# clayne/CPU-Raytracer

Hardware: AMD Instinct MI355X
Metric: Mrays/s (primary+shadow+reflection+refraction) (higher is better)
Workload: dtype f32

## Files before the change

### cpu-raytracer_amd/csrc/plan_check.cpp

```cpp
#include <stdio.h>
#include <initializer_list>
#include <type_traits>
#include "rtx_plan.h"

static_assert(std::is_trivially_copyable<RenderPlan>::value, "the graph key compares a plan's bytes");

static int failures = 0;
static const char * current = "";
#define CASE(name) current = name
#define CHECK(x) do { if (!(x)) { printf("FAILED [%s] line %d: %s\n", current, __LINE__, #x); failures++; } } while (0)

enum { CW = RTX_RENDER_COUNT_WORK, SIMPLE = RTX_RENDER_SIMPLE_TRACE, CULL = RTX_RENDER_CULL_DEAD_SHADOW_RAYS, SERIAL = RTX_RENDER_SERIAL,
       LANE = RTX_RENDER_LANE_TRACE, PSTAT = RTX_RENDER_PACKET_STATS, PKC = RTX_RENDER_PACKET_CLOSEST, AOV = RTX_RENDER_AOV };
static const int NEVER = RTX_MAX_LEVELS + 1;

static PlanInputs frame() {
    PlanInputs in; memset(&in, 0, sizeof(in));
    in.tile_count = 64; in.batch_tiles = 64;
    Knobs & K = in.knobs;
    K.slot_budget = 48ll * 1000 * 1000; K.item_bytes_max = 1ll << 30; K.shade_grid = 4; K.lane_from_level = -1; K.lane_from_level_any = -1;
    K.split_items = 256; K.resolve_block = 256; K.pk4_order = 1; K.merge_any = true; K.lpt = -1;
    in.instance_count = 1; in.light_count = 2; in.bounces = 3; in.can_spawn = true; in.all_wide = true;
    in.stack = StackFigures{ false, 1, 10, 20 };
    in.n_cu = 256; in.pk_blocks_closest = 1024; in.pk_blocks_any = 1280;
// ... 317 lines not shown
    }
    CASE("graph");
    {
        PlanInputs in = frame(); in.knobs.graph = true;
        CHECK(plan_render(in).graph_eligible);
        in.timing = true;  CHECK(!plan_render(in).graph_eligible);
        in.timing = false; in.knobs.graph = false; CHECK(!plan_render(in).graph_eligible);
    }
    CASE("more tiles than a batch");
    {
        PlanInputs in = frame(); in.knobs.graph = true; in.knobs.lpt = 1; in.tile_count = 65;
        RenderPlan p = plan_render(in);
        CHECK(!p.graph_eligible && !p.lpt);
        in.knobs.graph = false;
        p = plan_render(in);
        CHECK(!p.graph_eligible && !p.lpt);
        in.tile_count = 64;
        CHECK(plan_render(in).lpt);
    }
    CASE("the key sees flags and views");
    {
        PlanInputs a = frame(), b = frame(); b.views = 1;
        CHECK(!same(plan_render(a), plan_render(b)));
        b = frame(CULL);
        CHECK(!same(plan_render(a), plan_render(b)));
    }
}

static void small_grids() {
    const struct { int n_cu, pk_closest, pk_any; } grids[] = { { 1, 8, 8 }, { 1, 16, 8 }, { 2, 16, 24 }, { 2, 32, 32 }, { 8, 32, 32 }, { 8, 8, 16 } };
    auto small = [](int n_cu, int pkc, int pka, uint32_t flags) {
        PlanInputs in = frame(flags); in.n_cu = n_cu; in.pk_blocks_closest = pkc; in.pk_blocks_any = pka; in.tile_count = in.batch_tiles = 60;
        return in;
    };
    CASE("small grids: a level's partial tallies fit its stride");
    for (const auto & g : grids)
        for (int fuse = 0; fuse <= 1; fuse++)
            for (uint32_t flags : { 0u, (uint32_t)SERIAL, (uint32_t)LANE, (uint32_t)CW, (uint32_t)SIMPLE, (uint32_t)AOV, (uint32_t)(CULL | SERIAL) }) {
                PlanInputs in = small(g.n_cu, g.pk_closest, g.pk_any, flags); in.knobs.fuse_shade = fuse != 0; in.bounces = RTX_MAX_LEVELS - 1;
                for (int shade_grid : { 1, 4, 64 }) {
                    in.knobs.shade_grid = shade_grid;
                    const RenderPlan p = plan_render(in);
                    CHECK(p.levels == RTX_MAX_LEVELS && p.shade_blocks == g.n_cu * shade_grid && p.pk_waves_closest == g.pk_closest);
                    CHECK(p.stats_stride >= 64 && p.stats_stride >= p.shade_blocks && p.stats_stride >= p.pk_waves_closest);
                    for (int slots : { 1024, 60 * 1024, 2025 * 1024 })
                        for (int l = 0; l < p.levels; l++) {
                            const int n = plan_stats_n(p, slots, l);
                            CHECK(n >= 1 && n <= p.stats_stride);
                            CHECK(n == (p.shade[l] == SHADE_NONE ? g.pk_closest : plan_level_blocks(slots, l, p.shade_blocks)));
                        }
                    if (fuse && flags == 0u) CHECK(all_shade(p, SHADE_NONE));
                    if (!fuse) for (int l = 0; l < p.levels; l++) CHECK(p.shade[l] != SHADE_NONE);
                }
            }
    {
        const RenderPlan p = plan_render(small(1, 8, 8, 0u));
        CHECK(p.shade_blocks == 4 && p.stats_stride == 64 && plan_stats_n(p, 60 * 1024, 0) == 64 && plan_stats_n(p, 60 * 1024, 3) == 64);
        CHECK(plan_render(small(8, 32, 32, 0u)).stats_stride == 64 && plan_render(small(32, 96, 96, 0u)).stats_stride == 128);
        CHECK(plan_render(frame()).stats_stride == 1024);
    }
    CASE("small grids: item capacity follows the chunk count");
    {
        CHECK(plan_render(small(1, 8, 8, 0u)).item_cap == 24192);
        CHECK(plan_render(small(2, 16, 16, 0u)).item_cap == 12096);
        CHECK(plan_render(small(8, 32, 32, 0u)).item_cap == 6080);
        PlanInputs in = small(1, 8, 8, 0u); in.tile_count = in.batch_tiles = 200;
        CHECK(plan_render(in).item_cap == 1 << 16 && plan_render(in).split);
        in.knobs.item_bytes_max = 8ll * 48 * 128;
        CHECK(plan_render(in).item_cap == 128 && plan_render(in).split);
        in.knobs.item_bytes_max = 8ll * 48 * 63;
        CHECK(plan_render(in).item_cap == 0 && !plan_render(in).split);
        in = small(1, 8, 8, 0u); in.knobs.split_items = 64; in.tile_count = in.batch_tiles = 1; in.light_count = 1;
        CHECK(plan_render(in).item_cap == 256);
    }
    CASE("small grids: the LPT default rule");
    for (const auto & g : grids) {
        PlanInputs in = small(g.n_cu, g.pk_closest, g.pk_any, 0u);
        RenderPlan p = plan_render(in);
        CHECK(p.lpt && p.lpt_n == 960);
        in.flags = SERIAL;
        CHECK(!plan_render(in).lpt);
        in.knobs.lpt = 1;
        CHECK(plan_render(in).lpt);
        in.flags = 0; in.knobs.lpt = 0;
        CHECK(!plan_render(in).lpt);
        in.knobs.lpt = -1; in.tile_count = in.batch_tiles = g.pk_closest / 8;
        CHECK(plan_render(in).lpt);
        if (g.pk_closest > 8) { in.tile_count = in.batch_tiles = g.pk_closest / 8 - 1; CHECK(!plan_render(in).lpt); }
    }
}

static void twelve_levels() {
    CASE("twelve levels");
    const int L = RTX_MAX_LEVELS;
    static_assert(sizeof(((RenderPlan *)0)->any) / sizeof(AnyLaunch) == RTX_MAX_LEVELS && sizeof(((RenderPlan *)0)->closest) / sizeof(int32_t) == RTX_MAX_LEVELS &&
                  sizeof(((RenderPlan *)0)->shade) / sizeof(int32_t) == RTX_MAX_LEVELS, "the plan's per-level arrays");
    long plans = 0;
    for (uint32_t bits = 0; bits < 256; bits++) {
        const uint32_t flags = (bits & 1 ? SERIAL : 0) | (bits & 2 ? LANE : 0) | (bits & 4 ? PKC : 0) | (bits & 8 ? CULL : 0) | (bits & 16 ? CW : 0) |
                               (bits & 32 ? SIMPLE : 0) | (bits & 64 ? PSTAT : 0) | (bits & 128 ? AOV : 0);
        for (int lights : { 1, 33 }) for (int instances : { 1, 2, 65 }) for (int fuse = 0; fuse <= 1; fuse++) for (int split : { 0, 64 })
        for (int merge = 0; merge <= 1; merge++) for (int lane_from : { -1, 0, 5, 11 }) for (int lane_from_any : { -1, 5 }) {
            PlanInputs in = frame(flags);
            in.bounces = L - 1; in.can_spawn = true; in.light_count = lights; in.instance_count = instances;
            in.knobs.fuse_shade = fuse != 0; in.knobs.split_items = split; in.knobs.merge_any = merge != 0;
            in.knobs.lane_from_level = lane_from; in.knobs.lane_from_level_any = lane_from_any;
            const RenderPlan p = plan_render(in);
            plans++;
            CHECK(p.levels == L);
            CHECK(p.n_any >= 1 && p.n_any <= L);
            const bool plain = (flags & (CW | SIMPLE)) != 0;
            for (int l = 0; l < L; l++) {
                const int c = p.closest[l], s = p.shade[l];
                CHECK(c >= CLOSEST_PLAIN && c <= CLOSEST_PACKET_FUSED_CULL && s >= SHADE_NONE && s <= SHADE_AOV_CULL);
                CHECK((c == CLOSEST_PLAIN || c == CLOSEST_PLAIN_COUNT) == plain);
                CHECK((s == SHADE_NONE) == (c == CLOSEST_PACKET_FUSED || c == CLOSEST_PACKET_FUSED_CULL));
                CHECK((s == SHADE_AOV || s == SHADE_AOV_COUNT || s == SHADE_AOV_CULL) == ((flags & AOV) != 0 && l == 0));
                const int n = plan_stats_n(p, in.batch_tiles * 1024, l);
                CHECK(n >= 1 && n <= p.stats_stride);
            }
            int covered[RTX_MAX_LEVELS] = { 0 };
            int last_after = -1;
            for (int i = 0; i < p.n_any && i < L; i++) {
                const AnyLaunch & a = p.any[i];
                CHECK(a.lo >= 0 && a.lo <= a.hi && a.hi <= L - 1);
                CHECK(a.after_level >= a.hi && a.after_level <= p.levels - 1);
                CHECK(a.after_level >= last_after); last_after = a.after_level;
                CHECK(a.stream == (p.overlap ? 1 : 0));
                CHECK(a.kernel >= ANY_PLAIN && a.kernel <= ANY_PACKET_SPLIT && (a.items == 0 || a.kernel == ANY_PACKET_SPLIT));
                if (a.kernel == ANY_PLAIN || a.kernel == ANY_PLAIN_COUNT) CHECK(a.lo == a.hi);
                for (int l = a.lo; l <= a.hi && l < L; l++) if (l >= 0) covered[l]++;
            }
            for (int l = 0; l < L; l++) CHECK(covered[l] == 1);
            if (p.split) CHECK(p.item_cap >= 64 && p.item_cap <= (1 << 16));
        }
    }
    CHECK(plans == 256l * 2 * 3 * 2 * 2 * 2 * 4 * 2);
    {
        PlanInputs in = frame(SERIAL); in.bounces = L - 1; in.light_count = 33;
        CHECK(schedule(plan_render(in), { { 11, 0, ANY_PACKET_SPLIT, 0, 11, 1 } }));
        in.flags = 0;
        CHECK(schedule(plan_render(in), { { 0, 1, ANY_PACKET_SPLIT, 0, 0, 1 }, { 11, 1, ANY_PACKET_SPLIT, 1, 11, 1 } }));
        in.instance_count = 2; in.knobs.split_items = 0;
        CHECK(schedule(plan_render(in), { { 0, 1, ANY_PACKET, 0, 0, 0 }, { 11, 1, ANY_PACKET, 1, 1, 0 }, { 11, 1, ANY_LANE, 2, 11, 0 } }));
        in.knobs.lane_from_level = 11;
        const RenderPlan p = plan_render(in);
        CHECK(p.closest[10] == CLOSEST_PACKET && p.closest[11] == CLOSEST_LANE);
        CHECK(schedule(p, { { 0, 1, ANY_PACKET, 0, 0, 0 }, { 11, 1, ANY_PACKET, 1, 10, 0 }, { 11, 1, ANY_LANE, 11, 11, 0 } }));
        in.flags = SERIAL; in.knobs.merge_any = false;
        CHECK(plan_render(in).n_any == L);
    }
}

int main() {
    small_grids();
    twelve_levels();
    modes_and_schedule();
    instrumented_modes();
    stack_limits();
    two_deep_trees();
    lpt_items_graph();
    if (failures) { printf("plan_check: %d FAILED\n", failures); return 1; }
    printf("plan_check: ok\n");
    return 0;
}
```

### cpu-raytracer_amd/csrc/rtx_api.hip

```cpp
#include <hip/hip_runtime.h>
#include <stdio.h>
#include <stdlib.h>
#include <string.h>
#include <math.h>
#include <string>
#include <vector>
#include <algorithm>
#include <type_traits>

#include "../../include/rtx.h"
#include "rtx_device.h"
#include "rtx_math.h"
#include "rtx_libm.h"
#include "rtx_texture.h"
#include "rtx_trace.h"
#include "rtx_shade.h"
#include "rtx_packet.h"
#include "rtx_present.h"
#include "rtx_update.h"
#include "rtx_refit.h"
#include "rtx_build.h"
#include "rtx_normals.h"
#include "rtx_query.h"
#include "rtx_nearest.h"
#include "rtx_hits.h"
#include "rtx_sweep.h"
#include "rtx_overlap.h"
#include "rtx_boxsweep.h"
#include "rtx_texmip.h"
#include <rocprim/device/device_radix_sort.hpp>
#include "rtx_hostmem.h"
#include "rtx_layout_host.h"
#include "rtx_plan.h"

#define SLOT_BUDGET (48ll * 1000 * 1000)

static long long knob_int(const char * name, long long dflt, long long lo, long long hi) {
    const char * e = getenv(name);
    if (!e || !*e) return dflt;
    char * end = nullptr; const long long v = strtoll(e, &end, 10);
    if (end == e || *end != 0 || v < lo || v > hi) { fprintf(stderr, "librtx_hip: %s=%s ignored (expected an integer in [%lld, %lld])\n", name, e, lo, hi); return dflt; }
    return v;
}
static double knob_real(const char * name, double dflt, double lo, double hi) {
    const char * e = getenv(name);
    if (!e || !*e) return dflt;
    char * end = nullptr; const double v = strtod(e, &end);
    if (end == e || *end != 0 || !(v >= lo && v <= hi)) { fprintf(stderr, "librtx_hip: %s=%s ignored (expected a number in [%g, %g])\n", name, e, lo, hi); return dflt; }
    return v;
}
struct KernelTime { const char * name; hipEvent_t a, b; };

struct rtx_ctx {
    rtx_config cfg;
    hipStream_t stream = nullptr;
    hipStream_t own_stream = nullptr;
    hipStream_t any_stream = nullptr;
    hipEvent_t ev_shade0 = nullptr, ev_shade_last = nullptr, ev_any_done = nullptr;
    void * ext_rgb = nullptr, * ext_packed = nullptr;
    std::string err;
    int n_cu = 0;

    struct BlasRefit { std::vector<int32_t> map4, map4c; bool bound = false; int32_t vertex_count = 0; DevBuf block; DevRefit dev; float * planes[3] = { nullptr, nullptr, nullptr }; void * sort_tmp = nullptr; size_t sort_bytes = 0; };
    struct BlasBuild { bool allocated = false; DevBuf block; DevBuild dev; void * sort_tmp = nullptr; size_t sort_bytes = 0; int levels = 0; };
    struct BlasNormals { bool allocated = false, set = false; DevBuf block; DevNormals dev; void * sort_tmp = nullptr; size_t sort_bytes = 0; unsigned int key_bits = 0; };
    struct BlasSide { bool allocated = false; DevBuf block; DevSide dev; };
    struct BlasHost { std::vector<DevBuf> arrays; int max_local_material = -1, inner_depth = -1; bool packet_ok = true; BlasRefit refit; BlasBuild build; BlasNormals normals; BlasSide side; };
    std::vector<DevBlas> h_blas;
    std::vector<BlasHost> blas;
    DevBuf d_blas, d_materials, d_textures, d_sky, d_ewa;
    std::vector<DevTexture> h_tex;
    std::vector<DevBuf> tex_texels;
    struct TexUpdate { bool allocated = false; rtxt::Plan plan; };
    std::vector<TexUpdate> tex_update;
    DevBuf d_srgb_lut;
    bool sky_uploaded = false;
    int material_count = 0, sky_size = 0;
    std::vector<rtx_material> h_materials; int tlas_inner_depth = -1; std::vector<int> frame_primitive_materials; bool refs_dirty = true; Knobs knobs; int item_blocks = 0, item_cap_alloc = 0; DevBuf d_pk_items, d_pk_item_count;

    DevBuf d_frame;
    StageRing frame_ring;
    DevScene scene;
    bool frame_set = false;
    bool frame_rigid = true;
    DevBuf d_upd, d_upd_sort; int upd_cap = 0;
    DevBuf d_views, d_vfb_rgb, d_vfb_packed;
    StageRing view_ring;
    int32_t view_count = 0, vfb_cap = 0, ext_vcap = 0;
    void * ext_vrgb = nullptr, * ext_vpacked = nullptr;
    DevBuf d_rays;
    StageRing ray_ring;
    int32_t ray_count = 0, ext_ray_count = 0;
    const void * ext_rays = nullptr;
    uint32_t aov_channels = 0; bool aov_ext = false; int64_t aov_ext_cap = 0; DevAov aov_ext_ptrs = {};
    DevBuf d_aov[8]; int64_t aov_own_cap[8] = {};

    DevQueues q;
    DevBuf qb[20];
    DevBuf d_query[4], d_query_counters, d_query_heads; int32_t query_cap = 0;
    DevBuf d_query_sort; int32_t query_sort_cap = 0; size_t query_sort_tmp = 0;
    DevBuf d_nearest_head; bool nearest_fetch = true;
    int query_grid = 0;
    DevBuf d_object_masks; StageRing mask_ring; bool masks_set = false; int32_t mask_counts[3] = { 0, 0, 0 };
    std::vector<DevSideBlas> h_side; DevBuf d_side; StageRing side_ring; bool side_dirty = true;
    size_t slots_alloc = 0, shadow_alloc = 0;
    DevBuf d_stats_partial, d_pk_fifo, d_counters, d_spill, d_fb_rgb, d_fb_packed, d_display, d_gamma, d_pk_heads;
    int trace_blocks_closest = 0, trace_blocks_any = 0, trace_blocks_count = 0;
    int pk_blocks_closest = 0, pk_blocks_any = 0;

    rtx_stats stats_acc; rtx_work_counters work_acc; uint32_t err_flags_acc = 0;
    bool stats_pending = false;

    bool timing = false;
    bool serial = false;
    hipGraphExec_t graph_exec = nullptr; std::vector<unsigned char> graph_key, graph_warm;
    DevBuf d_pk_cost, d_pk_order; hipStream_t order_stream = nullptr; hipEvent_t ev_cost = nullptr, ev_order = nullptr; int32_t lpt_key[5] = { -1, -1, -1, -1, -1 }; bool lpt_valid = false;
    std::vector<KernelTime> times;
    std::vector<hipEvent_t> event_pool;
    size_t event_next = 0;
};

extern "C" int rtx_abi_version(void) { return RTX_ABI_VERSION; }

extern "C" const char * rtx_last_error(const rtx_ctx * ctx) { return ctx ? ctx->err.c_str() : "null context"; }

extern "C" int rtx_create(const rtx_config * config, rtx_ctx ** out_ctx) {
    if (!config || !out_ctx) return RTX_ERR_INVALID_ARG;
    *out_ctx = nullptr;
    if (config->width <= 0 || config->height <= 0 || config->bounces < 0) return RTX_ERR_INVALID_ARG;
    if (config->bounces + 1 > RTX_MAX_LEVELS) return RTX_ERR_LIMIT;
    if (config->stack_size < 1 || config->stack_size > RTX_MAX_STACK) return RTX_ERR_LIMIT;
    if (config->traversal_strategy < 0 || config->traversal_strategy > 1 || config->texture_mode < 0 || config->texture_mode > 2 ||
        config->mip_filter < 0 || config->mip_filter > 2) return RTX_ERR_INVALID_ARG;
    int n_dev = 0;
    if (hipGetDeviceCount(&n_dev) != hipSuccess || n_dev <= 0) return RTX_ERR_NO_DEVICE;
    if (config->device < 0 || config->device >= n_dev) return RTX_ERR_NO_DEVICE;
    if (hipSetDevice(config->device) != hipSuccess) return RTX_ERR_NO_DEVICE;

    rtx_ctx * c = new rtx_ctx();
    c->cfg = *config;
    memset(&c->scene, 0, sizeof(c->scene));
    memset(&c->q, 0, sizeof(c->q));
    memset(&c->stats_acc, 0, sizeof(c->stats_acc));
    memset(&c->work_acc, 0, sizeof(c->work_acc));
    hipDeviceProp_t prop;
    if (hipGetDeviceProperties(&prop, config->device) != hipSuccess) { delete c; return RTX_ERR_HIP; }
    c->n_cu = prop.multiProcessorCount;
    {
        const long long cus = knob_int("RTX_GRID_CUS", c->n_cu, 1, 1 << 20);
        if (cus < c->n_cu) c->n_cu = (int)cus;
    }
    if (hipStreamCreateWithFlags(&c->own_stream, hipStreamNonBlocking) != hipSuccess) { delete c; return RTX_ERR_HIP; }
    c->stream = c->own_stream;
    hipEventCreateWithFlags(&c->ev_shade0, hipEventDisableTiming); hipEventCreateWithFlags(&c->ev_shade_last, hipEventDisableTiming);
    hipEventCreateWithFlags(&c->ev_any_done, hipEventDisableTiming);

    float ewa[RTX_EWA_LUT_SIZE];
    {
        const float alpha = 2.0f;
        const float denom = 1.0f / (float)(RTX_EWA_LUT_SIZE - 1);
        const float exp_neg_alpha = expf(-alpha);
        for (int i = 0; i < RTX_EWA_LUT_SIZE; i++) { float r2 = (float)i * denom; ewa[i] = expf(-alpha * r2) - exp_neg_alpha; }
    }
    int rc = upload(c, c->d_ewa, ewa, sizeof(ewa));
    rtx_material m0; memset(&m0, 0, sizeof(m0)); m0.texture_id = -1; m0.index_of_refraction = 1.0f;
    if (!rc) rc = upload(c, c->d_materials, &m0, sizeof(m0));
    c->material_count = 1;
    const size_t px = (size_t)config->width * config->height;
    if (!rc) rc = ensure(c, c->d_fb_rgb, px * 12);
    if (!rc) rc = ensure(c, c->d_fb_packed, px * 4);
    if (!rc) rc = ensure(c, c->d_counters, sizeof(DevCounters));
    if (!rc) rc = ensure(c, c->d_pk_heads, (size_t)2 * (RTX_MAX_LEVELS + 1) * RTX_PK_CLASSES * 32 * sizeof(uint32_t));
    float zero_sky[6] = { 0, 0, 0, 0, 0, 0 };
    if (!rc) rc = upload(c, c->d_sky, zero_sky, sizeof(zero_sky));
    c->sky_size = 1;
    if (rc) { rtx_destroy(c); return rc; }
    hipMemset(c->d_fb_rgb.p, 0, px * 12);
    hipMemset(c->d_fb_packed.p, 0, px * 4);

    Knobs & K = c->knobs;
    K.slot_budget = knob_int("RTX_SLOT_BUDGET", SLOT_BUDGET, 1024, 1ll << 31);
    K.item_bytes_max = knob_int("RTX_PK_ITEM_BYTES", 1ll << 30, 0, 1ll << 36);
    K.shade_grid = (int)knob_int("RTX_SHADE_GRID", 4, 1, 64);
    K.lane_from_level = (int)knob_int("RTX_LANE_FROM_LEVEL", -1, 0, 1 << 20);
    K.lane_from_level_any = (int)knob_int("RTX_LANE_FROM_LEVEL_ANY", -1, 0, 1 << 20);
    K.split_items = (int)knob_int("RTX_PK_SPLIT", 256, 0, 1 << 16);
    if (K.split_items > 0) K.split_items = (K.split_items + 63) & ~63;
    K.resolve_block = (int)knob_int("RTX_RESOLVE_BLOCK", 256, 64, 256);
    if (K.resolve_block != 64 && K.resolve_block != 128 && K.resolve_block != 256) K.resolve_block = 256;
    K.pk4_order = (int)knob_int("RTX_PK4_ORDER", 1, 0, 1);
    K.merge_any = knob_int("RTX_SERIAL_MERGE_ANY", 1, 0, 1) != 0;
    K.no_wide = knob_int("RTX_PK_WIDE", 1, 0, 1) == 0;
    K.lpt = (int)knob_int("RTX_PK_LPT", -1, -1, 1);
    K.graph = knob_int("RTX_GRAPH", 0, 0, 1) != 0;
    K.no_wide_closest = knob_int("RTX_PK_WIDE_CLOSEST", 1, 0, 1) == 0;
    K.fuse_shade = knob_int("RTX_FUSE_SHADE", 0, 0, 1) != 0;
    K.update_small_max = (int)knob_int("RTX_UPDATE_SMALL_MAX", RTX_UPDATE_SMALL_MAX, 0, RTX_UPDATE_SMALL_MAX);
    K.tex_pass_levels = (int)knob_int("RTX_TEX_PASS_LEVELS", rtxt::DEFAULT_PASS_LEVELS, 1, rtxt::MAX_PASS_LEVELS);
    c->nearest_fetch = knob_int("RTX_NEAREST_FETCH", 1, 0, 1) != 0;
    c->query_grid = (int)knob_int("RTX_QUERY_GRID", 0, 0, 1 << 20);
    K.fail_item_alloc = knob_int("RTX_DEBUG_FAIL_ITEM_ALLOC", 0, 0, 1) != 0;
    int bpc = 0;
    hipOccupancyMaxActiveBlocksPerMultiprocessor(&bpc, k_trace_fast<false>, RTX_TRACE_BLOCK, 0);
    c->trace_blocks_closest = c->n_cu * (bpc > 0 ? bpc : 2);
    hipOccupancyMaxActiveBlocksPerMultiprocessor(&bpc, k_trace_fast<true>, RTX_TRACE_BLOCK, 0);
    c->trace_blocks_any = c->n_cu * (bpc > 0 ? bpc : 2);
    hipOccupancyMaxActiveBlocksPerMultiprocessor(&bpc, k_trace<false, true>, RTX_TRACE_BLOCK, 0);
    c->trace_blocks_count = c->n_cu * (bpc > 0 ? bpc : 2);
    if (K.fuse_shade) hipOccupancyMaxActiveBlocksPerMultiprocessor(&bpc, k_packet<false, false, false, true, false>, RTX_PK_BLOCK, 0);
    else              hipOccupancyMaxActiveBlocksPerMultiprocessor(&bpc, k_packet<false, false>, RTX_PK_BLOCK, 0);
    c->pk_blocks_closest = (c->n_cu * (bpc > 0 ? bpc : 4) + 1) & ~1;
    hipOccupancyMaxActiveBlocksPerMultiprocessor(&bpc, k_packet<true, false>, RTX_PK_BLOCK, 0);
    c->pk_blocks_any = (c->n_cu * (bpc > 0 ? bpc : 4) + 1) & ~1;
    {
        const double f = knob_real("RTX_PK_GRID_SCALE", 1.0, 0.05, 16.0);
        if (f != 1.0) { c->pk_blocks_closest = ((int)(c->pk_blocks_closest * f) + 1) & ~1; c->pk_blocks_any = ((int)(c->pk_blocks_any * f) + 1) & ~1; }
        const double fa = knob_real("RTX_PK_GRID_ANY", 0.0, 0.05, 64.0), fc = knob_real("RTX_PK_GRID_CLOSEST", 0.0, 0.05, 64.0);
        if (fa > 0.0) c->pk_blocks_any = ((int)(c->n_cu * fa) + 1) & ~1;
        if (fc > 0.0) c->pk_blocks_closest = ((int)(c->n_cu * fc) + 1) & ~1;
    }
    {
        const int g = RTX_PK_CLASSES * RTX_WAVE / RTX_PK_BLOCK > 1 ? RTX_PK_CLASSES * RTX_WAVE / RTX_PK_BLOCK : 1;
        c->pk_blocks_any = (c->pk_blocks_any + g - 1) / g * g; c->pk_blocks_closest = (c->pk_blocks_closest + g - 1) / g * g;
        if (c->pk_blocks_any < g) c->pk_blocks_any = g;
        if (c->pk_blocks_closest < g) c->pk_blocks_closest = g;
    }
    long long max_threads = (long long)(c->trace_blocks_closest > c->trace_blocks_any ? c->trace_blocks_closest : c->trace_blocks_any) * RTX_TRACE_BLOCK;
    if ((long long)c->trace_blocks_count * RTX_TRACE_BLOCK > max_threads) max_threads = (long long)c->trace_blocks_count * RTX_TRACE_BLOCK;
    if ((long long)c->pk_blocks_any * RTX_PK_BLOCK > max_threads) max_threads = (long long)c->pk_blocks_any * RTX_PK_BLOCK;
    if ((long long)c->pk_blocks_closest * RTX_PK_BLOCK > max_threads) max_threads = (long long)c->pk_blocks_closest * RTX_PK_BLOCK;
    c->q.pk_defer_t0 = (int)knob_int("RTX_PK_DEFER", 8, 0, 64);
    c->q.pk_defer_leaf = (int)knob_int("RTX_PK_DEFER_LEAF", c->q.pk_defer_t0 / 2, 0, 64);
    c->q.pk_defer_t0_closest = (int)knob_int("RTX_PK_DEFER_CLOSEST", 64, 0, 64);
    c->q.pk_closest_asm = (int)knob_int("RTX_PK_CLOSEST_ASM", 1, 0, 1);
    c->q.pk_defer_t0_primary = (int)knob_int("RTX_PK_DEFER_PRIMARY", c->q.pk_closest_asm ? 4 : 64, 0, 64);
    c->q.pk_order = (int)knob_int("RTX_PK_ORDER", 1, 0, 1);
    c->q.prof_level = (int)knob_int("RTX_LANE_PROF_LEVEL", 2, 0, 100 + RTX_MAX_LEVELS);
    c->q.pk_defer_grow = (int)knob_int("RTX_PK_GROW", 3, 0, 31);
    c->q.spill_threads = (int)max_threads;
    rc = ensure(c, c->d_spill, (size_t)c->q.spill_threads * (RTX_MAX_STACK - RTX_LDS_STACK) * 4 * 3);
    if (!rc) rc = ensure(c, c->d_pk_fifo, (size_t)c->q.spill_threads * RTX_PK_FIFO * 8);
    { int ib = 0; hipOccupancyMaxActiveBlocksPerMultiprocessor(&ib, k_items, RTX_ITEM_BLOCK, 0); c->item_blocks = c->n_cu * (ib > 0 ? ib : 4);
      const double f = knob_real("RTX_ITEM_GRID", 0.0, 0.05, 64.0); if (f > 0.0) c->item_blocks = (int)(c->n_cu * f) > 0 ? (int)(c->n_cu * f) : 1; }
    c->q.pk_items = nullptr; c->q.pk_item_count = nullptr; c->q.pk_item_cap = 0;
    if (rc) { rtx_destroy(c); return rc; }
    bind_tables(c);
    *out_ctx = c;
    return RTX_OK;
}

extern "C" int rtx_destroy(rtx_ctx * c) {
    if (!c) return RTX_ERR_INVALID_ARG;
    hipSetDevice(c->cfg.device);
    if (c->stream) hipStreamSynchronize(c->stream);
    for (hipEvent_t e : c->event_pool) hipEventDestroy(e);
    if (c->graph_exec) { hipGraphExecDestroy(c->graph_exec); c->graph_exec = nullptr; }
    if (c->order_stream) { hipStreamSynchronize(c->order_stream); hipStreamDestroy(c->order_stream); hipEventDestroy(c->ev_cost); hipEventDestroy(c->ev_order); }
    if (c->any_stream) { hipStreamSynchronize(c->any_stream); hipStreamDestroy(c->any_stream); }
    if (c->ev_shade0) hipEventDestroy(c->ev_shade0);
    if (c->ev_shade_last) hipEventDestroy(c->ev_shade_last);
    if (c->ev_any_done) hipEventDestroy(c->ev_any_done);
    if (c->own_stream) hipStreamDestroy(c->own_stream);
    delete c;
    return RTX_OK;
}

static bool validate_tree(const rtx_bvh_node * nodes, int node_count, int64_t primitive_count, int * max_inner_depth = nullptr, int * max_leaf_count = nullptr) {
    if (node_count < 1) return false;
    std::vector<unsigned char> seen((size_t)node_count, 0);
    std::vector<std::pair<int, int>> stack(1, std::make_pair(0, 0));
    int deepest = -1, biggest = 0;
    while (!stack.empty()) {
        const int i = stack.back().first, d = stack.back().second; stack.pop_back();
        if (seen[i]) return false;
        seen[i] = 1;
        const int cnt = nodes[i].count & 0x3fffffff, f = nodes[i].left_or_first;
        if (cnt > 0) { if (f < 0 || (int64_t)f + cnt > primitive_count) return false; if (cnt > biggest) biggest = cnt; }
        else { if (f < 0 || f + 1 >= node_count) return false; if (d > deepest) deepest = d; stack.push_back(std::make_pair(f, d + 1)); stack.push_back(std::make_pair(f + 1, d + 1)); }
    }
    if (max_inner_depth) *max_inner_depth = deepest;
    if (max_leaf_count) *max_leaf_count = biggest;
    return true;
}


struct BlasStaged { DevBlas B; rtx_ctx::BlasHost H; };

template <typename T> static int stage_array(rtx_ctx * c, std::vector<DevBuf> & arrays, const void * src, size_t copy, size_t bytes, const T ** out) {
    DevBuf b;
    if (int rc = ensure(c, b, bytes)) return rc;
    if (copy) HIP_OK(c, hipMemcpy(b.p, src, copy, hipMemcpyHostToDevice));
    *out = (const T *)b.p;
    arrays.push_back(std::move(b));
    return RTX_OK;
}

template <typename Accept> static int upload_blas_table(rtx_ctx * c, std::vector<DevBlas> & table, Accept && accept) {
    return replace_table(c, c->d_blas, table.data(), table.size() * sizeof(DevBlas), [&] { c->h_blas.swap(table); accept(); });
}

static void drop_side_entry(rtx_ctx * c, int32_t blas_id) {
    if ((size_t)blas_id < c->h_side.size() && c->h_side[blas_id].vert_pn) { memset(&c->h_side[blas_id], 0, sizeof(DevSideBlas)); c->side_dirty = true; }
}

static int commit_blas(rtx_ctx * c, int32_t blas_id, BlasStaged & S) {
    std::vector<DevBlas> table = c->h_blas;
    if ((size_t)blas_id >= table.size()) { DevBlas none; memset(&none, 0, sizeof(none)); table.resize(blas_id + 1, none); }
    table[blas_id] = S.B;
    return upload_blas_table(c, table, [&] {
        if (c->blas.size() < c->h_blas.size()) c->blas.resize(c->h_blas.size());
        c->blas[blas_id] = std::move(S.H);
        c->refs_dirty = true;
        drop_side_entry(c, blas_id);
    });
}

static int stage_blas(rtx_ctx * c, int32_t blas_id, const rtx_bvh_node * nodes, int32_t node_count,
                      const rtx_triangle_hot * tri_hot, const rtx_triangle_cold * tri_cold,
                      int32_t triangle_count, int32_t material_offset, int pk4_order, BlasStaged & S) {
    if (!c || blas_id < 0 || blas_id >= (1 << 20) || !nodes || node_count <= 0 || triangle_count < 0 || (triangle_count > 0 && (!tri_hot || !tri_cold)))
        return RTX_ERR_INVALID_ARG;
    int inner_depth = -1, leaf_max = 0;
    if (!validate_tree(nodes, node_count, triangle_count, &inner_depth, &leaf_max)) return RTX_ERR_INVALID_ARG;
    int max_local = -1;
    for (int i = 0; i < triangle_count; i++) { if (tri_cold[i].material_id < 0) return RTX_ERR_INVALID_ARG; if (tri_cold[i].material_id > max_local) max_local = tri_cold[i].material_id; }
    hipSetDevice(c->cfg.device);

    std::vector<float4> nd; convert_nodes(nodes, node_count, nd);
    std::vector<float4> th((size_t)RTX_TRI_STRIDE * (triangle_count > 0 ? triangle_count : 1), make_float4(0.0f, 0.0f, 0.0f, 0.0f));
    for (int i = 0; i < triangle_count; i++) {
        th[RTX_TRI_STRIDE * (size_t)i]     = make_float4(tri_hot[i].position_0[0], tri_hot[i].position_0[1], tri_hot[i].position_0[2], 0.0f);
        th[RTX_TRI_STRIDE * (size_t)i + 1] = make_float4(tri_hot[i].position_edge_1[0], tri_hot[i].position_edge_1[1], tri_hot[i].position_edge_1[2], 0.0f);
        th[RTX_TRI_STRIDE * (size_t)i + 2] = make_float4(tri_hot[i].position_edge_2[0], tri_hot[i].position_edge_2[1], tri_hot[i].position_edge_2[2], 0.0f);
    }
    std::vector<float4> ndp; convert_nodes_pk(nodes, node_count, ndp);
    rtx_ctx::BlasHost & H = S.H;
    std::vector<float4> nd4; int need4 = 0;
    const bool wide = !c->knobs.no_wide && build_nodes_pk4(nodes, node_count, triangle_count, nd4, &need4, pk4_order, RTX_PK4_MAX_NEED, &H.refit.map4) && need4 <= RTX_PK4_MAX_NEED;
    std::vector<float4> nd4c; int need4c = 0;
    const bool wide_closest = !c->knobs.no_wide_closest && build_nodes_pk4c(nodes, node_count, triangle_count, nd4c, &need4c, &H.refit.map4c) && need4c <= RTX_MAX_STACK - 2;
    if (!wide) H.refit.map4.clear();
    if (!wide_closest) H.refit.map4c.clear();
    std::vector<float> planes[3];
    for (int a = 0; a < 3; a++) {
        planes[a].reserve((size_t)node_count * 2);
        for (int i = 0; i < node_count; i++) { planes[a].push_back(nodes[i].aabb_min[a]); planes[a].push_back(nodes[i].aabb_max[a]); }
        planes[a].erase(std::remove_if(planes[a].begin(), planes[a].end(), [](float v) { return v != v; }), planes[a].end());
        std::sort(planes[a].begin(), planes[a].end());
        planes[a].erase(std::unique(planes[a].begin(), planes[a].end()), planes[a].end());
        if (planes[a].empty()) planes[a].push_back(INFINITY);
    }
    DevBlas & B = S.B;
    memset(&B, 0, sizeof(B));
    int rc = RTX_OK;
    for (int a = 0; a < 3 && !rc; a++) { rc = stage_array(c, H.arrays, planes[a].data(), planes[a].size() * 4, planes[a].size() * 4, &B.planes[a]); B.plane_count[a] = (int32_t)planes[a].size(); }
    if (!rc && wide_closest) rc = stage_array(c, H.arrays, nd4c.data(), nd4c.size() * 16, nd4c.size() * 16, &B.pk4c_nodes);
    if (!rc && wide) rc = stage_array(c, H.arrays, nd4.data(), nd4.size() * 16, nd4.size() * 16, &B.pk4_nodes);
    if (!rc) rc = stage_array(c, H.arrays, nd.data(), nd.size() * 16, nd.size() * 16, &B.nodes);
    if (!rc) rc = stage_array(c, H.arrays, ndp.data(), ndp.size() * 16, ndp.size() * 16, &B.pk_nodes);
    if (!rc) rc = stage_array(c, H.arrays, th.data(), th.size() * 16, th.size() * 16, &B.tri_hot);
    if (!rc) rc = stage_array(c, H.arrays, tri_cold, (size_t)triangle_count * sizeof(rtx_triangle_cold), (size_t)(triangle_count > 0 ? triangle_count : 1) * sizeof(rtx_triangle_cold), &B.tri_cold);
    if (rc) return rc;
    B.node_count = node_count; B.tri_count = triangle_count; B.material_offset = material_offset; B.pk4_need = wide ? need4 : -1; B.pk4c_need = wide_closest ? need4c : -1;
    H.max_local_material = max_local;
    H.inner_depth = inner_depth;
    H.packet_ok = leaf_max < 65536 && node_count < (1 << 26) && triangle_count < (1 << 25);
    return RTX_OK;
}

extern "C" int rtx_upload_blas(rtx_ctx * c, int32_t blas_id, const rtx_bvh_node * nodes, int32_t node_count,
                               const rtx_triangle_hot * tri_hot, const rtx_triangle_cold * tri_cold,
                               int32_t triangle_count, int32_t material_offset) {
    BlasStaged S;
    if (int rc = stage_blas(c, blas_id, nodes, node_count, tri_hot, tri_cold, triangle_count, material_offset, c ? c->knobs.pk4_order : 0, S)) return rc;
    return commit_blas(c, blas_id, S);
}

extern "C" int rtx_upload_materials(rtx_ctx * c, const rtx_material * materials, int32_t count) {
    if (!c || !materials || count <= 0) return RTX_ERR_INVALID_ARG;
    if (count > RTX_MAX_MATERIALS) return RTX_ERR_LIMIT;
    hipSetDevice(c->cfg.device);
    return replace_table(c, c->d_materials, materials, (size_t)count * sizeof(rtx_material), [&] {
        c->material_count = count;
        c->h_materials.assign(materials, materials + count); c->refs_dirty = true;
    });
}

static int commit_texture(rtx_ctx * c, int32_t texture_id, const rtx_texture_desc & desc, DevBuf & d, const rtx_ctx::TexUpdate & update) {
    std::vector<DevTexture> table = c->h_tex;
    if ((size_t)texture_id >= table.size()) { DevTexture none; memset(&none, 0, sizeof(none)); table.resize(texture_id + 1, none); }
    table[texture_id].desc = desc;
    table[texture_id].texels = (const float4 *)d.p;
    return replace_table(c, c->d_textures, table.data(), table.size() * sizeof(DevTexture), [&] {
        c->h_tex.swap(table);
        if (c->tex_texels.size() < c->h_tex.size()) { c->tex_texels.resize(c->h_tex.size()); c->tex_update.resize(c->h_tex.size()); }
        c->tex_texels[texture_id] = std::move(d);
        c->tex_update[texture_id] = update;
        c->refs_dirty = true;
    });
}

extern "C" int rtx_upload_texture(rtx_ctx * c, int32_t texture_id, const rtx_texture_desc * desc, const float * texels_rgb, int64_t texel_count) {
    if (!c || texture_id < 0 || texture_id >= 4096 || !desc || !texels_rgb) return RTX_ERR_INVALID_ARG;
    if (desc->width <= 0 || desc->height <= 0 || desc->mip_levels < 1 || desc->mip_levels > RTX_MAX_MIP_LEVELS) return RTX_ERR_INVALID_ARG;
    for (int l = 0; l < desc->mip_levels; l++) {
        const int64_t lw = desc->width >> l, lh = desc->height >> l;
        if (lw < 1 || lh < 1 || desc->mip_offsets[l] < 0 || desc->mip_offsets[l] + lw * lh > texel_count) return RTX_ERR_INVALID_ARG;
    }
    hipSetDevice(c->cfg.device);
    DevBuf d;
    {
        std::vector<float4> padded((size_t)texel_count);
        for (int64_t i = 0; i < texel_count; i++) padded[(size_t)i] = make_float4(texels_rgb[3 * i], texels_rgb[3 * i + 1], texels_rgb[3 * i + 2], 0.0f);
        if (int rc = upload(c, d, padded.data(), (size_t)texel_count * 16)) return rc;
    }
    return commit_texture(c, texture_id, *desc, d, rtx_ctx::TexUpdate());
}

extern "C" int rtx_upload_sky(rtx_ctx * c, const float * texels_rgb, int32_t size) {
    if (!c || !texels_rgb || size <= 0 || size > 16384) return RTX_ERR_INVALID_ARG;
    hipSetDevice(c->cfg.device);
    std::vector<float> padded((size_t)size * size * 3 + 3, 0.0f);
    memcpy(padded.data(), texels_rgb, (size_t)size * size * 12);
    return replace_table(c, c->d_sky, padded.data(), padded.size() * 4, [&] { c->sky_size = size; c->sky_uploaded = true; });
}

extern "C" int rtx_set_frame(rtx_ctx * c, const rtx_frame * f) {
    if (!c || !f) return RTX_ERR_INVALID_ARG;
    if (f->tlas_node_count < 0 || f->instance_count < 0 || f->sphere_count < 0 || f->plane_count < 0 || f->tlas_index_count < 0 ||
        f->point_light_count < 0 || f->spot_light_count < 0 || f->directional_light_count < 0) return RTX_ERR_INVALID_ARG;
    if ((f->tlas_node_count && !f->tlas_nodes) || (f->instance_count && !f->instances) || (f->tlas_index_count && !f->tlas_indices) ||
        (f->sphere_count && !f->spheres) || (f->plane_count && !f->planes) || (f->point_light_count && !f->point_lights) ||
        (f->spot_light_count && !f->spot_lights) || (f->directional_light_count && !f->directional_lights)) return RTX_ERR_INVALID_ARG;
    if (f->instance_count >= (1 << 28) || f->sphere_count >= (1 << 28) || f->plane_count >= (1 << 28)) return RTX_ERR_LIMIT;
    hipSetDevice(c->cfg.device);
    int tlas_depth = -1;
    if (f->tlas_node_count > 0 && !validate_tree(f->tlas_nodes, f->tlas_node_count, f->tlas_index_count, &tlas_depth)) return RTX_ERR_INVALID_ARG;
    for (int i = 0; i < f->tlas_index_count; i++) if (f->tlas_indices[i] < 0 || f->tlas_indices[i] >= f->instance_count) return RTX_ERR_INVALID_ARG;
    for (int i = 0; i < f->instance_count; i++) {
        const int b = f->instances[i].blas_id;
        if (b < 0 || (size_t)b >= c->h_blas.size() || !c->h_blas[b].nodes) return RTX_ERR_STATE;
    }
    bool rigid = true;
    for (int i = 0; i < f->instance_count; i++) {
        if (!rtxu::matrix_finite(f->instances[i].world) || !rtxu::matrix_finite(f->instances[i].world_inv)) {
            c->err = "rtx_set_frame: instance " + std::to_string(i) + " has a NaN or infinite world / world_inv cell"; return RTX_ERR_INVALID_ARG;
        }
        rigid = rigid && rtxu::instance_rigid(f->instances[i].world, f->instances[i].world_inv);
    }
    std::vector<float4> nd, ndp; convert_nodes(f->tlas_nodes, f->tlas_node_count, nd); convert_nodes_pk(f->tlas_nodes, f->tlas_node_count, ndp);
    const void * src[9] = { nd.data(), ndp.data(), f->tlas_indices, f->instances, f->spheres, f->planes, f->point_lights, f->spot_lights, f->directional_lights };
    const size_t len[9] = { nd.size() * 16, ndp.size() * 16, (size_t)f->tlas_index_count * 4, (size_t)f->instance_count * sizeof(rtx_instance),
                            (size_t)f->sphere_count * sizeof(rtx_sphere), (size_t)f->plane_count * sizeof(rtx_plane), (size_t)f->point_light_count * sizeof(rtx_point_light),
                            (size_t)f->spot_light_count * sizeof(rtx_spot_light), (size_t)f->directional_light_count * sizeof(rtx_directional_light) };
    size_t off[9], total = 0;
    for (int k = 0; k < 9; k++) { off[k] = total; total += (len[k] + 255) & ~(size_t)255; if (len[k] == 0) total += 256; }
    int rc = RTX_OK;
    if (total > c->d_frame.cap) {
        HIP_OK(c, hipStreamSynchronize(c->stream));
        rc = ensure(c, c->d_frame, total + total / 2);
        if (rc) return rc;
    }
    rc = stage_copy(c, c->frame_ring, c->d_frame.p, total, total + total / 2, [&](void * host) { for (int k = 0; k < 9; k++) if (len[k]) memcpy((char *)host + off[k], src[k], len[k]); });
    if (rc) return rc;
    char * const fb = (char *)c->d_frame.p;

    DevScene & s = c->scene;
    s.width = c->cfg.width; s.height = c->cfg.height; s.bounces = c->cfg.bounces; s.stack_size = c->cfg.stack_size;
    s.traversal_strategy = c->cfg.traversal_strategy; s.texture_mode = c->cfg.texture_mode; s.mip_filter = c->cfg.mip_filter;
    s.heatmap = c->cfg.heatmap ? 1 : 0;
    s.diff_enabled = c->cfg.texture_mode == RTX_TEXTURE_MIPMAP;
    s.max_anisotropy = c->cfg.max_anisotropy;
    s.tile_count_x = (c->cfg.width + RTX_TILE_SIZE - 1) / RTX_TILE_SIZE;
    memcpy(s.cam_pos, f->camera.position, 12); memcpy(s.cam_tl, f->camera.rotated_top_left_corner, 12);
    memcpy(s.cam_x, f->camera.rotated_x_axis, 12); memcpy(s.cam_y, f->camera.rotated_y_axis, 12);
    memcpy(s.ambient, f->ambient, 12);
    bind_tables(c);
    s.ewa_table = (const float *)c->d_ewa.p;
    s.tlas_nodes = (const float4 *)(fb + off[0]); s.tlas_node_count = f->tlas_node_count; s.pk_tlas_nodes = (const float4 *)(fb + off[1]);
    s.tlas_indices = (const int32_t *)(fb + off[2]); s.tlas_index_count = f->tlas_index_count;
    s.instances = (const rtx_instance *)(fb + off[3]); s.instance_count = f->instance_count;
    s.spheres = (const rtx_sphere *)(fb + off[4]); s.sphere_count = f->sphere_count;
    s.planes = (const rtx_plane *)(fb + off[5]); s.plane_count = f->plane_count;
    s.point_lights = (const rtx_point_light *)(fb + off[6]); s.point_light_count = f->point_light_count;
    s.spot_lights = (const rtx_spot_light *)(fb + off[7]); s.spot_light_count = f->spot_light_count;
    s.dir_lights = (const rtx_directional_light *)(fb + off[8]); s.dir_light_count = f->directional_light_count;
    s.light_count = f->point_light_count + f->spot_light_count + f->directional_light_count;
    c->frame_primitive_materials.clear();
    for (int i = 0; i < f->sphere_count; i++) c->frame_primitive_materials.push_back(f->spheres[i].material_id);
    for (int i = 0; i < f->plane_count; i++) c->frame_primitive_materials.push_back(f->planes[i].material_id);
    c->tlas_inner_depth = tlas_depth;
    c->frame_set = true; c->refs_dirty = true; c->frame_rigid = rigid;
    return RTX_OK;
}

static int validate_references(rtx_ctx * c) {
    if (!c->refs_dirty) return RTX_OK;
    const int nm = c->material_count;
    for (int id : c->frame_primitive_materials) if (id < 0 || id >= nm) { c->err = "sphere / plane material id outside the uploaded material table"; return RTX_ERR_STATE; }
    for (size_t b = 0; b < c->h_blas.size(); b++) {
        if (!c->h_blas[b].nodes) continue;
        const int hi = c->blas[b].max_local_material;
        if (c->h_blas[b].material_offset < 0 || (hi >= 0 && (long long)c->h_blas[b].material_offset + hi >= nm)) { c->err = "BLAS material_offset + triangle material id outside the uploaded material table"; return RTX_ERR_STATE; }
    }
    for (size_t b = 0; b < c->h_blas.size(); b++)
        if (c->h_blas[b].nodes && c->blas[b].inner_depth + 2 > c->cfg.stack_size) {
            c->err = "BVH deeper than rtx_config.stack_size allows (BVH_TRAVERSAL_STACK_SIZE, Config.h:25): an inner node at depth " + std::to_string(c->blas[b].inner_depth) + " needs " + std::to_string(c->blas[b].inner_depth + 2) + " stack entries";
            return RTX_ERR_LIMIT;
        }
    if (c->tlas_inner_depth + 2 > c->cfg.stack_size) { c->err = "TLAS deeper than rtx_config.stack_size allows (BVH_TRAVERSAL_STACK_SIZE, Config.h:25)"; return RTX_ERR_LIMIT; }
    for (size_t i = 0; i < c->h_materials.size(); i++) {
        const int t = c->h_materials[i].texture_id;
        if (t >= 0 && ((size_t)t >= c->h_tex.size() || !c->h_tex[t].texels)) { c->err = "material refers to a texture id that was never uploaded"; return RTX_ERR_STATE; }
    }
    c->refs_dirty = false;
    return RTX_OK;
}

static int plan_batch(rtx_ctx * c, int tiles, int & out_tiles) {
    const int levels = c->cfg.bounces + 1;
    const long long per_tile = 1024ll * ((1ll << levels) - 1);
    const long long budget = c->knobs.slot_budget;
    long long t = budget / per_tile;
    if (t < 1) t = 1;
    out_tiles = (int)(t < tiles ? t : tiles);
    return RTX_OK;
}

static int alloc_queues(rtx_ctx * c, int batch_tiles) {
    const int levels = c->cfg.bounces + 1;
    const long long P = 1024ll * batch_tiles;
    long long total = 0;
    const long long chunk_slack = c->knobs.fuse_shade ? (long long)c->pk_blocks_closest * (RTX_PK_BLOCK / RTX_WAVE) * RTX_PK_CHUNK : 0;
    for (int d = 0; d <= RTX_MAX_LEVELS; d++) {
        long long cap = d < levels ? (P << d) + (d > 0 ? chunk_slack : 0) : 0;
        c->q.level_base[d] = (int32_t)total; c->q.level_cap[d] = (int32_t)cap;
        total += cap;
    }
    if (total >= (1ll << 31)) { c->err = "batch too large"; return RTX_ERR_LIMIT; }
    const int nL = c->scene.light_count;
    long long stotal = 0;
    for (int d = 0; d <= RTX_MAX_LEVELS; d++) { c->q.shadow_base[d] = (int32_t)stotal; stotal += (long long)c->q.level_cap[d] * nL; }
    if (stotal >= (1ll << 31)) { c->err = "shadow queue too large"; return RTX_ERR_LIMIT; }
    const size_t slots = (size_t)total, sslots = (size_t)(stotal > 0 ? stotal : 1);
    int rc = 0, k = 0;
    void ** f4[] = { (void **)&c->q.r0, (void **)&c->q.r1, (void **)&c->q.r2, (void **)&c->q.r3, (void **)&c->q.r4, (void **)&c->q.h0,
                     (void **)&c->q.n0, (void **)&c->q.n1, (void **)&c->q.n2, (void **)&c->q.c0, (void **)&c->q.c1,
                     (void **)&c->q.sp, (void **)&c->q.sn };
    for (void ** p : f4) { if (!rc) rc = ensure(c, c->qb[k], slots * 16); *p = c->qb[k].p; k++; }
    if (!rc) rc = ensure(c, c->qb[k], slots * 4); c->q.h1 = (int32_t *)c->qb[k].p; k++;
    c->q.views = nullptr; c->q.s0 = c->q.s1 = nullptr; c->q.shadow_explicit = 0; c->q.cull = 0;
    if (!rc) rc = ensure(c, c->qb[k], sslots * 4); c->q.socc = (uint32_t *)c->qb[k].p; k++;
    c->q.spill = (int32_t *)c->d_spill.p;
    c->q.counters = (DevCounters *)c->d_counters.p;
    c->q.pk_heads = (uint32_t *)c->d_pk_heads.p;
    c->q.pk_fifo = (int32_t *)c->d_pk_fifo.p;
    c->q.fb_rgb = (float *)(c->ext_rgb ? c->ext_rgb : c->d_fb_rgb.p);
    c->q.fb_packed = (uint32_t *)(c->ext_packed ? c->ext_packed : c->d_fb_packed.p);
    return rc;
}

__global__ void k_begin_batch(DevCounters * ctr, uint32_t * pk_heads, uint32_t primary_slots, uint32_t closest_threads, uint32_t any_threads,
                              uint32_t pk_waves_closest, uint32_t pk_waves_any, int first_batch) {
    const int i = threadIdx.x;
    if (first_batch) {
        uint32_t * w = reinterpret_cast<uint32_t *>(ctr);
        for (int k = i; k < (int)(sizeof(DevCounters) / 4); k += blockDim.x) w[k] = 0u;
        __syncthreads();
    }
    if (i <= RTX_MAX_LEVELS) { ctr->ray_count[i] = (i == 0) ? primary_slots : 0u; ctr->item_max[i] = 0u; ctr->fetch_closest[i] = closest_threads; ctr->fetch_any[i] = any_threads; }
    for (int k = i; k < 2 * (RTX_MAX_LEVELS + 1) * RTX_PK_CLASSES; k += blockDim.x)
        pk_heads[k * 32] = (k < (RTX_MAX_LEVELS + 1) * RTX_PK_CLASSES ? pk_waves_closest : pk_waves_any) / RTX_PK_CLASSES;
}

static hipEvent_t next_event(rtx_ctx * c) {
    if (c->event_next == c->event_pool.size()) { hipEvent_t e; hipEventCreate(&e); c->event_pool.push_back(e); }
    return c->event_pool[c->event_next++];
}

__global__ __launch_bounds__(1024) void k_packet_order(const uint32_t * __restrict__ cost, uint32_t * __restrict__ order, const uint32_t n) {
    __shared__ uint32_t hist[256], base[256];
    for (uint32_t i = threadIdx.x; i < 256; i += blockDim.x) hist[i] = 0;
    __syncthreads();
    auto cls = [](uint32_t c) { const uint32_t k = c >> 7; return 255u - (k < 255u ? k : 255u); };
    for (uint32_t i = threadIdx.x; i < n; i += blockDim.x) atomicAdd(&hist[cls(cost[i])], 1u);
    __syncthreads();
    if (threadIdx.x == 0) { uint32_t acc = 0; for (int k = 0; k < 256; k++) { base[k] = acc; acc += hist[k]; } }
    __syncthreads();
    for (uint32_t i = threadIdx.x; i < n; i += blockDim.x) order[atomicAdd(&base[cls(cost[i])], 1u)] = i;
}

template <typename F>
static void launch_timed(rtx_ctx * c, const char * name, hipStream_t stream, F && launch) {
    if (c->timing) {
        KernelTime kt; kt.name = name; kt.a = next_event(c); kt.b = next_event(c);
        hipEventRecord(kt.a, stream);
        launch();
        hipEventRecord(kt.b, stream);
        c->times.push_back(kt);
    } else launch();
}

static void begin_batch(rtx_ctx * c, DevCounters * counters, uint32_t * pk_heads, uint32_t primary_slots, bool plain, bool first_batch) {
    hipLaunchKernelGGL(k_begin_batch, dim3(1), dim3(64), 0, c->stream, counters, pk_heads, primary_slots,
                       (uint32_t)((plain ? c->trace_blocks_count : c->trace_blocks_closest) * RTX_TRACE_BLOCK),
                       (uint32_t)((plain ? c->trace_blocks_count : c->trace_blocks_any) * RTX_TRACE_BLOCK),
                       (uint32_t)(c->pk_blocks_closest * (RTX_PK_BLOCK / RTX_WAVE)), (uint32_t)(c->pk_blocks_any * (RTX_PK_BLOCK / RTX_WAVE)), first_batch ? 1 : 0);
}

static void launch_closest_level1(rtx_ctx * c, const DevScene & sc, const DevQueues & q, bool lane) {
    if (lane) hipLaunchKernelGGL((k_trace_fast<false>), dim3(c->trace_blocks_closest), dim3(RTX_TRACE_BLOCK), 0, c->stream, sc, q, 1, 1);
    else      hipLaunchKernelGGL((k_packet<false, false>), dim3(c->pk_blocks_closest), dim3(RTX_PK_BLOCK), 0, c->stream, sc, q, 1, 1);
}
static void launch_any_level0(rtx_ctx * c, const DevScene & sc, const DevQueues & q, bool lane) {
    if (lane) hipLaunchKernelGGL((k_trace_fast<true>), dim3(c->trace_blocks_any), dim3(RTX_TRACE_BLOCK), 0, c->stream, sc, q, 0, 0);
    else      hipLaunchKernelGGL((k_packet<true, false>), dim3(c->pk_blocks_any), dim3(RTX_PK_BLOCK), 0, c->stream, sc, q, 0, 0);
}

static int32_t frame_tiles(const rtx_ctx * c) { return ((c->cfg.width + RTX_TILE_SIZE - 1) / RTX_TILE_SIZE) * ((c->cfg.height + RTX_TILE_SIZE - 1) / RTX_TILE_SIZE); }
static bool all_meshes_wide(const rtx_ctx * c) {
    for (const DevBlas & b : c->h_blas) if (b.nodes && !b.pk4_nodes) return false;
    return true;
}

static size_t aligned_parts(const size_t * len, size_t * off, int n) {
    size_t total = 0;
    for (int k = 0; k < n; k++) { off[k] = total; total += (len[k] + 255) & ~(size_t)255; }
    return total;
}

template <typename Key> static int sort_storage_bytes(rtx_ctx * c, size_t count, unsigned int bits, size_t & bytes) {
    bytes = 0;
    if (rocprim::radix_sort_keys(nullptr, bytes, (const Key *)nullptr, (Key *)nullptr, (unsigned int)count, 0u, bits, c->stream) == hipSuccess) return RTX_OK;
    hipGetLastError(); c->err = "rocprim::radix_sort_keys size query failed"; return RTX_ERR_HIP;
}

static int sort_failed(rtx_ctx * c, hipError_t se) {
    hipGetLastError(); c->err = std::string("rocprim::radix_sort_keys: ") + hipGetErrorString(se); return RTX_ERR_HIP;
}

static int read_lane_nodes(rtx_ctx * c, const float4 * dev, int n, rtx_bvh_node * out) {
    std::vector<float4> nd((size_t)2 * n);
    HIP_OK(c, hipMemcpy(nd.data(), dev, nd.size() * 16, hipMemcpyDeviceToHost));
    for (int i = 0; i < n; i++) rtxl::node_from_lane(nd.data(), i, out[i]);
    return RTX_OK;
}

extern "C" int rtx_update_instances(rtx_ctx * c, const void * positions_dev, const void * rotations_dev, int32_t instance_count) {
    if (!c) return RTX_ERR_INVALID_ARG;
    if (!positions_dev || !rotations_dev || ((uintptr_t)positions_dev & 3) || ((uintptr_t)rotations_dev & 3) || instance_count < 1) {
        c->err = "rtx_update_instances: null or misaligned pose pointer, or no instances"; return RTX_ERR_INVALID_ARG; }
    if (instance_count > RTX_UPDATE_MAX_INSTANCES) { c->err = "rtx_update_instances supports up to 65 536 instances"; return RTX_ERR_LIMIT; }
    if (!c->frame_set) { c->err = "rtx_update_instances before rtx_set_frame"; return RTX_ERR_STATE; }
    if (instance_count != c->scene.instance_count) { c->err = "rtx_update_instances: instance_count differs from the frame's"; return RTX_ERR_INVALID_ARG; }
    if (rtxu::tree_inner_depth(instance_count) + 2 > c->cfg.stack_size) {
        c->err = "rtx_update_instances: the balanced TLAS of " + std::to_string(instance_count) + " instances needs " + std::to_string(rtxu::tree_inner_depth(instance_count) + 2) +
                 " stack entries, rtx_config.stack_size allows fewer (BVH_TRAVERSAL_STACK_SIZE, Config.h:25)";
        return RTX_ERR_LIMIT;
    }
    hipSetDevice(c->cfg.device);
    const int n = instance_count, levels = rtxu::tree_levels(n), slots = rtxu::tree_node_count(n);
    const bool small = n <= c->knobs.update_small_max;
    const size_t len[7] = { (size_t)slots * 32, (size_t)slots * 32, (size_t)n * 4, (size_t)n * sizeof(rtx_instance), (size_t)n * 24, (size_t)n * 8, 24 };
    size_t off[7];
    const size_t total = aligned_parts(len, off, 7);
    if (n > c->upd_cap || total > c->d_upd.cap) {
        HIP_OK(c, hipStreamSynchronize(c->stream));
        if (int rc = ensure(c, c->d_upd, total)) return rc;
        c->upd_cap = n;
    }
    size_t sort_bytes = 0;
    if (!small) {
        if (int rc = sort_storage_bytes<uint64_t>(c, (size_t)n, RTXU_KEY_BITS, sort_bytes)) return rc;
        const size_t keys_in = ((size_t)n * 8 + 255) & ~(size_t)255;
        if (keys_in + sort_bytes > c->d_upd_sort.cap) {
            HIP_OK(c, hipStreamSynchronize(c->stream));
            if (int rc = ensure(c, c->d_upd_sort, keys_in + sort_bytes)) return rc;
        }
    }
    char * const ub = (char *)c->d_upd.p;
    DevUpdate u;
    u.positions = (const float *)positions_dev; u.rotations = (const float *)rotations_dev;
    u.src_instances = c->scene.instances; u.blas = c->scene.blas;
    u.nodes = (float4 *)(ub + off[0]); u.pk_nodes = (float4 *)(ub + off[1]); u.indices = (int32_t *)(ub + off[2]);
    u.instances = (rtx_instance *)(ub + off[3]); u.aabbs = (float *)(ub + off[4]); u.keys = (uint64_t *)(ub + off[5]); u.bounds = (uint32_t *)(ub + off[6]);
    u.n = n; u.levels = levels;
    if (small) {
        launch_timed(c, "k_update_small", c->stream, [&] { hipLaunchKernelGGL(k_update_small, dim3(1), dim3(RTX_UPDATE_BLOCK), 0, c->stream, u); });
    } else {
        uint64_t * const keys_in = (uint64_t *)c->d_upd_sort.p;
        void * const sort_tmp = (char *)c->d_upd_sort.p + (((size_t)n * 8 + 255) & ~(size_t)255);
        const int blocks = (n + 255) / 256;
        HIP_OK(c, hipMemsetAsync(u.bounds, 0xff, 24, c->stream));
        launch_timed(c, "k_update_instances", c->stream, [&] { hipLaunchKernelGGL(k_update_instances, dim3(blocks), dim3(256), 0, c->stream, u); });
        launch_timed(c, "k_update_keys", c->stream, [&] { hipLaunchKernelGGL(k_update_keys, dim3(blocks), dim3(256), 0, c->stream, u, keys_in); });
        hipError_t se = hipSuccess;
        launch_timed(c, "update_radix_sort", c->stream, [&] { se = rocprim::radix_sort_keys(sort_tmp, sort_bytes, (const uint64_t *)keys_in, u.keys, (unsigned int)n, 0u, (unsigned int)RTXU_KEY_BITS, c->stream); });
        if (se != hipSuccess) return sort_failed(c, se);
        for (int d = levels; d > RTX_UPDATE_TOP_LEVELS; d--)
            launch_timed(c, "k_update_level", c->stream, [&] { hipLaunchKernelGGL(k_update_level, dim3(((1 << d) + 255) / 256), dim3(256), 0, c->stream, u, d); });
        launch_timed(c, "k_update_top", c->stream, [&] { hipLaunchKernelGGL(k_update_top, dim3(1), dim3(RTX_UPDATE_BLOCK), 0, c->stream, u); });
    }
    HIP_OK(c, hipGetLastError());
    DevScene & s = c->scene;
    s.tlas_nodes = u.nodes; s.pk_tlas_nodes = u.pk_nodes; s.tlas_node_count = slots;
    s.tlas_indices = u.indices; s.tlas_index_count = n; s.instances = u.instances;
    c->tlas_inner_depth = rtxu::tree_inner_depth(n);
    c->refs_dirty = true;
    c->frame_rigid = true;
    return RTX_OK;
}

extern "C" int rtx_read_frame_state(rtx_ctx * c, rtx_instance * instances, rtx_bvh_node * tlas_nodes, int32_t * tlas_node_count, int32_t * tlas_indices) {
    if (!c) return RTX_ERR_INVALID_ARG;
    if (!c->frame_set) { c->err = "rtx_read_frame_state before rtx_set_frame"; return RTX_ERR_STATE; }
    hipSetDevice(c->cfg.device);
    HIP_OK(c, hipStreamSynchronize(c->stream));
    const DevScene & s = c->scene;
    if (tlas_node_count) *tlas_node_count = s.tlas_node_count;
    if (instances && s.instance_count) HIP_OK(c, hipMemcpy(instances, s.instances, (size_t)s.instance_count * sizeof(rtx_instance), hipMemcpyDeviceToHost));
    if (tlas_indices && s.tlas_index_count) HIP_OK(c, hipMemcpy(tlas_indices, s.tlas_indices, (size_t)s.tlas_index_count * 4, hipMemcpyDeviceToHost));
    if (tlas_nodes && s.tlas_node_count) return read_lane_nodes(c, s.tlas_nodes, s.tlas_node_count, tlas_nodes);
    return RTX_OK;
}

static int refit_launch_finish(rtx_ctx * c, rtx_ctx::BlasRefit & R, bool build = false) {
    const DevRefit & r = R.dev;
    const int n = r.node_count;
    const dim3 grid((2 * n + 4 + RTX_REFIT_BLOCK - 1) / RTX_REFIT_BLOCK);
    if (build) launch_timed(c, "k_build_finish", c->stream, [&] { hipLaunchKernelGGL(k_build_finish, grid, dim3(RTX_REFIT_BLOCK), 0, c->stream, r); });
    else launch_timed(c, "k_refit_finish", c->stream, [&] { hipLaunchKernelGGL(k_refit_finish, grid, dim3(RTX_REFIT_BLOCK), 0, c->stream, r); });
    hipError_t se = hipSuccess;
    launch_timed(c, "refit_plane_sort", c->stream, [&] {
        for (int a = 0; a < 3 && se == hipSuccess; a++) {
            size_t bytes = R.sort_bytes;
            se = rocprim::radix_sort_keys(R.sort_tmp, bytes, (const float *)r.plane_keys[a], R.planes[a], (unsigned int)(2 * n), 0u, 32u, c->stream);
        }
    });
    if (se != hipSuccess) return sort_failed(c, se);
    HIP_OK(c, hipGetLastError());
    return RTX_OK;
}

static int plan_refit(rtx_ctx * c, DevBlas & B, rtx_ctx::BlasRefit & R, const int32_t * slot_vertices, int32_t vertex_count) {
    const int n = B.node_count, T = B.tri_count;
    std::vector<float4> nd((size_t)2 * n);
    HIP_OK(c, hipMemcpy(nd.data(), B.nodes, nd.size() * 16, hipMemcpyDeviceToHost));
    std::vector<int32_t> parent;
    parent_table(nd.data(), n, parent);
    size_t sort_bytes = 0;
    if (int rc = sort_storage_bytes<float>(c, (size_t)2 * n, 32u, sort_bytes)) return rc;
    const size_t slots = (size_t)2 * n + 4, pl = (size_t)2 * n * 4;
    const size_t len[12] = { (size_t)(T > 0 ? T : 1) * 12, (size_t)n * 4, (size_t)n * 4, R.map4.empty() ? 0 : slots * 4, R.map4c.empty() ? 0 : slots * 4, pl, pl, pl, pl, pl, pl, sort_bytes };
    size_t off[12];
    if (int rc = ensure(c, R.block, aligned_parts(len, off, 12))) return rc;
    char * const bb = (char *)R.block.p;
    if (T) HIP_OK(c, hipMemcpy(bb + off[0], slot_vertices, (size_t)T * 12, hipMemcpyHostToDevice));
    HIP_OK(c, hipMemcpy(bb + off[1], parent.data(), (size_t)n * 4, hipMemcpyHostToDevice));
    HIP_OK(c, hipMemset(bb + off[2], 0, (size_t)n * 4));
    if (!R.map4.empty()) HIP_OK(c, hipMemcpy(bb + off[3], R.map4.data(), slots * 4, hipMemcpyHostToDevice));
    if (!R.map4c.empty()) HIP_OK(c, hipMemcpy(bb + off[4], R.map4c.data(), slots * 4, hipMemcpyHostToDevice));
    DevRefit & r = R.dev;
    memset(&r, 0, sizeof(r));
    r.slot_vertices = (const int32_t *)(bb + off[0]); r.parent = (const int32_t *)(bb + off[1]); r.arrivals = (uint32_t *)(bb + off[2]);
    r.map4 = R.map4.empty() ? nullptr : (const int32_t *)(bb + off[3]); r.map4c = R.map4c.empty() ? nullptr : (const int32_t *)(bb + off[4]);
    for (int a = 0; a < 3; a++) r.plane_keys[a] = (float *)(bb + off[5 + a]);
    r.nodes = (float4 *)B.nodes; r.pk_nodes = (float4 *)B.pk_nodes; r.pk4_nodes = (float4 *)B.pk4_nodes; r.pk4c_nodes = (float4 *)B.pk4c_nodes;
    r.tri_hot = (float4 *)B.tri_hot; r.tri_cold = (float4 *)B.tri_cold;
    r.node_count = n; r.tri_count = T;
    R.sort_tmp = bb + off[11]; R.sort_bytes = sort_bytes;
    for (int a = 0; a < 3; a++) { R.planes[a] = (float *)(bb + off[8 + a]); B.planes[a] = R.planes[a]; B.plane_count[a] = 2 * n; }
    const int rc = refit_launch_finish(c, R);
    const hipError_t waited = hipStreamSynchronize(c->stream);
    if (rc) return rc;
    if (waited != hipSuccess) { c->err = std::string("hipStreamSynchronize: ") + hipGetErrorString(waited); return RTX_ERR_HIP; }
    R.bound = true; R.vertex_count = vertex_count;
    return RTX_OK;
}

extern "C" int rtx_bind_blas_vertices(rtx_ctx * c, int32_t blas_id, const int32_t * slot_vertices, int32_t vertex_count) {
    if (!c) return RTX_ERR_INVALID_ARG;
    if (!slot_vertices || blas_id < 0 || blas_id >= (1 << 20) || vertex_count < 1) { c->err = "rtx_bind_blas_vertices: null index table, bad id or no vertices"; return RTX_ERR_INVALID_ARG; }
    if ((size_t)blas_id >= c->h_blas.size() || !c->h_blas[blas_id].nodes) { c->err = "rtx_bind_blas_vertices: no BLAS uploaded under that id"; return RTX_ERR_STATE; }
    const int64_t T3 = 3 * (int64_t)c->h_blas[blas_id].tri_count;
    for (int64_t k = 0; k < T3; k++) if (slot_vertices[k] < 0 || slot_vertices[k] >= vertex_count) {
        c->err = "rtx_bind_blas_vertices: vertex index outside [0, vertex_count)"; return RTX_ERR_INVALID_ARG; }
    hipSetDevice(c->cfg.device);
    HIP_OK(c, hipStreamSynchronize(c->stream));
    rtx_ctx::BlasRefit & R = c->blas[blas_id].refit;
    if (R.bound) {
        if (T3) HIP_OK(c, hipMemcpy((void *)R.dev.slot_vertices, slot_vertices, (size_t)T3 * 4, hipMemcpyHostToDevice));
        R.vertex_count = vertex_count;
        return RTX_OK;
    }
    DevBlas B = c->h_blas[blas_id];
    rtx_ctx::BlasRefit N; N.map4 = R.map4; N.map4c = R.map4c;
    if (int rc = plan_refit(c, B, N, slot_vertices, vertex_count)) return rc;
    std::vector<DevBlas> table = c->h_blas;
    table[blas_id] = B;
    return upload_blas_table(c, table, [&] { c->blas[blas_id].refit = std::move(N); });
}

extern "C" int rtx_refit_blas(rtx_ctx * c, int32_t blas_id, const void * positions_dev, const void * normals_dev, int32_t vertex_count) {
    if (!c) return RTX_ERR_INVALID_ARG;
    if (!positions_dev || ((uintptr_t)positions_dev & 3) || ((uintptr_t)normals_dev & 3)) { c->err = "rtx_refit_blas: null or misaligned vertex pointer"; return RTX_ERR_INVALID_ARG; }
    if (blas_id < 0 || (size_t)blas_id >= c->h_blas.size() || !c->h_blas[blas_id].nodes || !c->blas[blas_id].refit.bound) {
        c->err = "rtx_refit_blas: no BLAS uploaded under that id, or no vertices bound to it (rtx_bind_blas_vertices)"; return RTX_ERR_STATE; }
    rtx_ctx::BlasRefit & R = c->blas[blas_id].refit;
    if (vertex_count != R.vertex_count) { c->err = "rtx_refit_blas: vertex_count differs from the bound one"; return RTX_ERR_INVALID_ARG; }
    hipSetDevice(c->cfg.device);
    DevRefit & r = R.dev;
    r.positions = (const float *)positions_dev; r.normals = (const float *)normals_dev;
    const int n = r.node_count, T = r.tri_count;
    if (T) launch_timed(c, "k_refit_triangles", c->stream, [&] { hipLaunchKernelGGL(k_refit_triangles, dim3((T + RTX_REFIT_BLOCK - 1) / RTX_REFIT_BLOCK), dim3(RTX_REFIT_BLOCK), 0, c->stream, r); });
    launch_timed(c, "k_refit_climb", c->stream, [&] { hipLaunchKernelGGL(k_refit_climb, dim3((n + RTX_REFIT_BLOCK - 1) / RTX_REFIT_BLOCK), dim3(RTX_REFIT_BLOCK), 0, c->stream, r); });
    return refit_launch_finish(c, R);
}

extern "C" int rtx_alloc_blas(rtx_ctx * c, int32_t blas_id, int32_t triangle_count, int32_t vertex_count, const int32_t * material_ids, int32_t material_offset) {
    if (!c) return RTX_ERR_INVALID_ARG;
    if (blas_id < 0 || blas_id >= (1 << 20) || triangle_count < 1 || vertex_count < 1) { c->err = "rtx_alloc_blas: bad id, no triangles or no vertices"; return RTX_ERR_INVALID_ARG; }
    int max_local = 0;
    if (material_ids) for (int i = 0; i < triangle_count; i++) {
        if (material_ids[i] < 0) { c->err = "rtx_alloc_blas: negative material id"; return RTX_ERR_INVALID_ARG; }
        if (material_ids[i] > max_local) max_local = material_ids[i];
    }
    if (triangle_count >= RTX_BUILD_MAX_TRIANGLES) { c->err = "rtx_alloc_blas supports fewer than 2^24 triangles (the 4-wide walks' limit)"; return RTX_ERR_LIMIT; }
    if (rtxb::tree_inner_depth(triangle_count) + 2 > c->cfg.stack_size) {
        c->err = "rtx_alloc_blas: the balanced BLAS of " + std::to_string(triangle_count) + " triangles needs " + std::to_string(rtxb::tree_inner_depth(triangle_count) + 2) +
                 " stack entries, rtx_config.stack_size allows fewer (BVH_TRAVERSAL_STACK_SIZE, Config.h:25)";
        return RTX_ERR_LIMIT;
    }
    hipSetDevice(c->cfg.device);
    const int T = triangle_count;
    std::vector<rtx_bvh_node> nodes;
    balanced_topology(T, nodes);
    BlasStaged S;
    {
        std::vector<rtx_triangle_hot> hot((size_t)T); std::vector<rtx_triangle_cold> cold((size_t)T);
        memset(hot.data(), 0, hot.size() * sizeof(rtx_triangle_hot)); memset(cold.data(), 0, cold.size() * sizeof(rtx_triangle_cold));
        if (int rc = stage_blas(c, blas_id, nodes.data(), (int32_t)nodes.size(), hot.data(), cold.data(), T, material_offset, 0, S)) return rc;
    }
    S.H.max_local_material = max_local;
    HIP_OK(c, hipStreamSynchronize(c->stream));
    {
        std::vector<int32_t> sv((size_t)3 * T, -1);
        if (int rc = plan_refit(c, S.B, S.H.refit, sv.data(), vertex_count)) return rc;
    }
    size_t sort_bytes = 0;
    if (int rc = sort_storage_bytes<uint64_t>(c, (size_t)T, RTXB_KEY_BITS, sort_bytes)) return rc;
    const size_t len[5] = { (size_t)T * 4, 24, (size_t)T * 8, (size_t)T * 8, sort_bytes };
    size_t off[5];
    rtx_ctx::BlasBuild & U = S.H.build;
    if (int rc = ensure(c, U.block, aligned_parts(len, off, 5))) return rc;
    char * const bb = (char *)U.block.p;
    if (material_ids) HIP_OK(c, hipMemcpy(bb + off[0], material_ids, (size_t)T * 4, hipMemcpyHostToDevice));
    else HIP_OK(c, hipMemset(bb + off[0], 0, (size_t)T * 4));
    memset(&U.dev, 0, sizeof(U.dev));
    U.dev.material_ids = (const int32_t *)(bb + off[0]); U.dev.bounds = (uint32_t *)(bb + off[1]);
    U.dev.keys_in = (uint64_t *)(bb + off[2]); U.dev.keys = (uint64_t *)(bb + off[3]);
    U.dev.slot_vertices = (int32_t *)S.H.refit.dev.slot_vertices;
    U.dev.tri_count = T; U.dev.vertex_count = vertex_count;
// ... 153 lines not shown
    if (nodes) if (int rc = read_lane_nodes(c, B.nodes, B.node_count, nodes)) return rc;
    if (hot && B.tri_count) {
        std::vector<float4> th((size_t)RTX_TRI_STRIDE * B.tri_count);
        HIP_OK(c, hipMemcpy(th.data(), B.tri_hot, th.size() * 16, hipMemcpyDeviceToHost));
        for (int i = 0; i < B.tri_count; i++) {
            const float4 * t = &th[(size_t)RTX_TRI_STRIDE * i];
            hot[i].position_0[0] = t[0].x; hot[i].position_0[1] = t[0].y; hot[i].position_0[2] = t[0].z;
            hot[i].position_edge_1[0] = t[1].x; hot[i].position_edge_1[1] = t[1].y; hot[i].position_edge_1[2] = t[1].z;
            hot[i].position_edge_2[0] = t[2].x; hot[i].position_edge_2[1] = t[2].y; hot[i].position_edge_2[2] = t[2].z;
        }
    }
    if (cold && B.tri_count) HIP_OK(c, hipMemcpy(cold, B.tri_cold, (size_t)B.tri_count * sizeof(rtx_triangle_cold), hipMemcpyDeviceToHost));
    return RTX_OK;
}

extern "C" int rtx_alloc_texture(rtx_ctx * c, int32_t texture_id, int32_t width, int32_t height, int32_t mipmapped) {
    if (!c) return RTX_ERR_INVALID_ARG;
    if (texture_id < 0 || texture_id >= 4096 || width < 1 || height < 1) { c->err = "rtx_alloc_texture: id outside [0, 4096) or an empty side"; return RTX_ERR_INVALID_ARG; }
    rtx_texture_desc desc; int64_t texel_count = 0;
    if (rtxt::chain_shape(width, height, mipmapped, &desc, &texel_count)) { c->err = "rtx_alloc_texture: more than RTX_MAX_MIP_LEVELS levels, or more texels than the int32_t offsets hold"; return RTX_ERR_LIMIT; }
    hipSetDevice(c->cfg.device);
    if (!c->d_srgb_lut.p) {
        float lut[256];
        for (int b = 0; b < 256; b++) {
            const float x = float(b) * 0.00392156862f;
            lut[b] = x <= 0.0f ? 0.0f : x >= 1.0f ? 1.0f : x < 0.04045f ? x / 12.92f : powf((x + 0.055f) / 1.055f, 2.4f);
        }
        DevBuf t;
        if (int rc = upload(c, t, lut, sizeof(lut))) return rc;
        c->d_srgb_lut = std::move(t);
    }
    DevBuf d;
    if (int rc = ensure(c, d, (size_t)texel_count * 16)) return rc;
    HIP_OK(c, hipMemsetAsync(d.p, 0, (size_t)texel_count * 16, c->stream));
    rtx_ctx::TexUpdate U;
    U.allocated = true;
    U.plan = rtxt::plan_passes(width, height, desc.mip_levels, c->knobs.tex_pass_levels);
    return commit_texture(c, texture_id, desc, d, U);
}

extern "C" int rtx_update_texture(rtx_ctx * c, int32_t texture_id, const void * texels_dev, int32_t format) {
    if (!c) return RTX_ERR_INVALID_ARG;
    if (!texels_dev || (format != RTX_TEXELS_RGB_F32 && format != RTX_TEXELS_RGBA8_SRGB) || (format == RTX_TEXELS_RGB_F32 && ((uintptr_t)texels_dev & 3))) {
        c->err = "rtx_update_texture: null or misaligned texel pointer, or an unknown format"; return RTX_ERR_INVALID_ARG; }
    if (texture_id < 0 || (size_t)texture_id >= c->h_tex.size() || !c->h_tex[texture_id].texels || !c->tex_update[texture_id].allocated) {
        c->err = "rtx_update_texture: the id was not created by rtx_alloc_texture (or was uploaded again since)"; return RTX_ERR_STATE; }
    hipSetDevice(c->cfg.device);
    const rtxt::Plan & plan = c->tex_update[texture_id].plan;
    float4 * const chain = (float4 *)c->tex_texels[texture_id].p;
    const float * const lut = (const float *)c->d_srgb_lut.p;
    for (int k = 0; k < plan.count; k++) {
        const rtxt::Pass & p = plan.pass[k];
        const dim3 grid((unsigned)(p.tiles_x * p.tiles_y)), block(rtxt::BLOCK);
        if (k > 0) launch_timed(c, "k_texmip_chain", c->stream, [&] { hipLaunchKernelGGL(k_texmip<TEXMIP_CHAIN>, grid, block, 0, c->stream, p, (const void *)nullptr, chain, lut); });
        else if (format == RTX_TEXELS_RGB_F32) launch_timed(c, "k_texmip_rgb_f32", c->stream, [&] { hipLaunchKernelGGL(k_texmip<TEXMIP_RGB_F32>, grid, block, 0, c->stream, p, texels_dev, chain, lut); });
        else launch_timed(c, "k_texmip_rgba8", c->stream, [&] { hipLaunchKernelGGL(k_texmip<TEXMIP_RGBA8_SRGB>, grid, block, 0, c->stream, p, texels_dev, chain, lut); });
    }
    HIP_OK(c, hipGetLastError());
    return RTX_OK;
}

extern "C" int rtx_read_texture(rtx_ctx * c, int32_t texture_id, rtx_texture_desc * desc, float * texels_rgb, int64_t capacity_texels) {
    if (!c) return RTX_ERR_INVALID_ARG;
    if (texture_id < 0 || texture_id >= 4096) { c->err = "rtx_read_texture: bad id"; return RTX_ERR_INVALID_ARG; }
    if ((size_t)texture_id >= c->h_tex.size() || !c->h_tex[texture_id].texels) { c->err = "rtx_read_texture: no texture under that id"; return RTX_ERR_STATE; }
    const DevTexture & T = c->h_tex[texture_id];
    int64_t count = 0;
    for (int l = 0; l < T.desc.mip_levels; l++) {
        const int64_t end = (int64_t)T.desc.mip_offsets[l] + (int64_t)(T.desc.width >> l) * (T.desc.height >> l);
        if (end > count) count = end;
    }
    if (texels_rgb && capacity_texels < count) { c->err = "rtx_read_texture: capacity_texels is smaller than the chain"; return RTX_ERR_INVALID_ARG; }
    if (desc) *desc = T.desc;
    if (!texels_rgb) return RTX_OK;
    hipSetDevice(c->cfg.device);
    HIP_OK(c, hipStreamSynchronize(c->stream));
    std::vector<float4> padded((size_t)count);
    HIP_OK(c, hipMemcpy(padded.data(), T.texels, (size_t)count * 16, hipMemcpyDeviceToHost));
    for (int64_t i = 0; i < count; i++) { texels_rgb[3 * i] = padded[(size_t)i].x; texels_rgb[3 * i + 1] = padded[(size_t)i].y; texels_rgb[3 * i + 2] = padded[(size_t)i].z; }
    return RTX_OK;
}

extern "C" int rtx_update_sky(rtx_ctx * c, const void * texels_dev, int32_t size) {
    if (!c) return RTX_ERR_INVALID_ARG;
    if (!texels_dev || ((uintptr_t)texels_dev & 3)) { c->err = "rtx_update_sky: null or misaligned texel pointer"; return RTX_ERR_INVALID_ARG; }
    if (!c->sky_uploaded) { c->err = "rtx_update_sky: no probe to copy over (rtx_upload_sky)"; return RTX_ERR_STATE; }
    if (size != c->sky_size) { c->err = "rtx_update_sky: size differs from the uploaded one"; return RTX_ERR_INVALID_ARG; }
    hipSetDevice(c->cfg.device);
    HIP_OK(c, hipMemcpyAsync(c->d_sky.p, texels_dev, (size_t)size * size * 12, hipMemcpyDeviceToDevice, c->stream));
    return RTX_OK;
}

extern "C" int rtx_debug_read_layouts(rtx_ctx * c, int32_t blas_id, int32_t * info8, float * pk_nodes, float * pk4_nodes, float * pk4c_nodes,
                                      float * planes_x, float * planes_y, float * planes_z) {
    if (!c) return RTX_ERR_INVALID_ARG;
    if (blas_id < -1 || blas_id >= (1 << 20)) { c->err = "rtx_debug_read_layouts: bad id"; return RTX_ERR_INVALID_ARG; }
    int32_t info[8] = { 0, 0, 0, 0, 0, 0, 0, 0 };
    if (blas_id == -1) {
        if (!c->frame_set) { c->err = "rtx_debug_read_layouts before rtx_set_frame"; return RTX_ERR_STATE; }
        hipSetDevice(c->cfg.device);
        HIP_OK(c, hipStreamSynchronize(c->stream));
        const DevScene & s = c->scene;
        info[0] = s.tlas_node_count;
        if (info8) memcpy(info8, info, sizeof(info));
        if (pk_nodes && s.tlas_node_count) HIP_OK(c, hipMemcpy(pk_nodes, s.pk_tlas_nodes, (size_t)s.tlas_node_count * 32, hipMemcpyDeviceToHost));
        return RTX_OK;
    }
    if ((size_t)blas_id >= c->h_blas.size() || !c->h_blas[blas_id].nodes) { c->err = "rtx_debug_read_layouts: no BLAS uploaded under that id"; return RTX_ERR_STATE; }
    hipSetDevice(c->cfg.device);
    HIP_OK(c, hipStreamSynchronize(c->stream));
    const DevBlas & B = c->h_blas[blas_id];
    info[0] = B.node_count; info[1] = B.pk4_nodes ? 1 : 0; info[2] = B.pk4c_nodes ? 1 : 0;
    for (int a = 0; a < 3; a++) info[3 + a] = B.plane_count[a];
    if (info8) memcpy(info8, info, sizeof(info));
    const size_t wide_bytes = ((size_t)4 * B.node_count + 8) * 16;
    if (pk_nodes) HIP_OK(c, hipMemcpy(pk_nodes, B.pk_nodes, (size_t)B.node_count * 32, hipMemcpyDeviceToHost));
    if (pk4_nodes && B.pk4_nodes) HIP_OK(c, hipMemcpy(pk4_nodes, B.pk4_nodes, wide_bytes, hipMemcpyDeviceToHost));
    if (pk4c_nodes && B.pk4c_nodes) HIP_OK(c, hipMemcpy(pk4c_nodes, B.pk4c_nodes, wide_bytes, hipMemcpyDeviceToHost));
    float * const planes[3] = { planes_x, planes_y, planes_z };
    for (int a = 0; a < 3; a++)
        if (planes[a] && B.plane_count[a]) HIP_OK(c, hipMemcpy(planes[a], B.planes[a], (size_t)B.plane_count[a] * 4, hipMemcpyDeviceToHost));
    return RTX_OK;
}

static StackFigures stack_figures(const rtx_ctx * c) {
    StackFigures s = { false, c->tlas_inner_depth < 0 ? 0 : c->tlas_inner_depth + 1, 0, 0 };
    for (size_t b = 0; b < c->h_blas.size(); b++) {
        if (!c->h_blas[b].nodes) continue;
        if (!c->blas[b].packet_ok) s.unfit_mesh = true;
        const int depth = c->blas[b].inner_depth + 2;
        const int any = c->h_blas[b].pk4_nodes ? c->h_blas[b].pk4_need : depth;
        if (any > s.blas_any) s.blas_any = any;
        if (2 * depth > s.blas_shared) s.blas_shared = 2 * depth;
    }
    return s;
}

static int render_tiles_impl(rtx_ctx * c, int32_t first_tile, int32_t tile_stride, int32_t tile_count, uint32_t flags, uint32_t * tile_major, int views = RTX_CAM_TILES);
static int aov_targets_of_call(rtx_ctx * c, int64_t pixels, DevAov & out);

extern "C" int rtx_render_tiles(rtx_ctx * c, int32_t first_tile, int32_t tile_stride, int32_t tile_count, uint32_t flags) {
    return render_tiles_impl(c, first_tile, tile_stride, tile_count, flags, nullptr);
}

static PlanInputs gather_plan_inputs(const rtx_ctx * c, uint32_t flags, int views, int tile_count, int batch_tiles, bool tile_major) {
    PlanInputs in; memset(&in, 0, sizeof(in));
    in.flags = flags; in.views = views; in.tile_count = tile_count; in.batch_tiles = batch_tiles; in.tile_major = tile_major; in.timing = c->timing;
    in.knobs = c->knobs;
    in.instance_count = c->scene.instance_count; in.light_count = c->scene.light_count; in.bounces = c->cfg.bounces; in.heatmap = c->scene.heatmap != 0;
    in.can_spawn = plan_can_spawn(c->h_materials.data(), c->h_materials.size());
    in.all_wide = all_meshes_wide(c);
    in.stack = stack_figures(c);
    in.n_cu = c->n_cu; in.pk_blocks_closest = c->pk_blocks_closest; in.pk_blocks_any = c->pk_blocks_any;
    return in;
}

static int alloc_for_plan(rtx_ctx * c, RenderPlan & plan) {
    if (int rc = ensure(c, c->d_stats_partial, (size_t)(RTX_MAX_LEVELS + 1) * plan.stats_stride * 4 * sizeof(uint32_t))) return rc;
    c->q.pk_items = nullptr; c->q.pk_item_count = nullptr; c->q.pk_item_cap = 0;
    if (plan.split) {
        const size_t chunks = (size_t)c->pk_blocks_any * (RTX_PK_BLOCK / RTX_WAVE);
        int cap = plan.item_cap;
        if (cap <= c->item_cap_alloc && c->d_pk_items.p && !c->knobs.fail_item_alloc) cap = c->item_cap_alloc;
        else {
            c->item_cap_alloc = 0;
            const size_t bytes = c->knobs.fail_item_alloc ? ((size_t)1 << 46) : chunks * (size_t)cap * 48;
            if (ensure(c, c->d_pk_items, bytes) == 0 && ensure(c, c->d_pk_item_count, chunks * 4) == 0) c->item_cap_alloc = cap;
            else { (void)hipGetLastError(); c->err.clear(); cap = 0; }
        }
        if (cap >= 64) { c->q.pk_items = (uint4 *)c->d_pk_items.p; c->q.pk_item_count = (uint32_t *)c->d_pk_item_count.p; c->q.pk_item_cap = cap; }
        else plan_drop_split(plan);
    }
    c->q.pk_cost = nullptr; c->q.pk_lpt_order = nullptr;
    if (plan.lpt) {
        if (int rc = ensure(c, c->d_pk_cost, (size_t)plan.lpt_n * 4)) return rc;
        if (int rc = ensure(c, c->d_pk_order, (size_t)plan.lpt_n * 4)) return rc;
        if (!c->order_stream) HIP_OK(c, hipStreamCreateWithFlags(&c->order_stream, hipStreamNonBlocking));
        if (!c->ev_cost) HIP_OK(c, hipEventCreateWithFlags(&c->ev_cost, hipEventDisableTiming));
        if (!c->ev_order) HIP_OK(c, hipEventCreateWithFlags(&c->ev_order, hipEventDisableTiming));
    }
    if (plan.overlap && !c->any_stream) HIP_OK(c, hipStreamCreateWithFlags(&c->any_stream, hipStreamNonBlocking));
    return RTX_OK;
}

static int lpt_begin(rtx_ctx * c, const RenderPlan & plan, int32_t first_tile, int32_t tile_stride, int32_t tile_count) {
    if (!plan.lpt) { c->lpt_valid = false; return RTX_OK; }
    const int32_t key[5] = { first_tile, tile_stride, tile_count, plan.levels, plan.views };
    const bool use_order = c->lpt_valid && memcmp(key, c->lpt_key, sizeof(key)) == 0;
    memcpy(c->lpt_key, key, sizeof(key));
    c->q.pk_cost = (uint32_t *)c->d_pk_cost.p;
    if (use_order) c->q.pk_lpt_order = (const uint32_t *)c->d_pk_order.p;
    if (c->lpt_valid) HIP_OK(c, hipStreamWaitEvent(c->stream, c->ev_order, 0));
    return RTX_OK;
}

template <typename F>
static void with_views(int views, F && launch) {
    if (views == RTX_CAM_RAYS) launch(std::integral_constant<int, RTX_CAM_RAYS>()); else if (views) launch(std::integral_constant<int, RTX_CAM_VIEWS>()); else launch(std::integral_constant<int, RTX_CAM_TILES>());
}

static void launch_closest(rtx_ctx * c, const RenderPlan & plan, const DevScene & sc, const DevQueues & q, int level) {
    const int kernel = plan.closest[level];
    const bool fused = kernel == CLOSEST_PACKET_FUSED || kernel == CLOSEST_PACKET_FUSED_CULL;
    launch_timed(c, fused ? "k_trace_closest_shade" : "k_trace_closest", c->stream, [&] { with_views(plan.views, [&](auto V) { constexpr int VW = decltype(V)::value;
        const dim3 plain(c->trace_blocks_count), lane(c->trace_blocks_closest), tb(RTX_TRACE_BLOCK), pk(c->pk_blocks_closest), pb(RTX_PK_BLOCK);
        switch (kernel) {
        case CLOSEST_PLAIN_COUNT:       hipLaunchKernelGGL((k_trace<false, true, VW>),  plain, tb, 0, c->stream, sc, q, level); break;
        case CLOSEST_PLAIN:             hipLaunchKernelGGL((k_trace<false, false, VW>), plain, tb, 0, c->stream, sc, q, level); break;
        case CLOSEST_LANE:              hipLaunchKernelGGL((k_trace_fast<false, VW>),   lane, tb, 0, c->stream, sc, q, level, level); break;
        case CLOSEST_PACKET_STATS:      hipLaunchKernelGGL((k_packet<false, true, false, false, false, VW>),  pk, pb, 0, c->stream, sc, q, level, level); break;
        case CLOSEST_PACKET_FUSED_CULL: hipLaunchKernelGGL((k_packet<false, false, false, true, true, VW>),   pk, pb, 0, c->stream, sc, q, level, level); break;
        case CLOSEST_PACKET_FUSED:      hipLaunchKernelGGL((k_packet<false, false, false, true, false, VW>),  pk, pb, 0, c->stream, sc, q, level, level); break;
        default:                        hipLaunchKernelGGL((k_packet<false, false, false, false, false, VW>), pk, pb, 0, c->stream, sc, q, level, level); break;
        }
    }); });
}

static void launch_shade(rtx_ctx * c, const RenderPlan & plan, const DevScene & sc, const DevQueues & q, const DevAov & aov_t, int level) {
    if (plan.shade[level] == SHADE_NONE) return;
    launch_timed(c, "k_shade", c->stream, [&] { with_views(plan.views, [&](auto V) { constexpr int VW = decltype(V)::value;
        const dim3 g(plan_level_blocks(q.primary_slots, level, plan.shade_blocks)), b(RTX_SHADE_BLOCK);
        switch (plan.shade[level]) {
        case SHADE_AOV_COUNT: hipLaunchKernelGGL((k_shade<true, false, VW, true, DevAov>),  g, b, 0, c->stream, sc, q, level, aov_t); break;
        case SHADE_AOV_CULL:  hipLaunchKernelGGL((k_shade<false, true, VW, true, DevAov>),  g, b, 0, c->stream, sc, q, level, aov_t); break;
        case SHADE_AOV:       hipLaunchKernelGGL((k_shade<false, false, VW, true, DevAov>), g, b, 0, c->stream, sc, q, level, aov_t); break;
        case SHADE_COUNT:     hipLaunchKernelGGL((k_shade<true, false, VW>),  g, b, 0, c->stream, sc, q, level); break;
        case SHADE_CULL:      hipLaunchKernelGGL((k_shade<false, true, VW>),  g, b, 0, c->stream, sc, q, level); break;
        default:              hipLaunchKernelGGL((k_shade<false, false, VW>), g, b, 0, c->stream, sc, q, level); break;
        }
    }); });
}

static void launch_any(rtx_ctx * c, const AnyLaunch & a, const DevScene & sc, const DevQueues & q) {
    const hipStream_t st = a.stream ? c->any_stream : c->stream;
    const dim3 plain(c->trace_blocks_count), lane(c->trace_blocks_any), tb(RTX_TRACE_BLOCK), pk(c->pk_blocks_any), pb(RTX_PK_BLOCK);
    launch_timed(c, "k_trace_any", st, [&] {
        switch (a.kernel) {
        case ANY_PLAIN_COUNT:   hipLaunchKernelGGL((k_trace<true, true>),   plain, tb, 0, st, sc, q, a.lo); break;
        case ANY_PLAIN:         hipLaunchKernelGGL((k_trace<true, false>),  plain, tb, 0, st, sc, q, a.lo); break;
        case ANY_LANE:          hipLaunchKernelGGL((k_trace_fast<true>),    lane, tb, 0, st, sc, q, a.lo, a.hi); break;
        case ANY_PACKET_STATS:  hipLaunchKernelGGL((k_packet<true, true>),  pk, pb, 0, st, sc, q, a.lo, a.hi); break;
        case ANY_PACKET_SPLIT:  hipLaunchKernelGGL((k_packet<true, false, true>), pk, pb, 0, st, sc, q, a.lo, a.hi); break;
        default:                hipLaunchKernelGGL((k_packet<true, false>), pk, pb, 0, st, sc, q, a.lo, a.hi); break;
        }
    });
    if (a.items) launch_timed(c, "k_trace_items", st, [&] { hipLaunchKernelGGL(k_items, dim3(c->item_blocks), dim3(RTX_ITEM_BLOCK), 0, st, sc, q, c->pk_blocks_any * (RTX_PK_BLOCK / RTX_WAVE), a.lo); });
}

static int run_batch(rtx_ctx * c, const RenderPlan & plan, const DevScene & sc, const DevQueues & q, const DevAov & aov_t, bool first_batch) {
    begin_batch(c, q.counters, q.pk_heads, (uint32_t)q.primary_slots, plan.plain != 0, first_batch);
    if (plan.heatmap) {
        launch_closest(c, plan, sc, q, 0);
        launch_timed(c, "k_heatmap", c->stream, [&] { with_views(plan.views, [&](auto V) { if constexpr (decltype(V)::value != RTX_CAM_RAYS) hipLaunchKernelGGL((k_heatmap<decltype(V)::value>), dim3(plan.stream_blocks), dim3(256), 0, c->stream, sc, q); }); });
        return RTX_OK;
    }
    int next_any = 0;
    for (int level = 0; level < plan.levels; level++) {
        launch_closest(c, plan, sc, q, level);
        if (plan.lpt && level == 0) {
            HIP_OK(c, hipEventRecord(c->ev_cost, c->stream)); HIP_OK(c, hipStreamWaitEvent(c->order_stream, c->ev_cost, 0));
            hipLaunchKernelGGL(k_packet_order, dim3(1), dim3(1024), 0, c->order_stream, (const uint32_t *)c->d_pk_cost.p, (uint32_t *)c->d_pk_order.p, plan.lpt_n);
            HIP_OK(c, hipEventRecord(c->ev_order, c->order_stream));
            c->lpt_valid = true;
        }
        launch_shade(c, plan, sc, q, aov_t, level);
        bool joined = false;
        for (; next_any < plan.n_any && plan.any[next_any].after_level == level; next_any++) {
            if (plan.any[next_any].stream && !joined) {
                const hipEvent_t ev = level == 0 ? c->ev_shade0 : c->ev_shade_last;
                HIP_OK(c, hipEventRecord(ev, c->stream)); HIP_OK(c, hipStreamWaitEvent(c->any_stream, ev, 0));
                joined = true;
            }
            launch_any(c, plan.any[next_any], sc, q);
        }
    }
    if (plan.overlap) { HIP_OK(c, hipEventRecord(c->ev_any_done, c->any_stream)); HIP_OK(c, hipStreamWaitEvent(c->stream, c->ev_any_done, 0)); }
    for (int level = plan.levels - 1; level >= 0; level--)
        launch_timed(c, "k_resolve", c->stream, [&] { with_views(plan.views, [&](auto V) {
            hipLaunchKernelGGL((k_resolve<decltype(V)::value>), dim3(plan_level_blocks(q.primary_slots, level, plan.stream_blocks) * (256 / plan.resolve_block)), dim3(plan.resolve_block), 0, c->stream, sc, q, level); }); });
    return RTX_OK;
}

static std::vector<unsigned char> graph_key_of(const rtx_ctx * c, const RenderPlan & plan, int32_t first_tile, int32_t tile_stride, int32_t tile_count, const uint32_t * tile_major, const DevAov & aov_t) {
    const int32_t range[3] = { first_tile, tile_stride, tile_count };
    const struct { const void * p; size_t n; } parts[] = { { &c->scene, sizeof(DevScene) }, { &c->q, sizeof(DevQueues) }, { &plan, sizeof(plan) }, { range, sizeof(range) }, { &tile_major, sizeof(tile_major) }, { &aov_t, sizeof(aov_t) } };
    std::vector<unsigned char> key;
    for (const auto & part : parts) key.insert(key.end(), (const unsigned char *)part.p, (const unsigned char *)part.p + part.n);
    return key;
}

static int graph_finish(rtx_ctx * c, int rc) {
    hipGraph_t g = nullptr;
    const hipError_t ce = hipStreamEndCapture(c->stream, &g);
    hipError_t ie = hipSuccess;
    if (!rc && ce == hipSuccess && g) ie = hipGraphInstantiate(&c->graph_exec, g, nullptr, nullptr, 0);
    if (g) hipGraphDestroy(g);
    if (rc || ce != hipSuccess || !g || ie != hipSuccess) {
        hipGetLastError(); c->graph_exec = nullptr; c->graph_key.clear();
        if (!rc) c->err = (ce != hipSuccess || !g) ? "hipGraph capture failed" : "hipGraphInstantiate failed";
        return rc ? rc : RTX_ERR_HIP;
    }
    HIP_OK(c, hipGraphLaunch(c->graph_exec, c->stream));
    return RTX_OK;
}

static int render_tiles_impl(rtx_ctx * c, int32_t first_tile, int32_t tile_stride, int32_t tile_count, uint32_t flags, uint32_t * tile_major, int views) {
// ... 1229 lines not shown
```

### cpu-raytracer_amd/csrc/rtx_device.h

```cpp
#pragma once
#include <hip/hip_runtime.h>
#include <stdint.h>
#include "../../include/rtx.h"
#include "rtx_limits.h"

typedef float rtx_f4v __attribute__((ext_vector_type(4)));
typedef const __attribute__((address_space(1))) rtx_f4v * rtx_gptr;
#define RTX_GPTR(p) ((rtx_gptr)(const void *)(p))
static __device__ __forceinline__ float4 gld(rtx_gptr p, int i) { const rtx_f4v v = p[i]; return make_float4(v.x, v.y, v.z, v.w); }
typedef float rtx_f3v __attribute__((ext_vector_type(3)));
static __device__ __forceinline__ float3 gld3(rtx_gptr p, int i) {
    const rtx_f3v v = *(const __attribute__((address_space(1))) rtx_f3v *)(p + i);
    return make_float3(v.x, v.y, v.z);
}

#define RTX_TRI_STRIDE  4
#ifndef RTX_LDS_STACK
#define RTX_LDS_STACK    16
#endif
#define RTX_TRACE_BLOCK  256

#define PRIM_NONE     0
#define PRIM_TRI      (1 << 28)
#define PRIM_SPHERE   (2 << 28)
#define PRIM_PLANE    (3 << 28)
#define PRIM_KIND(p)  ((p) & (3 << 28))
#define PRIM_INDEX(p) ((p) & ((1 << 28) - 1))

#define NF_HIT      1
#define NF_LIT      2
#define NF_REFL     4
#define NF_REFR     8
#define NF_TIR      16
#define NF_ENTER    32
#define RAY_DEAD_PIXEL (-1)
#define NF_CLIP     64

struct DevBlas {
    const float4 *            nodes;
    const float4 *            pk_nodes;
    const float4 *            tri_hot;
    const rtx_triangle_cold * tri_cold;
    const float4 *            pk4_nodes;
    const float4 *            pk4c_nodes;
    const float *             planes[3];
    int32_t node_count, tri_count, material_offset, pk4_need, pk4c_need, plane_count[3];
};

struct DevTexture {
    rtx_texture_desc desc;
    const float4 *   texels;
};

struct DevCounters {
    uint32_t ray_count[RTX_MAX_LEVELS + 1];
    uint32_t item_max[RTX_MAX_LEVELS + 1];
    uint32_t fetch_closest[RTX_MAX_LEVELS + 1];
    uint32_t fetch_any[RTX_MAX_LEVELS + 1];
    uint32_t error_flags;
    uint32_t pad[3];
    unsigned long long stats[4];
    unsigned long long work[20];
};

#define ERR_STACK_OVERFLOW 1u
#define ERR_QUEUE_OVERFLOW 2u

enum { W_CLOSEST_RAYS, W_ANY_RAYS, W_TLAS_C, W_TLAS_A, W_BLAS_C, W_BLAS_A, W_INST_C, W_INST_A, W_TRI_C, W_TRI_A,
       W_TRI_HITS, W_SHADED, W_SKY, W_TEXELS, W_SPAWNED };

struct DevScene {
    int32_t width, height, bounces, stack_size;
    int32_t traversal_strategy, texture_mode, mip_filter, diff_enabled;
    int32_t heatmap;
    float   max_anisotropy;
    int32_t tile_count_x;
    float cam_pos[3], cam_tl[3], cam_x[3], cam_y[3];
    float ambient[3];

    const DevBlas *       blas;       int32_t blas_count;
    const rtx_material *  materials;  int32_t material_count;
    const DevTexture *    textures;   int32_t texture_count;
    const float *         sky;        int32_t sky_size;
    const float *         ewa_table;

    const float4 *        tlas_nodes;   int32_t tlas_node_count;
    const float4 *        pk_tlas_nodes;
    const int32_t *       tlas_indices; int32_t tlas_index_count;
    const rtx_instance *  instances;    int32_t instance_count;
    const rtx_sphere *    spheres;      int32_t sphere_count;
    const rtx_plane *     planes;       int32_t plane_count;
    const rtx_point_light *       point_lights; int32_t point_light_count;
    const rtx_spot_light *        spot_lights;  int32_t spot_light_count;
    const rtx_directional_light * dir_lights;   int32_t dir_light_count;
    int32_t light_count;
};

struct DevQueues {
    int32_t level_base[RTX_MAX_LEVELS + 1];
    int32_t level_cap[RTX_MAX_LEVELS + 1];
    int32_t shadow_base[RTX_MAX_LEVELS + 1];
    int32_t first_tile, tile_stride, tile_count, primary_slots;

    float4 * r0;
    float4 * r1;
    float4 * r2;
    float4 * r3;
    float4 * r4;
    float4 *  h0;
    int32_t * h1;
    float4 * n0;
    float4 * n1;
    float4 * n2;
    const rtx_camera * views;
    float4 * c0;
    float4 * c1;
    float4 *   sp;
    float4 *   sn;
    uint32_t * socc;
    float4 *   s0;
    float4 *   s1;
    int32_t    shadow_explicit;
    int32_t    cull;

    int32_t *     spill;
    int32_t       spill_threads;
    int32_t *     pk_fifo;
    int32_t       prof_level;
    int32_t       pk_order;
    int32_t       pk_defer_grow;
    int32_t       pk_closest_asm;
    int32_t       pk_defer_t0_primary;
    int32_t       pk_defer_t0_closest;
    int32_t       pk_defer_t0;
    int32_t       pk_defer_leaf;
    int32_t       pk_item_cap;
    uint4 *       pk_items;
    uint32_t *    pk_item_count;
    DevCounters * counters;
    uint32_t *    stats_partial;
    int32_t       stats_stride;
    int32_t       stats_n[RTX_MAX_LEVELS + 1];
    uint32_t *       pk_cost;
    const uint32_t * pk_lpt_order;
    uint32_t *    pk_heads;
    uint32_t *    tm_packed;
    int32_t       tm_base;
    float *       fb_rgb;
    uint32_t *    fb_packed;
};
```

### cpu-raytracer_amd/csrc/rtx_packet.h

```cpp
#pragma once
#include "rtx_math.h"
#include "rtx_device.h"
#include "rtx_trace.h"
#include "rtx_shade.h"

#define RTX_PK_CLASSES  8
#ifndef RTX_PK_WAVES_ANY
#define RTX_PK_WAVES_ANY 5
#endif
#ifndef RTX_PK_WAVES_SPLIT
#define RTX_PK_WAVES_SPLIT 5
#endif
#ifndef RTX_PK_WAVES_CLOSEST
#define RTX_PK_WAVES_CLOSEST 4
#endif
#ifndef RTX_PK_CHUNK
#define RTX_PK_CHUNK 64u
#endif
#ifndef RTX_PK_WAVES_FUSED
#define RTX_PK_WAVES_FUSED 3
#endif

typedef const __attribute__((address_space(4))) rtx_f4v * rtx_cptr;
typedef float rtx_f2v __attribute__((ext_vector_type(2)));
RTX_D int rfl(int v) { return __builtin_amdgcn_readfirstlane(v); }
RTX_D unsigned long long rfl64(unsigned long long v) { return ((unsigned long long)(uint32_t)rfl((int)(uint32_t)(v >> 32)) << 32) | (unsigned long long)(uint32_t)rfl((int)(uint32_t)v); }
RTX_D rtx_cptr pk_cptr(const void * p) {
    const unsigned long long a = (unsigned long long)p;
    const unsigned long long u = ((unsigned long long)(uint32_t)rfl((int)(uint32_t)(a >> 32)) << 32) | (unsigned long long)(uint32_t)rfl((int)(uint32_t)a);
    return (rtx_cptr)u;
}
RTX_D float4 sld(rtx_cptr p, int i) { const rtx_f4v v = p[i]; return make_float4(v.x, v.y, v.z, v.w); }

RTX_D float pk_min(float a, float b) { float r; asm("v_min_f32 %0, %1, %2" : "=v"(r) : "v"(a), "v"(b)); return r; }
RTX_D float pk_max(float a, float b) { float r; asm("v_max_f32 %0, %1, %2" : "=v"(r) : "v"(a), "v"(b)); return r; }
RTX_D float pk_min3(float a, float b, float c) { float r; asm("v_min3_f32 %0, %1, %2, %3" : "=v"(r) : "v"(a), "v"(b), "v"(c)); return r; }
RTX_D float pk_max3(float a, float b, float c) { float r; asm("v_max3_f32 %0, %1, %2, %3" : "=v"(r) : "v"(a), "v"(b), "v"(c)); return r; }
RTX_D float pk_max_s(float s, float b) { float r; asm("v_max_f32 %0, %1, %2" : "=v"(r) : "s"(s), "v"(b)); return r; }

#define PK_FLAG_ITER      0x40000000
#define PK_FLAG_PRETESTED 0x20000000

enum { PKS_PACKETS, PKS_PAIR_STEPS, PKS_TRI_STEPS, PKS_PAIR_LANES, PKS_TRI_LANES };

struct PkRay {
    rtx_f2v o_xy, o_zz, i_xy, i_zz;
    v3 d;
    float tcur;
};
RTX_D void pk_set_ray(PkRay & r, v3 o, v3 d, v3 inv) {
    r.o_xy = rtx_f2v{ o.x, o.y }; r.o_zz = rtx_f2v{ o.z, o.z };
    r.i_xy = rtx_f2v{ inv.x, inv.y }; r.i_zz = rtx_f2v{ inv.z, inv.z };
    r.d = d;
}

template <bool FAST>
RTX_D bool pk_slab(float4 q0, float4 q1, const PkRay & r) {
    const rtx_f2v t0xy = (rtx_f2v{ q0.x, q0.y } - r.o_xy) * r.i_xy;
    const rtx_f2v t1xy = (rtx_f2v{ q0.z, q0.w } - r.o_xy) * r.i_xy;
    const rtx_f2v tz   = (rtx_f2v{ q1.x, q1.y } - r.o_zz) * r.i_zz;
    if (FAST) {
        const float t_near = pk_max_s(RAY_EPSILON, pk_max3(pk_min(t0xy.x, t1xy.x), pk_min(t0xy.y, t1xy.y), pk_min(tz.x, tz.y)));
        const float t_far  = pk_min(r.tcur, pk_min3(pk_max(t0xy.x, t1xy.x), pk_max(t0xy.y, t1xy.y), pk_max(tz.x, tz.y)));
        return t_near < t_far;
    }
    const float tminx = fmin_ref(t0xy.x, t1xy.x), tminy = fmin_ref(t0xy.y, t1xy.y), tminz = fmin_ref(tz.x, tz.y);
    const float tmaxx = fmax_ref(t0xy.x, t1xy.x), tmaxy = fmax_ref(t0xy.y, t1xy.y), tmaxz = fmax_ref(tz.x, tz.y);
    const float t_near = fmax_ref(fmax_ref(RAY_EPSILON, tminx), fmax_ref(tminy, tminz));
    const float t_far  = fmin_ref(fmin_ref(r.tcur, tmaxx), fmin_ref(tmaxy, tmaxz));
    return t_near < t_far;
}

struct Pk4Step { int e1, e2, e3; bool q1, q2, q3; bool have_cur; int cur_first, cur_cnt; };
RTX_D Pk4Step pk4_step(rtx_gptr nodes4, const int first, const PkRay & ray) {
    const int base = 4 * first;
    const float4 a0 = gld(nodes4, base), a1 = gld(nodes4, base + 1), b0 = gld(nodes4, base + 2), b1 = gld(nodes4, base + 3);
    const float4 c0 = gld(nodes4, base + 4), c1 = gld(nodes4, base + 5), d0 = gld(nodes4, base + 6), d1 = gld(nodes4, base + 7);
    const bool p0 = pk_slab<true>(a0, a1, ray), p1 = pk_slab<true>(b0, b1, ray), p2 = pk_slab<true>(c0, c1, ray), p3 = pk_slab<true>(d0, d1, ray);
    Pk4Step r;
    r.e1 = rtxl::wide_pack((uint32_t)as_i(b1.z), (uint32_t)as_i(b1.w)); r.q1 = p1 & p0;
    r.e2 = rtxl::wide_pack((uint32_t)as_i(c1.z), (uint32_t)as_i(c1.w)); r.q2 = p2 & (p0 | p1);
    r.e3 = rtxl::wide_pack((uint32_t)as_i(d1.z), (uint32_t)as_i(d1.w)); r.q3 = p3 & (p0 | p1 | p2);
    r.have_cur = p0 | p1 | p2 | p3;
    r.cur_first = p0 ? as_i(a1.z) : (p1 ? as_i(b1.z) : (p2 ? as_i(c1.z) : as_i(d1.z)));
    r.cur_cnt   = p0 ? as_i(a1.w) : (p1 ? as_i(b1.w) : (p2 ? as_i(c1.w) : as_i(d1.w)));
    return r;
}

#ifdef RTX_PK_PROF
#define PK_T0() const unsigned long long pk_t0_ = __builtin_amdgcn_s_memtime()
#define PK_T1(slot) do { W.prof[slot] += __builtin_amdgcn_s_memtime() - pk_t0_; W.prof[slot + 5]++; } while (0)
#else
#define PK_T0() do {} while (0)
#define PK_T1(slot) do {} while (0)
#endif
struct PkWalk {
    rtx_cptr tlas, nodes, tris;
    rtx_gptr lane_nodes, lane_nodes4c, lane_tris;
    int sp, floor_sp, cur_inst, depth;
    int cur_idx, cur_first, cur_cnt;
    unsigned long long m, alive;
    int st_a, st_b, st_mlo, st_mhi, st_idx, st_df;
    PkRay ray;
    bool valid, occluded;
    int best_prim, best_tri; float best_u, best_v;
    unsigned long long pub;
    int fifo_n;
    int psp;
    int pk_steps;
    int item_n, cur_blas; uint32_t item_slot;
    uint32_t err;
    unsigned long long st_pairs, st_tris, st_pair_lanes, st_tri_lanes;
#ifdef RTX_PK_PROF
    unsigned long long prof[10];
#endif
#ifdef RTX_LANE_PROF
    uint32_t lp[16];
#endif
};

extern "C" __device__ int rtx_writelane(int value, int lane, int old) __asm("llvm.amdgcn.writelane.i32");

template <bool ANY>
RTX_D void pk_push(PkWalk & W, int a, int b, unsigned long long mask, int idx, int df) {
    if (W.sp >= RTX_PK_STACK) { W.err = 1; return; }
    W.st_a   = rtx_writelane(a, W.sp, W.st_a);
    W.st_b   = rtx_writelane(b, W.sp, W.st_b);
    W.st_mlo = rtx_writelane((int)(uint32_t)mask, W.sp, W.st_mlo);
    W.st_mhi = rtx_writelane((int)(uint32_t)(mask >> 32), W.sp, W.st_mhi);
    W.st_df  = rtx_writelane(df, W.sp, W.st_df);
    if (!ANY) W.st_idx = rtx_writelane(idx, W.sp, W.st_idx);
    W.sp++;
}

#define PK_ASM_SLAB(X0, X1, X2, X3, X4, X5, MASK)                                                                                   \
    "v_pk_add_f32 v[24:25], s[" #X0 ":" #X1 "], %[oxy] neg_lo:[0,1] neg_hi:[0,1]\n\t"                                              \
    "v_pk_add_f32 v[26:27], s[" #X2 ":" #X3 "], %[oxy] neg_lo:[0,1] neg_hi:[0,1]\n\t"                                              \
    "v_pk_add_f32 v[28:29], s[" #X4 ":" #X5 "], %[ozz] neg_lo:[0,1] neg_hi:[0,1]\n\t"                                              \
    "v_pk_mul_f32 v[24:25], %[ixy], v[24:25]\n\t"                                                                                   \
    "v_pk_mul_f32 v[26:27], %[ixy], v[26:27]\n\t"                                                                                   \
    "v_pk_mul_f32 v[28:29], %[izz], v[28:29]\n\t"                                                                                   \
    "v_min_f32 v30, v24, v26\n\t"                                                                                                   \
    "v_max_f32 v24, v24, v26\n\t"                                                                                                   \
    "v_min_f32 v31, v25, v27\n\t"                                                                                                   \
    "v_max_f32 v25, v25, v27\n\t"                                                                                                   \
    "v_min_f32 v26, v28, v29\n\t"                                                                                                   \
    "v_max_f32 v27, v28, v29\n\t"                                                                                                   \
    "v_max3_f32 v30, v30, v31, v26\n\t"                                                                                             \
    "v_min3_f32 v24, v24, v25, v27\n\t"                                                                                             \
    "v_max_f32 v30, %[eps], v30\n\t"                                                                                                \
    "v_min_f32 v24, %[tcur], v24\n\t"                                                                                               \
    "v_cmp_lt_f32 vcc, v30, v24\n\t"                                                                                                \
    "s_and_b64 " MASK ", vcc, %[m]\n\t"

#define PK_ASM_SLAB_S(X0, X1, X2, X3, X4, X5, MASK, NX, FX, NY, FY, NZ, FZ)                                                          \
    "v_pk_add_f32 v[24:25], s[" #X0 ":" #X1 "], %[oxy] neg_lo:[0,1] neg_hi:[0,1]\n\t"                                              \
    "v_pk_add_f32 v[26:27], s[" #X2 ":" #X3 "], %[oxy] neg_lo:[0,1] neg_hi:[0,1]\n\t"                                              \
    "v_pk_add_f32 v[28:29], s[" #X4 ":" #X5 "], %[ozz] neg_lo:[0,1] neg_hi:[0,1]\n\t"                                              \
    "v_pk_mul_f32 v[24:25], %[ixy], v[24:25]\n\t"                                                                                   \
    "v_pk_mul_f32 v[26:27], %[ixy], v[26:27]\n\t"                                                                                   \
    "v_pk_mul_f32 v[28:29], %[izz], v[28:29]\n\t"                                                                                   \
    "v_max3_f32 v30, " NX ", " NY ", " NZ "\n\t"                                                                                    \
    "v_min3_f32 v31, " FX ", " FY ", " FZ "\n\t"                                                                                    \
    "v_max_f32 v30, %[eps], v30\n\t"                                                                                                \
    "v_min_f32 v31, %[tcur], v31\n\t"                                                                                               \
    "v_cmp_lt_f32 vcc, v30, v31\n\t"                                                                                                \
    "s_and_b64 " MASK ", vcc, %[m]\n\t"
#define PK_ASM_QUAD_S(NX, FX, NY, FY, NZ, FZ)                                                                                       \
    PK_ASM_SLAB_S(48, 49, 50, 51, 52, 53, "s[80:81]", NX, FX, NY, FY, NZ, FZ)                                                       \
    PK_ASM_SLAB_S(56, 57, 58, 59, 60, 61, "s[82:83]", NX, FX, NY, FY, NZ, FZ)                                                       \
    PK_ASM_SLAB_S(64, 65, 66, 67, 68, 69, "s[84:85]", NX, FX, NY, FY, NZ, FZ)                                                       \
    PK_ASM_SLAB_S(72, 73, 74, 75, 76, 77, "s[86:87]", NX, FX, NY, FY, NZ, FZ)                                                       \
    "s_branch PKB_SEL_%=\n\t"

template <bool ANY>
RTX_D void pk_descend(PkWalk & W, int stack_size, int ordered, int thr) {
    W.cur_first = rfl(W.cur_first); W.cur_cnt = rfl(W.cur_cnt); W.cur_idx = rfl(W.cur_idx); W.m = rfl64(W.m); W.sp = rfl(W.sp);
    W.depth = rfl(W.depth); W.err = (uint32_t)rfl((int)W.err); stack_size = rfl(stack_size); ordered = rfl(ordered); thr = rfl(thr);
    int steps = rfl(W.pk_steps);
    const unsigned long long posx = __ballot(W.ray.d.x > 0.0f), posy = __ballot(W.ray.d.y > 0.0f), posz = __ballot(W.ray.d.z > 0.0f);
    const float eps = RAY_EPSILON;
    const unsigned long long nodes = rfl64((unsigned long long)W.nodes);
    if (ANY) {
        asm volatile(
            "s_mov_b64 s[94:95], %[nodes]\n\t"
            "PKA_TOP_%=:\n\t"
            "s_add_i32 s90, %[depth], 2\n\t"
            "s_cmp_gt_i32 s90, %[ssz]\n\t"
            "s_cselect_b32 %[err], 1, %[err]\n\t"
            "s_mov_b32 s92, %[first]\n\t"
            "s_mov_b32 s93, 0\n\t"
            "s_lshl_b64 s[92:93], s[92:93], 5\n\t"
            "s_add_u32 s92, s92, s94\n\t"
            "s_addc_u32 s93, s93, s95\n\t"
            "s_load_dwordx16 s[64:79], s[92:93], 0x0\n\t"
            "s_lshr_b32 s90, %[cnt], 30\n\t"
            "s_mov_b64 s[86:87], %[posx]\n\t"
            "s_cmp_eq_u32 s90, 2\n\t"
            "s_cselect_b64 s[86:87], %[posy], s[86:87]\n\t"
            "s_cmp_eq_u32 s90, 3\n\t"
            "s_cselect_b64 s[86:87], %[posz], s[86:87]\n\t"
            "s_ff1_i32_b64 s91, %[m]\n\t"
            "s_bitcmp1_b64 s[86:87], s91\n\t"
            "s_cselect_b32 s91, 1, 0\n\t"
            "s_cmp_eq_u32 s90, 0\n\t"
            "s_cselect_b32 s91, 1, s91\n\t"
            "s_cmp_eq_u32 %[ordered], 0\n\t"
            "s_cselect_b32 s91, 1, s91\n\t"
            "s_waitcnt lgkmcnt(0)\n\t"
            PK_ASM_SLAB(64, 65, 66, 67, 68, 69, "s[82:83]")
            PK_ASM_SLAB(72, 73, 74, 75, 76, 77, "s[84:85]")
            "s_cmp_lg_u32 s91, 0\n\t"
            "s_cselect_b64 s[86:87], s[82:83], s[84:85]\n\t"
            "s_cselect_b64 s[88:89], s[84:85], s[82:83]\n\t"
            "s_cselect_b32 s80, s70, s78\n\t"
            "s_cselect_b32 s81, s71, s79\n\t"
            "s_cselect_b32 s92, s78, s70\n\t"
            "s_cselect_b32 s93, s79, s71\n\t"
            "s_cmp_eq_u64 s[86:87], 0\n\t"
            "s_cbranch_scc1 PKA_NONEAR_%=\n\t"
            "s_cmp_eq_u64 s[88:89], 0\n\t"
            "s_cbranch_scc1 PKA_NOFAR_%=\n\t"
            "s_cmp_ge_i32 %[sp], 64\n\t"
            "s_cbranch_scc1 PKA_OVER_%=\n\t"
            "s_mov_b32 m0, %[sp]\n\t"
            "s_nop 0\n\t"
            "v_writelane_b32 %[sta], s92, m0\n\t"
            "v_writelane_b32 %[stb], s93, m0\n\t"
            "v_writelane_b32 %[stmlo], s88, m0\n\t"
            "v_writelane_b32 %[stmhi], s89, m0\n\t"
            "v_writelane_b32 %[stdf], %[depth], m0\n\t"
            "s_add_i32 %[sp], %[sp], 1\n\t"
            "PKA_NOFAR_%=:\n\t"
            "s_mov_b32 %[first], s80\n\t"
            "s_mov_b32 %[cnt], s81\n\t"
            "s_mov_b64 %[m], s[86:87]\n\t"
            "s_add_i32 %[depth], %[depth], 1\n\t"
            "s_branch PKA_CHECK_%=\n\t"
            "PKA_OVER_%=:\n\t"
            "s_mov_b32 %[err], 1\n\t"
            "s_branch PKA_NOFAR_%=\n\t"
            "PKA_NONEAR_%=:\n\t"
            "s_mov_b32 %[first], s92\n\t"
            "s_mov_b32 %[cnt], s93\n\t"
            "s_mov_b64 %[m], s[88:89]\n\t"
            "s_cmp_eq_u64 s[88:89], 0\n\t"
            "s_cbranch_scc1 PKA_END_%=\n\t"
            "PKA_CHECK_%=:\n\t"
            "s_and_b32 s90, %[cnt], 0x3fffffff\n\t"
            "s_cmp_eq_u32 s90, 0\n\t"
// ... 969 lines not shown
        "s_add_i32 s99, %[first], s88\n\t"
        "PKC_TRI_%=:\n\t"
        "s_lshl_b32 s89, s98, 6\n\t"
        "s_load_dwordx8 s[64:71], s[96:97], s89\n\t"
        "s_add_u32 s89, s89, 32\n\t"
        "s_load_dwordx4 s[72:75], s[96:97], s89\n\t"
        "s_waitcnt lgkmcnt(0)\n\t"
        "v_mul_f32 %[t0], s74, %[dy]\n\t"
        "v_mul_f32 %[t1], s73, %[dz]\n\t"
        "v_mul_f32 %[t2], s72, %[dz]\n\t"
        "v_mul_f32 %[t3], s74, %[dx]\n\t"
        "v_mul_f32 %[t4], s73, %[dx]\n\t"
        "v_mul_f32 %[t5], s72, %[dy]\n\t"
        "v_sub_f32 v24, %[t0], %[t1]\n\t"
        "v_sub_f32 v25, %[t2], %[t3]\n\t"
        "v_sub_f32 v26, %[t4], %[t5]\n\t"
        "v_mul_f32 %[t0], s69, v25\n\t"
        "v_mul_f32 %[t1], s70, v26\n\t"
        "v_mul_f32 %[t2], s68, v24\n\t"
        "v_add_f32 %[t0], %[t0], %[t1]\n\t"
        "v_add_f32 %[t9], %[t2], %[t0]\n\t"
        "v_div_scale_f32 %[t0], s[84:85], %[t9], %[t9], 1.0\n\t"
        "v_rcp_f32 %[t1], %[t0]\n\t"
        "v_div_scale_f32 %[t2], vcc, 1.0, %[t9], 1.0\n\t"
        "v_subrev_f32 v27, s64, %[ox]\n\t"
        "v_fma_f32 %[t3], -%[t0], %[t1], 1.0\n\t"
        "v_fmac_f32 %[t1], %[t3], %[t1]\n\t"
        "v_mul_f32 %[t4], %[t2], %[t1]\n\t"
        "v_fma_f32 %[t5], -%[t0], %[t4], %[t2]\n\t"
        "v_fmac_f32 %[t4], %[t5], %[t1]\n\t"
        "v_fma_f32 %[t0], -%[t0], %[t4], %[t2]\n\t"
        "v_subrev_f32 v28, s65, %[oy]\n\t"
        "v_div_fmas_f32 %[t0], %[t0], %[t1], %[t4]\n\t"
        "v_subrev_f32 v29, s66, %[oz]\n\t"
        "v_div_fixup_f32 %[t8], %[t0], %[t9], 1.0\n\t"
        "v_mul_f32 %[t0], v28, v25\n\t"
        "v_mul_f32 %[t1], v29, v26\n\t"
        "v_mul_f32 %[t2], v27, v24\n\t"
        "v_add_f32 %[t0], %[t0], %[t1]\n\t"
        "v_add_f32 %[t0], %[t2], %[t0]\n\t"
        "v_mul_f32 %[t7], %[t8], %[t0]\n\t"
        "v_cmp_lt_f32 s[84:85], 0, %[t7]\n\t"
        "v_cmp_gt_f32 s[86:87], 1.0, %[t7]\n\t"
        "s_and_b64 s[84:85], s[84:85], s[86:87]\n\t"
        "s_and_b64 s[84:85], s[84:85], %[m]\n\t"
        "s_cmp_lg_u64 s[84:85], 0\n\t"
        "s_cbranch_scc0 PKC_NEXT_%=\n\t"
        "v_mul_f32 %[t0], s70, v28\n\t"
        "v_mul_f32 %[t1], s69, v29\n\t"
        "v_mul_f32 %[t2], s68, v29\n\t"
        "v_mul_f32 %[t3], s70, v27\n\t"
        "v_mul_f32 %[t4], s69, v27\n\t"
        "v_mul_f32 %[t5], s68, v28\n\t"
        "v_sub_f32 v24, %[t0], %[t1]\n\t"
        "v_sub_f32 v25, %[t2], %[t3]\n\t"
        "v_sub_f32 v26, %[t4], %[t5]\n\t"
        "v_mul_f32 %[t0], %[dy], v25\n\t"
        "v_mul_f32 %[t1], %[dz], v26\n\t"
        "v_mul_f32 %[t2], %[dx], v24\n\t"
        "v_add_f32 %[t0], %[t0], %[t1]\n\t"
        "v_add_f32 %[t0], %[t2], %[t0]\n\t"
        "v_mul_f32 %[t6], %[t8], %[t0]\n\t"
        "v_mul_f32 %[t0], s73, v25\n\t"
        "v_mul_f32 %[t1], s74, v26\n\t"
        "v_mul_f32 %[t2], s72, v24\n\t"
        "v_add_f32 %[t0], %[t0], %[t1]\n\t"
        "v_add_f32 %[t0], %[t2], %[t0]\n\t"
        "v_mul_f32 %[t5], %[t8], %[t0]\n\t"
        "v_add_f32 %[t4], %[t7], %[t6]\n\t"
        "v_cmp_lt_f32 s[86:87], 0, %[t6]\n\t"
        "s_and_b64 s[84:85], s[84:85], s[86:87]\n\t"
        "v_cmp_gt_f32 s[86:87], 1.0, %[t4]\n\t"
        "s_and_b64 s[84:85], s[84:85], s[86:87]\n\t"
        "v_cmp_lt_f32 s[86:87], %[eps], %[t5]\n\t"
        "s_and_b64 s[84:85], s[84:85], s[86:87]\n\t"
        "v_cmp_lt_f32 s[86:87], %[t5], %[tcur]\n\t"
        "s_and_b64 s[84:85], s[84:85], s[86:87]\n\t"
        "s_cmp_lg_u64 s[84:85], 0\n\t"
        "s_cbranch_scc0 PKC_NEXT_%=\n\t"
        "s_mov_b64 s[92:93], exec\n\t"
        "s_mov_b64 exec, s[84:85]\n\t"
        "v_mov_b32 %[tcur], %[t5]\n\t"
        "v_mov_b32 %[bu], %[t7]\n\t"
        "v_mov_b32 %[bv], %[t6]\n\t"
        "v_mov_b32 %[btri], s98\n\t"
        "v_mov_b32 %[bprim], %[prim]\n\t"
        "s_mov_b64 exec, s[92:93]\n\t"
        "PKC_NEXT_%=:\n\t"
        "s_add_i32 s98, s98, 1\n\t"
        "s_cmp_lt_i32 s98, s99\n\t"
        "s_cbranch_scc1 PKC_TRI_%=\n\t"
        "PKC_POP_%=:\n\t"
        "s_mov_b64 %[m], 0\n\t"
        "s_cmp_le_i32 %[sp], %[floor]\n\t"
        "s_cbranch_scc1 PKC_END_%=\n\t"
        "s_sub_i32 %[sp], %[sp], 1\n\t"
        "s_mov_b32 m0, %[sp]\n\t"
        "s_nop 0\n\t"
        "v_readlane_b32 s84, %[stmlo], m0\n\t"
        "v_readlane_b32 s85, %[stmhi], m0\n\t"
        "v_readlane_b32 %[first], %[sta], m0\n\t"
        "v_readlane_b32 %[cnt], %[stb], m0\n\t"
        "v_readlane_b32 s91, %[stdf], m0\n\t"
        "v_readlane_b32 %[idx], %[stidx], m0\n\t"
        "s_and_b32 %[depth], s91, 0xffff\n\t"
        "s_bitcmp1_b32 s91, 29\n\t"
        "s_cbranch_scc0 PKC_FAR_%=\n\t"
        "s_andn2_b64 s[86:87], s[84:85], %[pub]\n\t"
        "s_cmp_lg_u64 s[86:87], 0\n\t"
        "s_cbranch_scc0 PKC_PRE_PUB_%=\n\t"
        PK_ASM_REF
        PK_ASM_FIFO_APPEND("s86", "s87", "0xff800000")
        "PKC_PRE_PUB_%=:\n\t"
        "s_and_b64 %[m], s[84:85], %[pub]\n\t"
        "s_cmp_eq_u64 %[m], 0\n\t"
        "s_cbranch_scc1 PKC_POP_%=\n\t"
        "s_branch PKC_DISPATCH_%=\n\t"
        "PKC_FAR_%=:\n\t"
        "s_mov_b64 %[m], s[84:85]\n\t"
        "s_lshl_b32 s88, %[idx], 5\n\t"
        "s_load_dwordx8 s[64:71], s[94:95], s88\n\t"
        "s_waitcnt lgkmcnt(0)\n\t"
        PK_ASM_SLAB(64, 65, 66, 67, 68, 69, "s[80:81]")
        "s_andn2_b64 s[86:87], s[80:81], %[pub]\n\t"
        "s_cmp_lg_u64 s[86:87], 0\n\t"
        "s_cbranch_scc0 PKC_FAR_PUB_%=\n\t"
        PK_ASM_REF
        PK_ASM_FIFO_APPEND("s86", "s87", "v30")
        "PKC_FAR_PUB_%=:\n\t"
        "s_and_b64 %[m], s[80:81], %[pub]\n\t"
        "s_cmp_eq_u64 %[m], 0\n\t"
        "s_cbranch_scc1 PKC_POP_%=\n\t"
        "s_branch PKC_DISPATCH_%=\n\t"
        "PKC_END_%=:\n\t"
        : [first] "+&s"(W.cur_first), [cnt] "+&s"(W.cur_cnt), [idx] "+&s"(W.cur_idx), [m] "+&s"(W.m), [sp] "+&s"(W.sp), [depth] "+&s"(W.depth),
          [err] "+&s"(err), [steps] "+&s"(steps), [pub] "+&s"(W.pub),
          [sta] "+&v"(W.st_a), [stb] "+&v"(W.st_b), [stmlo] "+&v"(W.st_mlo), [stmhi] "+&v"(W.st_mhi), [stdf] "+&v"(W.st_df), [stidx] "+&v"(W.st_idx),
          [tcur] "+&v"(W.ray.tcur), [bu] "+&v"(W.best_u), [bv] "+&v"(W.best_v), [btri] "+&v"(W.best_tri), [bprim] "+&v"(W.best_prim),
          [fvoff] "+&v"(fvoff), [fn] "+&v"(W.fifo_n),
          [t0] "=&v"(t0), [t1] "=&v"(t1), [t2] "=&v"(t2), [t3] "=&v"(t3), [t4] "=&v"(t4), [t5] "=&v"(t5), [t6] "=&v"(t6), [t7] "=&v"(t7),
          [t8] "=&v"(t8), [t9] "=&v"(t9)
        : [nodes] "s"(nodes), [tris] "s"(tris), [floor] "s"(floor_sp), [ssz] "s"(ssz), [eps] "s"(eps), [ordered] "s"(ord), [t0d] "s"(t0d), [gsh] "s"(gsh),
          [posx] "s"(posx), [posy] "s"(posy), [posz] "s"(posz), [fbase] "s"(fbase), [fstride] "s"(fstride), [prim] "s"(primv), [fifomax] "s"((int)RTX_PK_FIFO),
          [oxy] "v"(W.ray.o_xy), [ozz] "v"(W.ray.o_zz), [ixy] "v"(W.ray.i_xy), [izz] "v"(W.ray.i_zz),
          [ox] "v"(W.ray.o_xy.x), [oy] "v"(W.ray.o_xy.y), [oz] "v"(W.ray.o_zz.x), [dx] "v"(W.ray.d.x), [dy] "v"(W.ray.d.y), [dz] "v"(W.ray.d.z)
        : "vcc", "scc", "m0", "memory",
          "s64", "s65", "s66", "s67", "s68", "s69", "s70", "s71", "s72", "s73", "s74", "s75", "s76", "s77", "s78", "s79",
          "s80", "s81", "s82", "s83", "s84", "s85", "s86", "s87", "s88", "s89", "s90", "s91", "s92", "s93", "s94", "s95", "s96", "s97", "s98", "s99",
          "v24", "v25", "v26", "v27", "v28", "v29", "v30", "v31");
    W.pk_steps = steps;
    if (err) W.err = 1;
}

template <bool ANY, bool PSTAT, bool FAST, bool ASM, bool SPLIT, typename WorldFn>
RTX_D bool pk_walk(const DevScene & sc, PkWalk & W, const int lane, const bool ordered, const PkHybrid & H, WorldFn && world) {
    for (;;) {
        if (W.m != 0ull) {
            if (!ANY && ASM && FAST && W.floor_sp >= 0) {
                const int thr = H.t0 + (W.pk_steps >> H.grow);
                if (__popcll(W.m) <= thr && (W.sp - W.floor_sp) + 2 <= RTX_PK_FIFO) {
                    if ((W.m >> lane) & 1ull) { H.fifo[W.fifo_n * H.fifo_stride] = make_int2(W.cur_idx, as_i(PK_KEY_PASSED)); W.fifo_n++; }
                    W.pub &= ~W.m; W.m = 0ull;
                    continue;
                }
                W.pk_steps++;
            }
            const int leafc = W.cur_cnt & 0x3fffffff;
            if (leafc > 0) {
                PK_T0();
                if (W.floor_sp >= 0) {
                    const v3 co = V3(W.ray.o_xy.x, W.ray.o_xy.y, W.ray.o_zz.x), cd = W.ray.d;
                    for (int i = W.cur_first; i < W.cur_first + leafc; i++) {
                        const float4 p0 = sld(W.tris, RTX_TRI_STRIDE * i), e1 = sld(W.tris, RTX_TRI_STRIDE * i + 1), e2 = sld(W.tris, RTX_TRI_STRIDE * i + 2);
                        if (PSTAT) { W.st_tris++; W.st_tri_lanes += (unsigned long long)__popcll(W.m); }
                        float t, u, v;
                        const bool hit = tri_test_all(v3q(p0), v3q(e1), v3q(e2), co, cd, W.ray.tcur, t, u, v);
                        const unsigned long long hm = __ballot(hit) & W.m;
                        if (hm != 0ull) {
                            const bool mine = (hm >> lane) & 1ull;
                            if (ANY) { if (mine) W.occluded = true; W.alive &= ~hm; W.m &= ~hm; if (W.m == 0ull) break; }
                            else if (mine) { W.ray.tcur = t; W.best_u = u; W.best_v = v; W.best_tri = i; W.best_prim = PRIM_TRI | W.cur_inst; }
                        }
                    }
                } else {
                    pk_push<ANY>(W, W.cur_first, leafc, W.m, 0, PK_FLAG_ITER);
                }
                W.m = 0ull;
                PK_T1(2);
            } else if (ASM && FAST) {
                PK_T0();
                pk_descend<ANY>(W, sc.stack_size, ordered ? 1 : 0, (!ANY && W.floor_sp >= 0) ? H.t0 + (W.pk_steps >> H.grow) : -1);
                PK_T1(1);
            } else {
                if (W.depth + 2 > sc.stack_size) W.err = 1;
                int left_first = 1;
                if (ordered) {
                    const int axis = (int)((uint32_t)W.cur_cnt >> 30);
                    if (axis != 0) {
                        const float c = axis == 1 ? W.ray.d.x : (axis == 2 ? W.ray.d.y : W.ray.d.z);
                        const unsigned long long pos = __ballot(c > 0.0f) & W.m;
                        if (ANY) left_first = (int)((pos >> (__ffsll((long long)W.m) - 1)) & 1ull);
                        else if (pos == 0ull) left_first = 0;
                        else if (pos != W.m) {
                            pk_push<ANY>(W, W.cur_first, W.cur_cnt, W.m & ~pos, W.cur_idx, W.depth | PK_FLAG_PRETESTED);
                            W.m = pos;
                        }
                    }
                }
                left_first = rfl(left_first);
                const int left = W.cur_first;
                const float4 la = sld(W.nodes, 2 * left), lb = sld(W.nodes, 2 * left + 1), ra = sld(W.nodes, 2 * left + 2), rb = sld(W.nodes, 2 * left + 3);
                if (PSTAT) { W.st_pairs++; W.st_pair_lanes += (unsigned long long)__popcll(W.m); }
                const unsigned long long ml = __ballot(pk_slab<FAST>(la, lb, W.ray)) & W.m, mr = __ballot(pk_slab<FAST>(ra, rb, W.ray)) & W.m;
                const unsigned long long m_near = left_first ? ml : mr, m_far = left_first ? mr : ml;
                const int near_idx = left_first ? left : left + 1, far_idx = left_first ? left + 1 : left;
                const int near_first = left_first ? as_i(lb.z) : as_i(rb.z), near_cnt = left_first ? as_i(lb.w) : as_i(rb.w);
                const int far_first  = left_first ? as_i(rb.z) : as_i(lb.z), far_cnt  = left_first ? as_i(rb.w) : as_i(lb.w);
                if (m_near != 0ull) {
                    if (m_far != 0ull) pk_push<ANY>(W, far_first, far_cnt, m_far, far_idx, W.depth);
                    W.cur_idx = rfl(near_idx); W.cur_first = rfl(near_first); W.cur_cnt = rfl(near_cnt); W.m = m_near; W.depth = rfl(W.depth + 1);
                } else if (m_far != 0ull) {
                    W.cur_idx = rfl(far_idx); W.cur_first = rfl(far_first); W.cur_cnt = rfl(far_cnt); W.m = m_far;
                } else W.m = 0ull;
            }
            continue;
        }
        PK_T0();
        if (ANY && W.alive == 0ull) return true;
        if (W.floor_sp >= 0 && W.sp == W.floor_sp) {
            if (!ANY && ASM && FAST && W.pub != W.alive) {
                if (W.lane_nodes4c) pk_lane_phase_closest<true>(W, lane, ordered, H, W.lane_nodes, W.lane_nodes4c, W.lane_tris);
                else pk_lane_phase_closest<false>(W, lane, ordered, H, W.lane_nodes, nullptr, W.lane_tris);
                W.pub = W.alive;
            }
            if (W.sp == 0) return true;
            W.floor_sp = -1; W.nodes = W.tlas;
            v3 o, d; world(o, d);
            pk_set_ray(W.ray, o, d, vrcp(d));
        }
        if (W.sp == 0) return true;
        W.sp--;
        const int ea = __builtin_amdgcn_readlane(W.st_a, W.sp), eb = __builtin_amdgcn_readlane(W.st_b, W.sp);
        const int edf = __builtin_amdgcn_readlane(W.st_df, W.sp);
        const unsigned long long em = ((unsigned long long)(uint32_t)__builtin_amdgcn_readlane(W.st_mhi, W.sp) << 32) |
                                      (unsigned long long)(uint32_t)__builtin_amdgcn_readlane(W.st_mlo, W.sp);
        unsigned long long pm = em & W.alive;
        if (!ANY && ASM && FAST && (pm & ~W.pub) != 0ull) {
            if (((pm & ~W.pub) >> lane) & 1ull) {
                H.fifo[W.fifo_n * H.fifo_stride] = make_int2(__builtin_amdgcn_readlane(W.st_idx, W.sp), (edf & PK_FLAG_PRETESTED) ? as_i(PK_KEY_PASSED) : 0x7fc00000); W.fifo_n++;
            }
            pm &= W.pub;
        }
        if (pm == 0ull) continue;
        if (edf & PK_FLAG_ITER) {
            if (eb > 1) pk_push<ANY>(W, ea + 1, eb - 1, pm, 0, PK_FLAG_ITER);
            const int inst = rfl(sc.tlas_indices[ea]);
            const rtx_instance & I = sc.instances[inst];
            v3 o, d; world(o, d);
            const v3 co = xform_pos(I.world_inv, o), cd = xform_dir(I.world_inv, d), cinv = vrcp(cd);
            pk_set_ray(W.ray, co, cd, cinv);
            W.cur_blas = rfl(I.blas_id);
            const DevBlas & B = sc.blas[W.cur_blas];
            W.nodes = pk_cptr(B.pk_nodes); W.tris = pk_cptr(B.tri_hot); W.cur_inst = inst;
            W.lane_nodes = RTX_GPTR(B.nodes); W.lane_tris = RTX_GPTR(B.tri_hot); if (!ANY) W.lane_nodes4c = RTX_GPTR(B.pk4c_nodes);
            W.floor_sp = W.sp; W.depth = 0;
            const float4 na = sld(W.nodes, 0), nb = sld(W.nodes, 1);
            const bool risky = FAST && __ballot(W.valid && !inv_is_finite(cinv) && pk_nan_possible(B, co, cinv)) != 0ull;
            W.m = (risky ? __ballot(pk_slab<false>(na, nb, W.ray)) : __ballot(pk_slab<FAST>(na, nb, W.ray))) & pm;
            W.cur_idx = 0; W.cur_first = as_i(nb.z); W.cur_cnt = as_i(nb.w);
            if (risky) return false;
            if (ASM && FAST && !ANY && H.closest_asm) {
#ifdef RTX_LANE_PROF
                asm volatile("s_waitcnt vmcnt(0) lgkmcnt(0)" ::: "memory"); const unsigned long long sw_t0 = __builtin_amdgcn_s_memtime(); const int sw_s0 = W.pk_steps;
#endif
#ifdef RTX_PK_SKIPWALK
                W.m = 0ull;
#else
                pk_blas_closest_asm(W, sc.stack_size, ordered ? 1 : 0, H, PRIM_TRI | inst, H.gthread);
#endif
#ifdef RTX_LANE_PROF
                asm volatile("s_waitcnt vmcnt(0) lgkmcnt(0)" ::: "memory");
                W.lp[13] = (uint32_t)rfl((int)(W.lp[13] + (uint32_t)(__builtin_amdgcn_s_memtime() - sw_t0))); W.lp[14] = (uint32_t)rfl((int)(W.lp[14] + (uint32_t)(W.pk_steps - sw_s0)));
                W.lp[15] = (uint32_t)rfl((int)(W.lp[15] + 1u));
#endif
            }
            if (ASM && FAST && ANY) {
                PK_T0();
                W.psp = 0;
                if (SPLIT) {
#ifdef RTX_PK_SKIPWALK
                    W.m = 0ull;
#else
                    pk_blas_any_asm4(W, pk_cptr(B.pk4_nodes), H.lane_lds, H.t0, H.t_leaf, H.grow, H.item_cap, H.item_base, W.item_slot);
#endif
                    PK_T1(1);
                } else if (B.pk4_nodes) {
                    pk_blas_any_asm4(W, pk_cptr(B.pk4_nodes), H.lane_lds, H.t0, H.t_leaf, H.grow, 0u, 0ull, 0u);
                    PK_T1(1);
                    if (W.alive != 0ull && __ballot(W.psp > 0) != 0ull) { PK_T0(); pk_lane_phase_any4(W, lane, H.lane_lds, H.spill, H.spill_stride, RTX_GPTR(B.pk4_nodes), RTX_GPTR(B.tri_hot)); PK_T1(2); }
                } else {
                    pk_blas_any_asm(W, sc.stack_size, H.lane_lds, H.t0, H.grow);
                    PK_T1(1);
                    if (W.alive != 0ull && __ballot(W.psp > 0) != 0ull) { PK_T0(); pk_lane_phase_any(W, lane, H.stk, H.spill, H.spill_stride, RTX_GPTR(B.nodes), RTX_GPTR(B.tri_hot)); PK_T1(2); }
                }
            }
        } else {
            W.m = pm;
            if (!ANY && !(edf & PK_FLAG_PRETESTED)) {
                const int eidx = __builtin_amdgcn_readlane(W.st_idx, W.sp);
                const float4 na = sld(W.nodes, 2 * eidx), nb = sld(W.nodes, 2 * eidx + 1);
                W.m = __ballot(pk_slab<FAST>(na, nb, W.ray)) & pm;
                W.cur_idx = eidx;
            } else if (!ANY) W.cur_idx = __builtin_amdgcn_readlane(W.st_idx, W.sp);
            W.cur_first = rfl(ea); W.cur_cnt = rfl(eb); W.depth = rfl(edf & 0xffff);
        }
        PK_T1(3);
    }
}

template <bool ANY, bool PSTAT, bool SPLIT = false, bool FUSE = false, bool CULL = false, int VIEWS = 0>
__global__ __launch_bounds__(RTX_PK_BLOCK, ANY ? (SPLIT ? RTX_PK_WAVES_SPLIT : RTX_PK_WAVES_ANY) : (FUSE ? RTX_PK_WAVES_FUSED : RTX_PK_WAVES_CLOSEST))
void k_packet(const DevScene sc, const DevQueues q, const int level, const int level_hi) {
    __shared__ int s_priv[RTX_PK_BLOCK / RTX_WAVE][SPLIT ? 1 : (ANY ? RTX_PK_PRIV : 2 * RTX_LDS_STACK)][RTX_WAVE];
    const int lane = threadIdx.x & 63;
    PkHybrid H;
    H.stk = &s_priv[threadIdx.x >> 6][0][lane];
    H.stk_key = (float *)&s_priv[threadIdx.x >> 6][(ANY || SPLIT) ? 0 : RTX_LDS_STACK][lane];
    H.lane_lds = (uint32_t)(uintptr_t)H.stk;
    H.spill_stride = q.spill_threads;
    {
        const size_t region = (size_t)q.spill_threads * (RTX_MAX_STACK - RTX_LDS_STACK), gt = blockIdx.x * blockDim.x + threadIdx.x;
        H.spill = q.spill + (ANY ? 2 * region : 0) + gt;
        H.spill_key = (float *)(q.spill + region) + gt;
        H.fifo = (int2 *)q.pk_fifo + gt; H.fifo_stride = q.spill_threads; H.gthread = (uint32_t)gt;
    }
    H.closest_asm = q.pk_closest_asm;
    H.t0 = ANY ? q.pk_defer_t0 : (level == 0 ? q.pk_defer_t0_primary : q.pk_defer_t0_closest); H.t_leaf = q.pk_defer_leaf; H.grow = q.pk_defer_grow;
    H.item_cap = 0; H.item_base = 0ull;
    const uint32_t gwave  = (uint32_t)rfl((int)(blockIdx.x * (RTX_PK_BLOCK / RTX_WAVE) + (threadIdx.x >> 6)));
    const uint32_t nwaves = gridDim.x * (RTX_PK_BLOCK / RTX_WAVE);

    if (ANY && SPLIT && q.pk_items) { H.item_cap = (uint32_t)q.pk_item_cap; H.item_base = (unsigned long long)(q.pk_items + 3 * (size_t)gwave * (size_t)q.pk_item_cap); }
    DevCounters * const ctr = q.counters;
    const int nL = sc.light_count;
    uint32_t npk = 0;
    if (ANY) { for (int d = level; d <= level_hi; d++) npk += ((shadow_slots(ctr, q, d) + 63u) >> 6) * (uint32_t)nL; }
    else npk = (ctr->ray_count[level] + 63u) >> 6;
    npk = (uint32_t)rfl((int)npk);
    uint32_t * const heads = q.pk_heads + (size_t)((ANY ? RTX_MAX_LEVELS + 1 : 0) + level) * RTX_PK_CLASSES * 32;
    const bool ordered = sc.traversal_strategy == RTX_TRAVERSE_ORDERED;

    PkWalk W;
#ifdef RTX_PK_PROF
    for (int i = 0; i < 10; i++) W.prof[i] = 0ull;
    const unsigned long long pk_k0_ = __builtin_amdgcn_s_memtime();
#endif
#ifdef RTX_LANE_PROF
    for (int i = 0; i < 16; i++) W.lp[i] = 0u;
    const unsigned long long lp_k0 = __builtin_amdgcn_s_memtime(), lp_r0 = __builtin_amdgcn_s_memrealtime(); bool lp_had_packet = false;
#endif
    W.tlas = pk_cptr(sc.pk_tlas_nodes);
    W.err = 0; W.st_pairs = W.st_tris = W.st_pair_lanes = W.st_tri_lanes = 0ull; W.item_n = 0; W.item_slot = 0; W.cur_blas = 0;
    W.st_a = W.st_b = W.st_mlo = W.st_mhi = W.st_idx = W.st_df = 0;
    unsigned long long st_packets = 0ull;
    ShadeTally tally = { 0, 0, 0, 0, 0, 0, 0, 0 };
    uint32_t chunk_next = 0, chunk_end = 0;
    auto wave_alloc2 = [&](bool want_a, bool want_b, uint32_t * counter, uint32_t & slot_a, uint32_t & slot_b) {
        const unsigned long long ma = __ballot(want_a), mb = __ballot(want_b);
        const uint32_t ca = (uint32_t)__popcll(ma), need = ca + (uint32_t)__popcll(mb);
        if (need == 0u) { slot_a = slot_b = 0u; return; }
        const uint32_t avail = chunk_end - chunk_next, first_base = chunk_next, first_n = need < avail ? need : avail;
        uint32_t second_base = 0;
        if (need > avail) {
            const uint32_t want = need - avail, grab = (want + RTX_PK_CHUNK - 1u) / RTX_PK_CHUNK * RTX_PK_CHUNK;
            if (lane == 0) second_base = atomicAdd(counter, grab);
            second_base = (uint32_t)rfl((int)second_base);
            chunk_next = second_base + want; chunk_end = second_base + grab;
        } else chunk_next += need;
        const uint32_t rank_a = (uint32_t)__popcll(ma & ((1ull << lane) - 1ull)), rank_b = ca + (uint32_t)__popcll(mb & ((1ull << lane) - 1ull));
        slot_a = rank_a < first_n ? first_base + rank_a : second_base + (rank_a - first_n);
        slot_b = rank_b < first_n ? first_base + rank_b : second_base + (rank_b - first_n);
    };
    uint32_t cls = gwave & (RTX_PK_CLASSES - 1);
    int probes_left = 2;
    bool first_round = true;
    const bool all_static = nwaves >= npk;

    for (;;) {
        PK_T0();
        uint32_t pk;
        if (first_round) { first_round = false; pk = gwave; if (pk >= npk) break; }
        else {
            if (all_static) break;
            bool got = false;
            while (probes_left > 0) {
                uint32_t k = 0;
                if (lane == 0) k = atomicAdd(&heads[cls * 32], 1u);
                k = (uint32_t)rfl((int)k);
                pk = k * RTX_PK_CLASSES + cls;
                if (pk < npk) { got = true; break; }
                cls = (cls + 1) & (RTX_PK_CLASSES - 1); probes_left--;
            }
            if (!got) break;
        }

#ifdef RTX_LANE_PROF
        lp_had_packet = true;
#endif
        const unsigned long long pk_t_start = (!ANY && level == 0 && q.pk_cost) ? __builtin_amdgcn_s_memtime() : 0ull;
        if (!ANY && level == 0 && q.pk_lpt_order) pk = (uint32_t)rfl((int)q.pk_lpt_order[pk]);
        if (ANY && q.pk_order != 0) pk = npk - 1u - pk;
        W.valid = false; W.occluded = false;
        uint32_t out_slot = 0;
        v3 wo = V3(0.0f, 0.0f, 0.0f), wd = V3(1.0f, 1.0f, 1.0f);
        W.ray.tcur = INFINITY;
        W.best_prim = PRIM_NONE; W.best_tri = 0; W.best_u = 0.0f; W.best_v = 0.0f;
        bool clipped = false;
        uint32_t pix_idx = 0;
        int any_level = 0, any_light = 0; uint32_t any_rank = 0;
        if (ANY) {
            uint32_t local = pk; int d = level;
            uint32_t lit_n = shadow_slots(ctr, q, d), seg = (lit_n + 63u) >> 6;
            while (d < level_hi && local >= seg * (uint32_t)nL) { local -= seg * (uint32_t)nL; d++; lit_n = shadow_slots(ctr, q, d); seg = (lit_n + 63u) >> 6; }
            uint32_t light = 0; while (local >= seg && light + 1u < (uint32_t)nL) { local -= seg; light++; }
            const uint32_t rank = local * 64u + (uint32_t)lane;
            W.valid = rank < lit_n && shadow_slot_is_lit(q, d, rank);
            any_level = d; any_light = (int)light; any_rank = rank;
            if (W.valid) {
                out_slot = (uint32_t)q.shadow_base[d] + light * (uint32_t)q.level_cap[d] + rank;
                load_shadow_ray(sc, q, d, (int)light, rank, out_slot, wo, wd, W.ray.tcur);
                if (W.ray.tcur < 0.0f) W.valid = false;
            }
        } else {
            pix_idx = pk * 64u + (uint32_t)lane;
            W.valid = pix_idx < ctr->ray_count[level];
            if (W.valid) {
                out_slot = (uint32_t)q.level_base[level] + pix_idx;
                if (level == 0) {
                    int px, py, view;
                    if (primary_pixel_v<VIEWS, true>(sc, q, pix_idx, px, py, view)) {
                        RayFull r; primary_ray_v<VIEWS>(sc, q, view, px, py, r, false); wo = r.o; wd = r.d;
                        if (VIEWS == RTX_CAM_RAYS && !ray_is_finite(wo, wd)) W.occluded = true;
                    }
                    else { clipped = true; W.valid = false; }
                } else {
                    v3 o, d;
                    if (queued_ray(q, out_slot, o, d)) { wo = o; wd = d; }
                    else { clipped = true; W.valid = false; }
                }
            }
        }
        auto world = [&](v3 & o, v3 & d) {
            o = V3(0.0f, 0.0f, 0.0f); d = V3(1.0f, 1.0f, 1.0f);
            if (!W.valid) return;
            if (ANY) { float tm; load_shadow_ray(sc, q, any_level, any_light, any_rank, out_slot, o, d, tm); }
            else if (level == 0) { int px, py, view; primary_pixel_v<VIEWS, true>(sc, q, pix_idx, px, py, view); RayFull r; primary_ray_v<VIEWS>(sc, q, view, px, py, r, false); o = r.o; d = r.d; }
            else queued_ray(q, out_slot, o, d);
        };
        if (W.valid && world_primitives<ANY>(sc, wo, wd, W.ray.tcur, W.best_prim)) W.occluded = true;
        W.psp = 0; W.pk_steps = 0; W.fifo_n = 0; W.item_slot = out_slot;
        W.alive = __ballot(W.valid && !W.occluded);
        const unsigned long long alive0 = W.alive;
        W.pub = W.alive;
        if (PSTAT) st_packets++;

        if (W.alive != 0ull && sc.tlas_node_count > 0) {
            const v3 winv = vrcp(wd);
            pk_set_ray(W.ray, wo, wd, winv);
            const bool nanfree_world = __ballot(W.valid && !inv_is_finite(winv) && pk_nan_possible_tlas(sc, wo, winv)) == 0ull;
            W.nodes = W.tlas; W.tris = W.tlas;
            W.sp = 0; W.floor_sp = -1; W.cur_inst = 0; W.depth = 0; W.cur_idx = 0;
            {
                const float4 na = sld(W.nodes, 0), nb = sld(W.nodes, 1);
                W.m = (nanfree_world ? __ballot(pk_slab<true>(na, nb, W.ray)) : __ballot(pk_slab<false>(na, nb, W.ray))) & W.alive;
                W.cur_first = as_i(nb.z); W.cur_cnt = as_i(nb.w);
            }
            PK_T1(0);
#ifdef RTX_PK_PROF
            const unsigned long long pk_w0_ = __builtin_amdgcn_s_memtime();
#endif
            bool done = false;
            if (nanfree_world && !done) done = pk_walk<ANY, PSTAT, true, !PSTAT, SPLIT>(sc, W, lane, ordered, H, world);
            if (!done) pk_walk<ANY, PSTAT, false, false, SPLIT>(sc, W, lane, ordered, H, world);
#ifdef RTX_PK_PROF
            {
                const unsigned long long dt = __builtin_amdgcn_s_memtime() - pk_w0_;
                if (dt > W.prof[4]) W.prof[4] = dt;
            }
#endif
        }

        if (ANY) { if (((alive0 & ~W.alive) >> lane) & 1ull) W.occluded = true; }
        if (ANY) { if (W.valid) q.socc[out_slot] = W.occluded ? 1u : 0u; }
        else if (FUSE) {
            const bool in_range = W.valid || clipped;
#ifdef RTX_LANE_PROF
            asm volatile("s_waitcnt vmcnt(0) lgkmcnt(0)" ::: "memory"); const unsigned long long sp_t0 = __builtin_amdgcn_s_memtime();
#endif
            shade_ray<false, CULL, VIEWS>(sc, q, level, pix_idx, in_range, W.valid, make_float4(W.ray.tcur, W.best_u, W.best_v, as_f(W.best_prim)),
                                   clipped ? -1 : W.best_tri, wave_alloc2, tally);
#ifdef RTX_LANE_PROF
            asm volatile("s_waitcnt vmcnt(0) lgkmcnt(0)" ::: "memory");
            W.lp[13] = (uint32_t)rfl((int)(W.lp[13] + (uint32_t)(__builtin_amdgcn_s_memtime() - sp_t0))); W.lp[14] = (uint32_t)rfl((int)(W.lp[14] + 1u));
#endif
        }
        else if (W.valid) { q.h0[out_slot] = make_float4(W.ray.tcur, W.best_u, W.best_v, as_f(W.best_prim)); q.h1[out_slot] = W.best_tri; }
        else if (clipped) { q.h0[out_slot] = make_float4(INFINITY, 0.0f, 0.0f, as_f(PRIM_NONE)); q.h1[out_slot] = -1; }
        if (!ANY && level == 0 && q.pk_cost && lane == 0) q.pk_cost[pk] = (uint32_t)((__builtin_amdgcn_s_memtime() - pk_t_start) >> 6);
    }
    if (!ANY && FUSE && chunk_next < chunk_end) {
        const uint32_t dead = chunk_next + (uint32_t)lane;
        if (dead < chunk_end && dead < (uint32_t)q.level_cap[level + 1])
            q.r1[(uint32_t)q.level_base[level + 1] + dead] = make_float4(0.0f, 0.0f, as_f(RAY_DEAD_PIXEL), as_f(-1));
    }
    if (!ANY && FUSE && lane < 4) {
        const uint32_t v = lane == 0 ? tally.n_primary : (lane == 1 ? tally.n_shadow : (lane == 2 ? tally.n_refl : tally.n_refr));
        q.stats_partial[((size_t)level * q.stats_stride + gwave) * 4 + lane] = v;
    }

#ifdef RTX_PK_PROF
    W.prof[6] = __builtin_amdgcn_s_memtime() - pk_k0_;
    W.prof[7] = __builtin_amdgcn_s_memtime();
    W.prof[8] = (1ull << 62) - pk_k0_;
    if (lane == 0) for (int i = 0; i < 10; i++) { if (i == 4 || i == 5 || i == 7 || i == 8 || i == 9) atomicMax(&ctr->work[(ANY ? 0 : 10) + i], W.prof[i]); else atomicAdd(&ctr->work[(ANY ? 0 : 10) + i], W.prof[i]); }
#endif
#ifdef RTX_LANE_PROF
    if (!ANY && level == q.prof_level % 100 && lane == 0 && (W.lp[12] > 0u || (q.prof_level >= 100 && lp_had_packet))) {
        for (int i = 0; i < 10; i++) atomicAdd(&ctr->work[i], (unsigned long long)W.lp[i]);
        atomicMax(&ctr->work[10], (unsigned long long)W.lp[10]); atomicMax(&ctr->work[11], (unsigned long long)W.lp[11]); atomicAdd(&ctr->work[12], (unsigned long long)W.lp[12]);
        atomicMax(&ctr->work[13], __builtin_amdgcn_s_memtime() - lp_k0);
        atomicAdd(&ctr->work[14], __builtin_amdgcn_s_memtime() - lp_k0);
        atomicAdd(&ctr->work[15], 1ull);
        atomicAdd(&ctr->work[16], __builtin_amdgcn_s_memrealtime() - lp_r0);
        atomicAdd(&ctr->work[17], (unsigned long long)W.lp[13]); atomicAdd(&ctr->work[18], (unsigned long long)W.lp[14]);
        atomicAdd(&ctr->work[19], (unsigned long long)W.lp[15]);
    }
#endif
    if (ANY && SPLIT && q.pk_items && lane == 0) { q.pk_item_count[gwave] = (uint32_t)W.item_n; if ((uint32_t)W.item_n > __hip_atomic_load(&ctr->item_max[level], __ATOMIC_RELAXED, __HIP_MEMORY_SCOPE_AGENT)) atomicMax(&ctr->item_max[level], (uint32_t)W.item_n); }
    if (W.err) { if (lane == 0) atomicOr(&ctr->error_flags, ERR_STACK_OVERFLOW); }
    if (PSTAT && lane == 0) {
        atomicAdd(&ctr->work[15 + PKS_PACKETS], st_packets); atomicAdd(&ctr->work[15 + PKS_PAIR_STEPS], W.st_pairs);
        atomicAdd(&ctr->work[15 + PKS_TRI_STEPS], W.st_tris); atomicAdd(&ctr->work[15 + PKS_PAIR_LANES], W.st_pair_lanes);
        atomicAdd(&ctr->work[15 + PKS_TRI_LANES], W.st_tri_lanes);
    }
}

#define RTX_ITEM_LDS 8
#ifndef RTX_ITEM_BLOCK
#define RTX_ITEM_BLOCK 64
#endif
#define RTX_ITEM_MESHES 32
#ifndef RTX_ITEM_WAVES
#define RTX_ITEM_WAVES 6
#endif
__global__ __launch_bounds__(RTX_ITEM_BLOCK, RTX_ITEM_WAVES)
void k_items(const DevScene sc, const DevQueues q, const int n_chunks, const int level) {
    __shared__ int s_stk[RTX_ITEM_LDS][RTX_ITEM_BLOCK];
    __shared__ unsigned long long s_mesh[RTX_ITEM_MESHES][2];
    for (int b = threadIdx.x; b < RTX_ITEM_MESHES && b < sc.blas_count; b += blockDim.x) { s_mesh[b][0] = (unsigned long long)sc.blas[b].pk4_nodes; s_mesh[b][1] = (unsigned long long)sc.blas[b].tri_hot; }
    __syncthreads();
    const uint32_t gwave = (uint32_t)rfl((int)(blockIdx.x * (RTX_ITEM_BLOCK / RTX_WAVE) + (threadIdx.x >> 6)));
    const uint32_t n_batches = ((uint32_t)rfl((int)q.counters->item_max[level]) + 63u) >> 6;
    const uint32_t nwaves = gridDim.x * (RTX_ITEM_BLOCK / RTX_WAVE), units = (uint32_t)n_chunks * n_batches;
    int ovf[RTX_PK4_MAX_NEED + 4];
#ifdef RTX_ITEM_STATS
    unsigned long long st_iters = 0, st_busy = 0, st_batches = 0, st_items = 0;
#endif
    uint32_t u = gwave, pos = 0, lim = 0; const uint4 * items = q.pk_items;
    auto next_unit = [&]() {
        for (; u < units; u += nwaves) {
            const uint32_t chunk = u % (uint32_t)n_chunks, first = (u / (uint32_t)n_chunks) * 64u;
            const uint32_t n = (uint32_t)rfl((int)q.pk_item_count[chunk]);
            if (first < n) { pos = first; lim = first + 64u < n ? first + 64u : n; items = q.pk_items + 3 * (size_t)chunk * (size_t)q.pk_item_cap; u += nwaves; return true; }
        }
        return false;
    };
    bool have_unit = next_unit();
    bool busy = false, have_cur = false; uint32_t slot = 0; int psp = 0, cur_first = 0, cur_cnt = 0;
    v3 co = V3(0.0f, 0.0f, 0.0f), cd = V3(1.0f, 1.0f, 1.0f);
    PkRay ray; pk_set_ray(ray, co, cd, cd); ray.tcur = 0.0f;
    rtx_gptr nodes4 = nullptr, tris = nullptr;
    auto push = [&](int e) { if (psp < RTX_ITEM_LDS) s_stk[psp][threadIdx.x] = e; else if (psp < RTX_ITEM_LDS + RTX_PK4_MAX_NEED + 4) ovf[psp - RTX_ITEM_LDS] = e; psp++; };
    for (;;) {
        const unsigned long long idle = __ballot(!busy);
        if (idle != 0ull && have_unit) {
            const uint32_t rank = (uint32_t)__builtin_amdgcn_mbcnt_hi((uint32_t)(idle >> 32), __builtin_amdgcn_mbcnt_lo((uint32_t)idle, 0u));
            const uint32_t take = (uint32_t)__popcll(idle), avail = lim - pos;
            if (!busy && rank < avail) {
                const uint4 * const it = items + 3 * (size_t)(pos + rank);
                const uint4 q0 = it[0], q1 = it[1]; const uint2 q2 = *(const uint2 *)(it + 2);
                slot = q1.w;
                if (q2.y < RTX_ITEM_MESHES) { nodes4 = (rtx_gptr)s_mesh[q2.y][0]; tris = (rtx_gptr)s_mesh[q2.y][1]; }
                else { const DevBlas & B = sc.blas[q2.y]; nodes4 = RTX_GPTR(B.pk4_nodes); tris = RTX_GPTR(B.tri_hot); }
                co = V3(as_f((int)q0.x), as_f((int)q0.y), as_f((int)q0.z)); cd = V3(as_f((int)q1.x), as_f((int)q1.y), as_f((int)q1.z));
                pk_set_ray(ray, co, cd, vrcp(cd)); ray.tcur = as_f((int)q0.w);
                cur_first = rtxl::wide_first((int)q2.x); cur_cnt = rtxl::wide_count((int)q2.x); have_cur = true; psp = 0;
                busy = q.socc[slot] == 0u;
#ifdef RTX_ITEM_STATS
                st_items++;
#endif
            }
            pos += take < avail ? take : avail;
            if (pos >= lim) have_unit = next_unit();
        }
        if (__ballot(busy) == 0ull) { if (!have_unit) break; else continue; }
#ifdef RTX_ITEM_STATS
        st_iters++; st_busy += (unsigned long long)__popcll(__ballot(busy));
#endif
        if (busy && have_cur && cur_cnt == 0) {
            const Pk4Step s = pk4_step(nodes4, cur_first, ray);
            if (s.q3) push(s.e3);
            if (s.q2) push(s.e2);
            if (s.q1) push(s.e1);
            have_cur = s.have_cur; cur_first = s.cur_first; cur_cnt = s.cur_cnt;
        }
        if (busy && have_cur && cur_cnt > 0) {
            have_cur = false;
            for (int t = cur_first; t < cur_first + cur_cnt; t++) {
                const float4 p0 = gld(tris, RTX_TRI_STRIDE * t), e1 = gld(tris, RTX_TRI_STRIDE * t + 1), e2 = gld(tris, RTX_TRI_STRIDE * t + 2);
                float tt, uu, vv;
                if (tri_test(v3q(p0), v3q(e1), v3q(e2), co, cd, ray.tcur, tt, uu, vv)) { q.socc[slot] = 1u; busy = false; break; }
            }
        }
        if (busy && !have_cur) {
            if (psp == 0) busy = false;
            else {
                psp--;
                const int e = psp < RTX_ITEM_LDS ? s_stk[psp][threadIdx.x] : ovf[psp - RTX_ITEM_LDS];
                cur_first = rtxl::wide_first(e); cur_cnt = rtxl::wide_count(e); have_cur = true;
            }
        }
    }
#ifdef RTX_ITEM_STATS
    if ((threadIdx.x & 63) == 0) { atomicAdd(&q.counters->work[16], st_iters); atomicAdd(&q.counters->work[17], st_busy); atomicMax(&q.counters->work[19], st_iters); }
    atomicAdd(&q.counters->work[15], st_items);
#endif
// ... 2 lines not shown
```

### cpu-raytracer_amd/csrc/rtx_plan.h

```cpp
#pragma once
#include <stdint.h>
#include <string.h>
#include "../../include/rtx.h"
#include "rtx_limits.h"

struct Knobs {
    long long slot_budget;
    long long item_bytes_max;
    int shade_grid;
    int lane_from_level;
    int lane_from_level_any;
    int split_items;
    int resolve_block;
    int pk4_order;
    bool merge_any, no_wide, no_wide_closest, fail_item_alloc, graph; int lpt;
    bool fuse_shade;
    int update_small_max;
    int tex_pass_levels;
};

struct StackFigures { bool unfit_mesh; int dt, blas_any, blas_shared; };

static inline bool plan_can_spawn(const rtx_material * materials, size_t count) {
    for (size_t i = 0; i < count; i++)
        for (int a = 0; a < 3; a++) if (materials[i].reflection[a] != 0.0f || materials[i].transmittance[a] != 0.0f) return true;
    return false;
}

struct PlanInputs {
    uint32_t flags; int views;
    int tile_count, batch_tiles; bool tile_major, timing;
    Knobs knobs;
    int instance_count, light_count, bounces;
    bool heatmap, can_spawn, all_wide;
    StackFigures stack;
    int n_cu, pk_blocks_closest, pk_blocks_any;
};

enum : int32_t { CLOSEST_PLAIN, CLOSEST_PLAIN_COUNT, CLOSEST_LANE, CLOSEST_PACKET_STATS, CLOSEST_PACKET, CLOSEST_PACKET_FUSED, CLOSEST_PACKET_FUSED_CULL };
enum : int32_t { SHADE_NONE, SHADE_PLAIN, SHADE_COUNT, SHADE_CULL, SHADE_AOV, SHADE_AOV_COUNT, SHADE_AOV_CULL };
enum : int32_t { ANY_PLAIN, ANY_PLAIN_COUNT, ANY_LANE, ANY_PACKET_STATS, ANY_PACKET, ANY_PACKET_SPLIT };
struct AnyLaunch { int32_t after_level, stream, kernel, lo, hi, items; };

struct RenderPlan {
    uint32_t flags; int32_t views;
    int32_t lane, pk_closest, pstat, cull, aov, serial, plain, heatmap;
    int32_t levels;
    int32_t overlap, merged;
    int32_t lane_from, lane_from_closest;
    int32_t closest[RTX_MAX_LEVELS], shade[RTX_MAX_LEVELS];
    int32_t shade_blocks, stream_blocks, resolve_block, pk_waves_closest, stats_stride;
    int32_t n_any; AnyLaunch any[RTX_MAX_LEVELS];
    int32_t split, item_cap;
    int32_t lpt; uint32_t lpt_n;
    int32_t graph_eligible;
};

static inline int plan_shared_walk_need(const StackFigures & s) {
    const int tlas_sib = s.dt > 0 ? s.dt : 0, blas_sib = s.blas_shared > 2 ? s.blas_shared / 2 - 1 : 0;
    return tlas_sib + (tlas_sib < 3 ? tlas_sib : 3) + 1 + blas_sib + (blas_sib < 3 ? blas_sib : 3);
}

static inline void plan_stack_limits(const StackFigures & s, bool & lane, bool & pk_closest) {
    if (s.unfit_mesh) lane = true;
    if (s.dt + 1 + s.blas_any > RTX_PK_STACK || 2 * s.dt + 1 > RTX_PK_STACK) lane = true;
    if (2 * s.dt + 1 + s.blas_shared > RTX_PK_STACK) pk_closest = false;
    if (plan_shared_walk_need(s) > RTX_PK_STACK) lane = true;
}

#define PLAN_LEVEL_BLOCKS_MIN 64
static inline int plan_level_blocks(int primary_slots, int level, int full) {
    const long long want = (((long long)primary_slots >> level) + 255) / 256;
    const long long most = (long long)full < want ? (long long)full : want;
    return (int)(most > PLAN_LEVEL_BLOCKS_MIN ? most : PLAN_LEVEL_BLOCKS_MIN);
}

static inline int plan_stats_n(const RenderPlan & p, int primary_slots, int level) {
    return p.shade[level] == SHADE_NONE ? p.pk_waves_closest : plan_level_blocks(primary_slots, level, p.shade_blocks);
}

static inline void plan_add_any(RenderPlan & p, bool packets, int after_level, int stream, int lo, int hi) {
    const bool count_work = (p.flags & RTX_RENDER_COUNT_WORK) != 0, simple = (p.flags & RTX_RENDER_SIMPLE_TRACE) != 0;
    const int packet_kernel = p.split ? ANY_PACKET_SPLIT : ANY_PACKET;
    if (packets && hi >= p.lane_from) {
        if (lo < p.lane_from) p.any[p.n_any++] = AnyLaunch{ after_level, stream, packet_kernel, lo, p.lane_from - 1, p.split };
        p.any[p.n_any++] = AnyLaunch{ after_level, stream, ANY_LANE, lo > p.lane_from ? lo : p.lane_from, hi, 0 };
        return;
    }
    const int kernel = count_work ? ANY_PLAIN_COUNT : simple ? ANY_PLAIN : p.lane ? ANY_LANE : p.pstat ? ANY_PACKET_STATS : packet_kernel;
    p.any[p.n_any++] = AnyLaunch{ after_level, stream, kernel, lo, hi, packets ? p.split : 0 };
}

static inline void plan_drop_split(RenderPlan & p) {
    p.split = 0; p.item_cap = 0;
    for (int i = 0; i < p.n_any; i++) { if (p.any[i].kernel == ANY_PACKET_SPLIT) p.any[i].kernel = ANY_PACKET; p.any[i].items = 0; }
}

static inline RenderPlan plan_render(const PlanInputs & in) {
    RenderPlan p; memset(&p, 0, sizeof(p));
    const Knobs & K = in.knobs;
    p.flags = in.flags; p.views = in.views;
    const bool count_work = (in.flags & RTX_RENDER_COUNT_WORK) != 0;
    const bool simple = (in.flags & RTX_RENDER_SIMPLE_TRACE) != 0;
    p.cull = (in.flags & RTX_RENDER_CULL_DEAD_SHADOW_RAYS) != 0 && !simple && !count_work;
    bool lane = (in.flags & RTX_RENDER_LANE_TRACE) != 0;
    bool pk_closest = (in.flags & RTX_RENDER_PACKET_CLOSEST) != 0;
    plan_stack_limits(in.stack, lane, pk_closest);
    p.lane = lane; p.pk_closest = pk_closest;
    p.pstat = (in.flags & RTX_RENDER_PACKET_STATS) != 0 && !simple && !count_work && !lane;
    p.aov = (in.flags & RTX_RENDER_AOV) != 0;
    p.serial = (in.flags & RTX_RENDER_SERIAL) != 0;
    p.heatmap = in.heatmap; p.plain = count_work || simple || in.heatmap;
    const bool packets = !count_work && !simple && !lane && !p.pstat;
    p.levels = in.can_spawn ? in.bounces + 1 : 1;
    p.stream_blocks = in.n_cu * 8;
    p.resolve_block = K.resolve_block;
    p.shade_blocks = in.n_cu * K.shade_grid;
    p.pk_waves_closest = in.pk_blocks_closest * (RTX_PK_BLOCK / RTX_WAVE);
    p.stats_stride = p.shade_blocks > p.pk_waves_closest ? p.shade_blocks : p.pk_waves_closest;
    if (p.stats_stride < PLAN_LEVEL_BLOCKS_MIN) p.stats_stride = PLAN_LEVEL_BLOCKS_MIN;

    if (K.split_items > 0 && in.light_count > 0 && in.all_wide) {
        const size_t chunks = (size_t)in.pk_blocks_any * (RTX_PK_BLOCK / RTX_WAVE);
        const double expect = 0.45 * 1024.0 * (double)in.batch_tiles * in.light_count / (double)chunks;
        long long cap = K.split_items;
        if (cap < (long long)(3.5 * expect)) cap = ((long long)(3.5 * expect) + 63) & ~63ll;
        const long long cap_max = (K.item_bytes_max / (long long)(chunks * 48)) & ~63ll;
        if (cap > cap_max) cap = cap_max;
        if (cap > (1 << 16)) cap = 1 << 16;
        if (cap >= 64) { p.split = 1; p.item_cap = (int32_t)cap; }
    }

    p.lpt_n = (uint32_t)in.tile_count * 16u;
    const bool lpt_want = K.lpt > 0 || (K.lpt < 0 && !p.serial && p.lpt_n >= 2u * (uint32_t)p.pk_waves_closest);
    p.lpt = lpt_want && !K.graph && in.tile_count <= in.batch_tiles && packets && !in.heatmap && !K.fuse_shade;
    p.graph_eligible = K.graph && !in.timing && in.tile_count <= in.batch_tiles;

    p.overlap = !count_work && !simple && in.light_count > 0 && !p.serial;
    p.merged = !p.overlap && !count_work && !simple && K.merge_any;

    p.lane_from = K.lane_from_level >= 0 ? K.lane_from_level : (in.instance_count > 1 ? 2 : RTX_MAX_LEVELS + 1);
    p.lane_from_closest = K.lane_from_level >= 0 ? K.lane_from_level : (in.instance_count > 64 ? 1 : p.lane_from);
    if (K.lane_from_level < 0 && K.split_items > 0 && in.light_count > 0 && in.all_wide) p.lane_from = RTX_MAX_LEVELS + 1;
    if (K.lane_from_level_any >= 0) p.lane_from = K.lane_from_level_any;

    if (in.heatmap) { p.closest[0] = count_work ? CLOSEST_PLAIN_COUNT : CLOSEST_PLAIN; return p; }

    for (int level = 0; level < p.levels; level++) {
        const bool fused = K.fuse_shade && packets && level < p.lane_from_closest && !(p.aov && level == 0);
        p.closest[level] = count_work ? CLOSEST_PLAIN_COUNT : simple ? CLOSEST_PLAIN : (lane || (!p.pstat && level >= p.lane_from_closest)) ? CLOSEST_LANE :
                           p.pstat ? CLOSEST_PACKET_STATS : fused ? (p.cull ? CLOSEST_PACKET_FUSED_CULL : CLOSEST_PACKET_FUSED) : CLOSEST_PACKET;
        const bool aov0 = p.aov && level == 0;
        p.shade[level] = fused ? SHADE_NONE : count_work ? (aov0 ? SHADE_AOV_COUNT : SHADE_COUNT) : p.cull ? (aov0 ? SHADE_AOV_CULL : SHADE_CULL) : (aov0 ? SHADE_AOV : SHADE_PLAIN);
    }
    if (in.light_count > 0) for (int level = 0; level < p.levels; level++) {
        if (p.overlap) {
            if (level == 0) plan_add_any(p, packets, 0, 1, 0, 0);
            if (level == p.levels - 1 && p.levels > 1) plan_add_any(p, packets, level, 1, 1, p.levels - 1);
        } else if (p.merged) {
            if (level == p.levels - 1) plan_add_any(p, packets, level, 0, 0, p.levels - 1);
        } else plan_add_any(p, packets, level, 0, level, level);
    }
    return p;
}
```

Measured before the change: 9587.

## Enter the single mesh directly when the TLAS holds one lone instance

Result: faster. 9937, median of 6 (+3.7%).

```diff
diff --git a/cpu-raytracer_amd/csrc/lone_check.cpp b/cpu-raytracer_amd/csrc/lone_check.cpp
--- /dev/null
+++ b/cpu-raytracer_amd/csrc/lone_check.cpp
@@ -0,0 +1,160 @@
+#include <stdio.h>
+#include <string.h>
+#include <vector>
+#include "rtx_plan.h"
+
+static int failures = 0;
+static char current[128] = "";
+#define CHECK(x) do { if (!(x)) { if (failures < 20) printf("FAILED [%s] line %d: %s\n", current, __LINE__, #x); failures++; } } while (0)
+
+static float from_bits(uint32_t u) { float f; memcpy(&f, &u, 4); return f; }
+static uint32_t bits_of(float f) { uint32_t u; memcpy(&u, &f, 4); return u; }
+
+static uint32_t rng_state = 11;
+static uint32_t rng() { rng_state = rng_state * 1664525u + 1013904223u; return rng_state >> 8; }
+
+struct v3 { float x, y, z; };
+static v3 xform_pos(const float * c, v3 d) {
+    return v3{ c[0] * d.x + (c[1] * d.y + (c[2]  * d.z + c[3])),
+               c[4] * d.x + (c[5] * d.y + (c[6]  * d.z + c[7])),
+               c[8] * d.x + (c[9] * d.y + (c[10] * d.z + c[11])) };
+}
+static v3 xform_dir(const float * c, v3 d) {
+    return v3{ c[0] * d.x + (c[1] * d.y + c[2]  * d.z),
+               c[4] * d.x + (c[5] * d.y + c[6]  * d.z),
+               c[8] * d.x + (c[9] * d.y + c[10] * d.z) };
+}
+
+static float component() {
+    static const uint32_t SPECIAL[] = { 0x00000000u, 0x80000000u, 0x00000001u, 0x80000001u, 0x007fffffu, 0x807fffffu, 0x00800000u, 0x80800000u,
+                                        0x7f7fffffu, 0xff7fffffu, 0x7f61b1e6u , 0xff61b1e6u, 0x3f800000u, 0xbf800000u };
+    const uint32_t pick = rng() % 8u;
+    if (pick < 2u) return from_bits(SPECIAL[rng() % (sizeof(SPECIAL) / sizeof(SPECIAL[0]))]);
+    if (pick == 2u) return from_bits(((rng() & 1u) << 31) | (rng() & 0x7fffffu));
+    return from_bits(((rng() & 1u) << 31) | ((1u + rng() % 254u) << 23) | (rng() & 0x7fffffu));
+}
+
+static const int OFF_DIAGONAL[9] = { 1, 2, 3, 4, 6, 7, 8, 9, 11 };
+static void class_matrix(uint32_t pattern, float m[16]) {
+    for (int k = 0; k < 16; k++) m[k] = k >= 12 ? 7.5f : 0.0f;
+    m[0] = m[5] = m[10] = 1.0f;
+    for (int k = 0; k < 9; k++) if ((pattern >> k) & 1u) m[OFF_DIAGONAL[k]] = -0.0f;
+}
+
+static LoneFacts facts(const std::vector<rtx_bvh_node> & nodes, const std::vector<int32_t> & idx, const std::vector<rtx_instance> & inst) {
+    return plan_lone_facts((int)inst.size(), nodes.data(), (int)nodes.size(), idx.data(), (int)idx.size(), inst.data());
+}
+
+static rtx_bvh_node node(int32_t left_or_first, int32_t count) {
+    rtx_bvh_node n; memset(&n, 0, sizeof(n));
+    for (int a = 0; a < 3; a++) { n.aabb_min[a] = -1.0f; n.aabb_max[a] = 1.0f; }
+    n.left_or_first = left_or_first; n.count = count;
+    return n;
+}
+
+static rtx_instance instance(uint32_t pattern) {
+    rtx_instance I; memset(&I, 0, sizeof(I));
+    class_matrix(0u, I.world); class_matrix(pattern, I.world_inv);
+    return I;
+}
+
+static void check_facts() {
+    snprintf(current, sizeof(current), "facts");
+    const rtx_bvh_node garbage = node(0x7fffffff, -5);
+    {
+        const LoneFacts f = facts({ node(0, 1), garbage }, { 0 }, { instance(0u) });
+        CHECK(f.lone && f.copy_class);
+        const LoneFacts g = facts({ node(0, 1) }, { 0 }, { instance(0x1ffu) });
+        CHECK(g.lone && g.copy_class);
+        const LoneFacts h = facts({ node(0, 1), garbage }, { 0 }, { instance(0x0a5u) });
+        CHECK(h.lone && h.copy_class);
+    }
+    {
+        CHECK(!facts({ node(0, 1), garbage }, { 0 }, { instance(0u), instance(0u) }).lone);
+        CHECK(!facts({ node(2, 0), garbage, node(0, 1), node(1, 1) }, { 0, 1 }, { instance(0u), instance(0u) }).lone);
+        CHECK(!facts({ node(2, 0), garbage, node(0, 1), node(0, 1) }, { 0 }, { instance(0u) }).lone);
+        CHECK(!facts({ node(0, 2), garbage }, { 0, 0 }, { instance(0u) }).lone);
+        CHECK(!facts({ node(0, 1 | (1 << 30)), garbage }, { 0 }, { instance(0u) }).lone);
+        CHECK(!facts({ node(1, 1), garbage }, { 0, 0 }, { instance(0u) }).lone);
+        CHECK(!facts({ node(0, 1), garbage }, { 1 }, { instance(0u) }).lone);
+        CHECK(!facts({}, {}, { instance(0u) }).lone);
+        CHECK(!facts({ node(0, 1) }, {}, { instance(0u) }).lone);
+        CHECK(!facts({ node(0, 1) }, { 0 }, {}).lone);
+        CHECK(!facts({ node(0, 1), garbage }, { 0 }, { instance(0u), instance(0u) }).copy_class);
+    }
+    {
+        for (int k = 0; k < 12; k++) {
+            const bool diagonal = k == 0 || k == 5 || k == 10;
+            const uint32_t wrong[] = { diagonal ? 0x3f800001u  : 0x00000001u , diagonal ? 0x3f7fffffu : 0x80000001u,
+                                       diagonal ? 0xbf800000u  : 0x3f800000u, diagonal ? 0x00000000u : 0x7f800000u, 0x7fc00000u };
+            for (uint32_t w : wrong) {
+                rtx_instance I = instance(rng() & 0x1ffu);
+                I.world_inv[k] = from_bits(w);
+                const LoneFacts f = facts({ node(0, 1), garbage }, { 0 }, { I });
+                CHECK(f.lone && !f.copy_class);
+            }
+        }
+        rtx_instance moved = instance(0u); moved.world_inv[3] = -2.0f; moved.world[3] = 2.0f;
+        CHECK(facts({ node(0, 1), garbage }, { 0 }, { moved }).lone && !facts({ node(0, 1), garbage }, { 0 }, { moved }).copy_class);
+        rtx_instance turned = instance(0u); turned.world_inv[0] = 0.0f; turned.world_inv[2] = -1.0f; turned.world_inv[8] = 1.0f; turned.world_inv[10] = 0.0f;
+        CHECK(facts({ node(0, 1), garbage }, { 0 }, { turned }).lone && !facts({ node(0, 1), garbage }, { 0 }, { turned }).copy_class);
+    }
+    {
+        rtx_instance I = instance(0x155u);
+        for (int k = 12; k < 16; k++) I.world_inv[k] = from_bits(0x7fc00000u);
+        for (int k = 0; k < 16; k++) I.world[k] = 3.0f;
+        CHECK(facts({ node(0, 1), garbage }, { 0 }, { I }).copy_class);
+    }
+}
+
+static long vectors = 0, zero_components = 0, flipped_pos = 0, flipped_dir = 0, nonzero_components = 0;
+
+static void check_vector(const float m[16], v3 v) {
+    const v3 p = xform_pos(m, v), d = xform_dir(m, v);
+    const float in[3] = { v.x, v.y, v.z }, po[3] = { p.x, p.y, p.z }, dr[3] = { d.x, d.y, d.z };
+    for (int a = 0; a < 3; a++) {
+        if (in[a] != 0.0f) {
+            nonzero_components++;
+            CHECK(bits_of(po[a]) == bits_of(in[a]));
+            CHECK(bits_of(dr[a]) == bits_of(in[a]));
+        } else {
+            zero_components++;
+            CHECK((bits_of(po[a]) & 0x7fffffffu) == 0u);
+            CHECK((bits_of(dr[a]) & 0x7fffffffu) == 0u);
+            if (bits_of(po[a]) != bits_of(in[a])) flipped_pos++;
+            if (bits_of(dr[a]) != bits_of(in[a])) flipped_dir++;
+        }
+    }
+    vectors++;
+}
+
+static void check_arithmetic() {
+    snprintf(current, sizeof(current), "arithmetic");
+    float m[16];
+    const long N = 1l << 20;
+    for (long i = 0; i < N; i++) {
+        const v3 v = { component(), component(), component() };
+        class_matrix(0u, m); check_vector(m, v);
+        class_matrix(0x1ffu, m); check_vector(m, v);
+        for (int k = 0; k < 6; k++) { class_matrix((uint32_t)((i * 6 + k) & 0x1ff), m); check_vector(m, v); }
+    }
+    const uint32_t corner[] = { 0x00000000u, 0x80000000u, 0x00000001u, 0x80000001u, 0x7f7fffffu, 0xff7fffffu, 0x3f800000u, 0xc0490fdbu };
+    for (uint32_t pattern = 0; pattern < 512u; pattern++) {
+        class_matrix(pattern, m);
+        for (uint32_t x : corner) for (uint32_t y : corner) for (uint32_t z : corner) check_vector(m, v3{ from_bits(x), from_bits(y), from_bits(z) });
+    }
+    CHECK(vectors >= 8 * N);
+    CHECK(zero_components > N / 8 && nonzero_components > N);
+    CHECK(flipped_pos > zero_components / 20 && flipped_dir > zero_components / 20);
+}
+
+int main() {
+    check_facts();
+    check_arithmetic();
+    printf("lone_check: %ld vector transforms, %ld non-zero components copied, %ld zero components, sign changed under xform_pos %ld (%.1f %%), under xform_dir %ld (%.1f %%)\n",
+           vectors, nonzero_components, zero_components, flipped_pos, 100.0 * (double)flipped_pos / (double)zero_components, flipped_dir,
+           100.0 * (double)flipped_dir / (double)zero_components);
+    if (failures) { printf("lone_check: %d FAILED\n", failures); return 1; }
+    printf("lone_check: ok\n");
+    return 0;
+}
diff --git a/cpu-raytracer_amd/csrc/plan_check.cpp b/cpu-raytracer_amd/csrc/plan_check.cpp
--- a/cpu-raytracer_amd/csrc/plan_check.cpp
+++ b/cpu-raytracer_amd/csrc/plan_check.cpp
@@ -493,7 +493,29 @@
     }
 }
 
+static void lone_entry() {
+    CASE("lone entry");
+    PlanInputs in = frame(); in.knobs.lone_entry = true;
+    const RenderPlan none = plan_render(in);
+    CHECK(!none.lone && !none.copy_class);
+    in.lone = true;
+    const RenderPlan lone = plan_render(in);
+    CHECK(lone.lone == 1 && !lone.copy_class && memcmp(&lone, &none, sizeof(lone)) != 0);
+    in.copy_class = true;
+    const RenderPlan copy = plan_render(in);
+    CHECK(copy.lone == 1 && copy.copy_class == 1 && memcmp(&copy, &lone, sizeof(copy)) != 0);
+    in.lone = false;
+    CHECK(!plan_render(in).lone && !plan_render(in).copy_class);
+    in.lone = true; in.knobs.lone_entry = false;
+    const RenderPlan off = plan_render(in);
+    CHECK(!off.lone && !off.copy_class);
+    in.lone = false; in.copy_class = false;
+    const RenderPlan off_none = plan_render(in);
+    CHECK(memcmp(&off, &off_none, sizeof(off)) == 0);
+}
+
 int main() {
+    lone_entry();
     small_grids();
     twelve_levels();
     modes_and_schedule();
diff --git a/cpu-raytracer_amd/csrc/rtx_api.hip b/cpu-raytracer_amd/csrc/rtx_api.hip
--- a/cpu-raytracer_amd/csrc/rtx_api.hip
+++ b/cpu-raytracer_amd/csrc/rtx_api.hip
@@ -83,6 +83,7 @@
     DevScene scene;
     bool frame_set = false;
     bool frame_rigid = true;
+    LoneFacts frame_lone = { false, false };
     DevBuf d_upd, d_upd_sort; int upd_cap = 0;
     DevBuf d_views, d_vfb_rgb, d_vfb_packed;
     StageRing view_ring;
@@ -199,6 +200,7 @@
     K.tex_pass_levels = (int)knob_int("RTX_TEX_PASS_LEVELS", rtxt::DEFAULT_PASS_LEVELS, 1, rtxt::MAX_PASS_LEVELS);
     c->nearest_fetch = knob_int("RTX_NEAREST_FETCH", 1, 0, 1) != 0;
     c->query_grid = (int)knob_int("RTX_QUERY_GRID", 0, 0, 1 << 20);
+    K.lone_entry = knob_int("RTX_PK_LONE_ENTRY", 1, 0, 1) != 0;
     K.fail_item_alloc = knob_int("RTX_DEBUG_FAIL_ITEM_ALLOC", 0, 0, 1) != 0;
     int bpc = 0;
     hipOccupancyMaxActiveBlocksPerMultiprocessor(&bpc, k_trace_fast<false>, RTX_TRACE_BLOCK, 0);
@@ -491,6 +493,8 @@
     for (int i = 0; i < f->plane_count; i++) c->frame_primitive_materials.push_back(f->planes[i].material_id);
     c->tlas_inner_depth = tlas_depth;
     c->frame_set = true; c->refs_dirty = true; c->frame_rigid = rigid;
+    c->frame_lone = plan_lone_facts(f->instance_count, f->tlas_nodes, f->tlas_node_count, f->tlas_indices, f->tlas_index_count, f->instances);
+    s.lone = c->knobs.lone_entry && c->frame_lone.lone; s.copy_class = s.lone && c->frame_lone.copy_class;
     return RTX_OK;
 }
 
@@ -708,6 +712,7 @@
     c->tlas_inner_depth = rtxu::tree_inner_depth(n);
     c->refs_dirty = true;
     c->frame_rigid = true;
+    c->frame_lone = LoneFacts{ false, false }; s.lone = 0; s.copy_class = 0;
     return RTX_OK;
 }
 
@@ -1167,6 +1172,7 @@
     in.all_wide = all_meshes_wide(c);
     in.stack = stack_figures(c);
     in.n_cu = c->n_cu; in.pk_blocks_closest = c->pk_blocks_closest; in.pk_blocks_any = c->pk_blocks_any;
+    in.lone = c->frame_lone.lone; in.copy_class = c->frame_lone.copy_class;
     return in;
 }
 
diff --git a/cpu-raytracer_amd/csrc/rtx_device.h b/cpu-raytracer_amd/csrc/rtx_device.h
--- a/cpu-raytracer_amd/csrc/rtx_device.h
+++ b/cpu-raytracer_amd/csrc/rtx_device.h
@@ -94,6 +94,7 @@
     const rtx_spot_light *        spot_lights;  int32_t spot_light_count;
     const rtx_directional_light * dir_lights;   int32_t dir_light_count;
     int32_t light_count;
+    int32_t lone, copy_class;
 };
 
 struct DevQueues {
diff --git a/cpu-raytracer_amd/csrc/rtx_packet.h b/cpu-raytracer_amd/csrc/rtx_packet.h
--- a/cpu-raytracer_amd/csrc/rtx_packet.h
+++ b/cpu-raytracer_amd/csrc/rtx_packet.h
@@ -96,6 +96,7 @@
 #endif
 struct PkWalk {
     rtx_cptr tlas, nodes, tris;
+    rtx_cptr nodes4;
     rtx_gptr lane_nodes, lane_nodes4c, lane_tris;
     int sp, floor_sp, cur_inst, depth;
     int cur_idx, cur_first, cur_cnt;
@@ -1371,8 +1372,74 @@
     if (err) W.err = 1;
 }
 
+template <bool ANY>
+RTX_D void pk_bind_mesh(const DevScene & sc, PkWalk & W, const int inst) {
+    W.cur_blas = rfl(sc.instances[inst].blas_id);
+    const DevBlas & B = sc.blas[W.cur_blas];
+    W.nodes = pk_cptr(B.pk_nodes); W.tris = pk_cptr(B.tri_hot); W.cur_inst = inst;
+    W.lane_nodes = RTX_GPTR(B.nodes); W.lane_tris = RTX_GPTR(B.tri_hot);
+    if (ANY) W.nodes4 = pk_cptr(B.pk4_nodes); else W.lane_nodes4c = RTX_GPTR(B.pk4c_nodes);
+}
+
+template <bool ANY, bool FAST, bool ASM, bool SPLIT>
+RTX_D bool pk_enter(const DevScene & sc, PkWalk & W, const int lane, const bool ordered, const PkHybrid & H, const int inst, const unsigned long long pm,
+                    const v3 o, const v3 d, const bool bound, const bool copy) {
+    if (!bound) pk_bind_mesh<ANY>(sc, W, inst);
+    v3 co = o, cinv = V3(W.ray.i_xy.x, W.ray.i_xy.y, W.ray.i_zz.x);
+    if (!copy) {
+        const rtx_instance & I = sc.instances[inst];
+        co = xform_pos(I.world_inv, o);
+        const v3 cd = xform_dir(I.world_inv, d);
+        cinv = vrcp(cd);
+        pk_set_ray(W.ray, co, cd, cinv);
+    }
+    const DevBlas & B = sc.blas[W.cur_blas];
+    W.floor_sp = W.sp; W.depth = 0;
+    const float4 na = sld(W.nodes, 0), nb = sld(W.nodes, 1);
+    const bool risky = FAST && __ballot(W.valid && !inv_is_finite(cinv) && pk_nan_possible(B, co, cinv)) != 0ull;
+    W.m = (risky ? __ballot(pk_slab<false>(na, nb, W.ray)) : __ballot(pk_slab<FAST>(na, nb, W.ray))) & pm;
+    W.cur_idx = 0; W.cur_first = as_i(nb.z); W.cur_cnt = as_i(nb.w);
+    if (risky) return false;
+    if (ASM && FAST && !ANY && H.closest_asm) {
+#ifdef RTX_LANE_PROF
+        asm volatile("s_waitcnt vmcnt(0) lgkmcnt(0)" ::: "memory"); const unsigned long long sw_t0 = __builtin_amdgcn_s_memtime(); const int sw_s0 = W.pk_steps;
+#endif
+#ifdef RTX_PK_SKIPWALK
+        W.m = 0ull;
+#else
+        pk_blas_closest_asm(W, sc.stack_size, ordered ? 1 : 0, H, PRIM_TRI | inst, H.gthread);
+#endif
+#ifdef RTX_LANE_PROF
+        asm volatile("s_waitcnt vmcnt(0) lgkmcnt(0)" ::: "memory");
+        W.lp[13] = (uint32_t)rfl((int)(W.lp[13] + (uint32_t)(__builtin_amdgcn_s_memtime() - sw_t0))); W.lp[14] = (uint32_t)rfl((int)(W.lp[14] + (uint32_t)(W.pk_steps - sw_s0)));
+        W.lp[15] = (uint32_t)rfl((int)(W.lp[15] + 1u));
+#endif
+    }
+    if (ASM && FAST && ANY) {
+        PK_T0();
+        W.psp = 0;
+        if (SPLIT) {
+#ifdef RTX_PK_SKIPWALK
+            W.m = 0ull;
+#else
+            pk_blas_any_asm4(W, W.nodes4, H.lane_lds, H.t0, H.t_leaf, H.grow, H.item_cap, H.item_base, W.item_slot);
+#endif
+            PK_T1(1);
+        } else if (W.nodes4) {
+            pk_blas_any_asm4(W, W.nodes4, H.lane_lds, H.t0, H.t_leaf, H.grow, 0u, 0ull, 0u);
+            PK_T1(1);
+            if (W.alive != 0ull && __ballot(W.psp > 0) != 0ull) { PK_T0(); pk_lane_phase_any4(W, lane, H.lane_lds, H.spill, H.spill_stride, RTX_GPTR(W.nodes4), W.lane_tris); PK_T1(2); }
+        } else {
+            pk_blas_any_asm(W, sc.stack_size, H.lane_lds, H.t0, H.grow);
+            PK_T1(1);
+            if (W.alive != 0ull && __ballot(W.psp > 0) != 0ull) { PK_T0(); pk_lane_phase_any(W, lane, H.stk, H.spill, H.spill_stride, W.lane_nodes, W.lane_tris); PK_T1(2); }
+        }
+    }
+    return true;
+}
+
 template <bool ANY, bool PSTAT, bool FAST, bool ASM, bool SPLIT, typename WorldFn>
-RTX_D bool pk_walk(const DevScene & sc, PkWalk & W, const int lane, const bool ordered, const PkHybrid & H, WorldFn && world) {
+RTX_D bool pk_walk(const DevScene & sc, PkWalk & W, const int lane, const bool ordered, const PkHybrid & H, WorldFn && world, unsigned long long enter_m, const bool copy) {
     for (;;) {
         if (W.m != 0ull) {
             if (!ANY && ASM && FAST && W.floor_sp >= 0) {
@@ -1445,24 +1512,28 @@
             continue;
         }
         PK_T0();
-        if (ANY && W.alive == 0ull) return true;
-        if (W.floor_sp >= 0 && W.sp == W.floor_sp) {
-            if (!ANY && ASM && FAST && W.pub != W.alive) {
-                if (W.lane_nodes4c) pk_lane_phase_closest<true>(W, lane, ordered, H, W.lane_nodes, W.lane_nodes4c, W.lane_tris);
-                else pk_lane_phase_closest<false>(W, lane, ordered, H, W.lane_nodes, nullptr, W.lane_tris);
-                W.pub = W.alive;
+        const bool direct = enter_m != 0ull;
+        if (!direct) {
+            if (ANY && W.alive == 0ull) return true;
+            if (W.floor_sp >= 0 && W.sp == W.floor_sp) {
+                if (!ANY && ASM && FAST && W.pub != W.alive) {
+                    if (W.lane_nodes4c) pk_lane_phase_closest<true>(W, lane, ordered, H, W.lane_nodes, W.lane_nodes4c, W.lane_tris);
+                    else pk_lane_phase_closest<false>(W, lane, ordered, H, W.lane_nodes, nullptr, W.lane_tris);
+                    W.pub = W.alive;
+                }
+                if (W.sp == 0) return true;
+                W.floor_sp = -1; W.nodes = W.tlas;
+                v3 o, d; world(o, d);
+                pk_set_ray(W.ray, o, d, vrcp(d));
             }
             if (W.sp == 0) return true;
-            W.floor_sp = -1; W.nodes = W.tlas;
-            v3 o, d; world(o, d);
-            pk_set_ray(W.ray, o, d, vrcp(d));
-        }
-        if (W.sp == 0) return true;
-        W.sp--;
-        const int ea = __builtin_amdgcn_readlane(W.st_a, W.sp), eb = __builtin_amdgcn_readlane(W.st_b, W.sp);
-        const int edf = __builtin_amdgcn_readlane(W.st_df, W.sp);
-        const unsigned long long em = ((unsigned long long)(uint32_t)__builtin_amdgcn_readlane(W.st_mhi, W.sp) << 32) |
-                                      (unsigned long long)(uint32_t)__builtin_amdgcn_readlane(W.st_mlo, W.sp);
+            W.sp--;
+        }
+        const int ea = direct ? 0 : __builtin_amdgcn_readlane(W.st_a, W.sp), eb = direct ? 1 : __builtin_amdgcn_readlane(W.st_b, W.sp);
+        const int edf = direct ? PK_FLAG_ITER : __builtin_amdgcn_readlane(W.st_df, W.sp);
+        const unsigned long long em = direct ? enter_m : ((unsigned long long)(uint32_t)__builtin_amdgcn_readlane(W.st_mhi, W.sp) << 32) |
+                                                         (unsigned long long)(uint32_t)__builtin_amdgcn_readlane(W.st_mlo, W.sp);
+        enter_m = 0ull;
         unsigned long long pm = em & W.alive;
         if (!ANY && ASM && FAST && (pm & ~W.pub) != 0ull) {
             if (((pm & ~W.pub) >> lane) & 1ull) {
@@ -1473,56 +1544,10 @@
         if (pm == 0ull) continue;
         if (edf & PK_FLAG_ITER) {
             if (eb > 1) pk_push<ANY>(W, ea + 1, eb - 1, pm, 0, PK_FLAG_ITER);
-            const int inst = rfl(sc.tlas_indices[ea]);
-            const rtx_instance & I = sc.instances[inst];
-            v3 o, d; world(o, d);
-            const v3 co = xform_pos(I.world_inv, o), cd = xform_dir(I.world_inv, d), cinv = vrcp(cd);
-            pk_set_ray(W.ray, co, cd, cinv);
-            W.cur_blas = rfl(I.blas_id);
-            const DevBlas & B = sc.blas[W.cur_blas];
-            W.nodes = pk_cptr(B.pk_nodes); W.tris = pk_cptr(B.tri_hot); W.cur_inst = inst;
-            W.lane_nodes = RTX_GPTR(B.nodes); W.lane_tris = RTX_GPTR(B.tri_hot); if (!ANY) W.lane_nodes4c = RTX_GPTR(B.pk4c_nodes);
-            W.floor_sp = W.sp; W.depth = 0;
-            const float4 na = sld(W.nodes, 0), nb = sld(W.nodes, 1);
-            const bool risky = FAST && __ballot(W.valid && !inv_is_finite(cinv) && pk_nan_possible(B, co, cinv)) != 0ull;
-            W.m = (risky ? __ballot(pk_slab<false>(na, nb, W.ray)) : __ballot(pk_slab<FAST>(na, nb, W.ray))) & pm;
-            W.cur_idx = 0; W.cur_first = as_i(nb.z); W.cur_cnt = as_i(nb.w);
-            if (risky) return false;
-            if (ASM && FAST && !ANY && H.closest_asm) {
-#ifdef RTX_LANE_PROF
-                asm volatile("s_waitcnt vmcnt(0) lgkmcnt(0)" ::: "memory"); const unsigned long long sw_t0 = __builtin_amdgcn_s_memtime(); const int sw_s0 = W.pk_steps;
-#endif
-#ifdef RTX_PK_SKIPWALK
-                W.m = 0ull;
-#else
-                pk_blas_closest_asm(W, sc.stack_size, ordered ? 1 : 0, H, PRIM_TRI | inst, H.gthread);
-#endif
-#ifdef RTX_LANE_PROF
-                asm volatile("s_waitcnt vmcnt(0) lgkmcnt(0)" ::: "memory");
-                W.lp[13] = (uint32_t)rfl((int)(W.lp[13] + (uint32_t)(__builtin_amdgcn_s_memtime() - sw_t0))); W.lp[14] = (uint32_t)rfl((int)(W.lp[14] + (uint32_t)(W.pk_steps - sw_s0)));
-                W.lp[15] = (uint32_t)rfl((int)(W.lp[15] + 1u));
-#endif
-            }
-            if (ASM && FAST && ANY) {
-                PK_T0();
-                W.psp = 0;
-                if (SPLIT) {
-#ifdef RTX_PK_SKIPWALK
-                    W.m = 0ull;
-#else
-                    pk_blas_any_asm4(W, pk_cptr(B.pk4_nodes), H.lane_lds, H.t0, H.t_leaf, H.grow, H.item_cap, H.item_base, W.item_slot);
-#endif
-                    PK_T1(1);
-                } else if (B.pk4_nodes) {
-                    pk_blas_any_asm4(W, pk_cptr(B.pk4_nodes), H.lane_lds, H.t0, H.t_leaf, H.grow, 0u, 0ull, 0u);
-                    PK_T1(1);
-                    if (W.alive != 0ull && __ballot(W.psp > 0) != 0ull) { PK_T0(); pk_lane_phase_any4(W, lane, H.lane_lds, H.spill, H.spill_stride, RTX_GPTR(B.pk4_nodes), RTX_GPTR(B.tri_hot)); PK_T1(2); }
-                } else {
-                    pk_blas_any_asm(W, sc.stack_size, H.lane_lds, H.t0, H.grow);
-                    PK_T1(1);
-                    if (W.alive != 0ull && __ballot(W.psp > 0) != 0ull) { PK_T0(); pk_lane_phase_any(W, lane, H.stk, H.spill, H.spill_stride, RTX_GPTR(B.nodes), RTX_GPTR(B.tri_hot)); PK_T1(2); }
-                }
-            }
+            const int inst = direct ? 0 : rfl(sc.tlas_indices[ea]);
+            v3 o = V3(W.ray.o_xy.x, W.ray.o_xy.y, W.ray.o_zz.x), d = W.ray.d;
+            if (!direct) world(o, d);
+            if (!pk_enter<ANY, FAST, ASM, SPLIT>(sc, W, lane, ordered, H, inst, pm, o, d, direct, direct && copy)) return false;
         } else {
             W.m = pm;
             if (!ANY && !(edf & PK_FLAG_PRETESTED)) {
@@ -1581,6 +1606,9 @@
     W.tlas = pk_cptr(sc.pk_tlas_nodes);
     W.err = 0; W.st_pairs = W.st_tris = W.st_pair_lanes = W.st_tri_lanes = 0ull; W.item_n = 0; W.item_slot = 0; W.cur_blas = 0;
     W.st_a = W.st_b = W.st_mlo = W.st_mhi = W.st_idx = W.st_df = 0;
+    W.nodes4 = (rtx_cptr)0;
+    const bool lone = sc.lone != 0;
+    if (lone) pk_bind_mesh<ANY>(sc, W, 0);
     unsigned long long st_packets = 0ull;
     ShadeTally tally = { 0, 0, 0, 0, 0, 0, 0, 0 };
     uint32_t chunk_next = 0, chunk_end = 0;
@@ -1687,10 +1715,10 @@
             const v3 winv = vrcp(wd);
             pk_set_ray(W.ray, wo, wd, winv);
             const bool nanfree_world = __ballot(W.valid && !inv_is_finite(winv) && pk_nan_possible_tlas(sc, wo, winv)) == 0ull;
-            W.nodes = W.tlas; W.tris = W.tlas;
-            W.sp = 0; W.floor_sp = -1; W.cur_inst = 0; W.depth = 0; W.cur_idx = 0;
+            if (!lone) { W.nodes = W.tlas; W.tris = W.tlas; W.cur_inst = 0; }
+            W.sp = 0; W.floor_sp = -1; W.depth = 0; W.cur_idx = 0;
             {
-                const float4 na = sld(W.nodes, 0), nb = sld(W.nodes, 1);
+                const float4 na = sld(W.tlas, 0), nb = sld(W.tlas, 1);
                 W.m = (nanfree_world ? __ballot(pk_slab<true>(na, nb, W.ray)) : __ballot(pk_slab<false>(na, nb, W.ray))) & W.alive;
                 W.cur_first = as_i(nb.z); W.cur_cnt = as_i(nb.w);
             }
@@ -1698,9 +1726,15 @@
 #ifdef RTX_PK_PROF
             const unsigned long long pk_w0_ = __builtin_amdgcn_s_memtime();
 #endif
+            unsigned long long enter_m = 0ull; bool copy = false;
+            if (lone) {
+                enter_m = W.m; W.m = 0ull;
+                const bool has_zero = wo.x == 0.0f || wo.y == 0.0f || wo.z == 0.0f || wd.x == 0.0f || wd.y == 0.0f || wd.z == 0.0f;
+                copy = sc.copy_class != 0 && __ballot(W.valid && has_zero) == 0ull;
+            }
             bool done = false;
-            if (nanfree_world && !done) done = pk_walk<ANY, PSTAT, true, !PSTAT, SPLIT>(sc, W, lane, ordered, H, world);
-            if (!done) pk_walk<ANY, PSTAT, false, false, SPLIT>(sc, W, lane, ordered, H, world);
+            if (nanfree_world && !done) { done = pk_walk<ANY, PSTAT, true, !PSTAT, SPLIT>(sc, W, lane, ordered, H, world, enter_m, copy); enter_m = 0ull; }
+            if (!done) pk_walk<ANY, PSTAT, false, false, SPLIT>(sc, W, lane, ordered, H, world, enter_m, copy);
 #ifdef RTX_PK_PROF
             {
                 const unsigned long long dt = __builtin_amdgcn_s_memtime() - pk_w0_;
diff --git a/cpu-raytracer_amd/csrc/rtx_plan.h b/cpu-raytracer_amd/csrc/rtx_plan.h
--- a/cpu-raytracer_amd/csrc/rtx_plan.h
+++ b/cpu-raytracer_amd/csrc/rtx_plan.h
@@ -17,7 +17,24 @@
     bool fuse_shade;
     int update_small_max;
     int tex_pass_levels;
+    bool lone_entry;
 };
+
+struct LoneFacts { bool lone, copy_class; };
+static inline LoneFacts plan_lone_facts(int instance_count, const rtx_bvh_node * tlas_nodes, int tlas_node_count, const int32_t * tlas_indices, int tlas_index_count,
+                                        const rtx_instance * instances) {
+    LoneFacts f = { false, false };
+    if (instance_count != 1 || tlas_node_count < 1 || tlas_index_count < 1 || !tlas_nodes || !tlas_indices || !instances) return f;
+    if (tlas_nodes[0].count != 1 || tlas_nodes[0].left_or_first != 0 || tlas_indices[0] != 0) return f;
+    f.lone = true;
+    uint32_t bits[12]; memcpy(bits, instances[0].world_inv, sizeof(bits));
+    f.copy_class = true;
+    for (int k = 0; k < 12; k++) {
+        const bool diagonal = k == 0 || k == 5 || k == 10;
+        if (diagonal ? bits[k] != 0x3f800000u : (bits[k] & 0x7fffffffu) != 0u) f.copy_class = false;
+    }
+    return f;
+}
 
 struct StackFigures { bool unfit_mesh; int dt, blas_any, blas_shared; };
 
@@ -35,6 +52,7 @@
     bool heatmap, can_spawn, all_wide;
     StackFigures stack;
     int n_cu, pk_blocks_closest, pk_blocks_any;
+    bool lone, copy_class;
 };
 
 enum : int32_t { CLOSEST_PLAIN, CLOSEST_PLAIN_COUNT, CLOSEST_LANE, CLOSEST_PACKET_STATS, CLOSEST_PACKET, CLOSEST_PACKET_FUSED, CLOSEST_PACKET_FUSED_CULL };
@@ -54,6 +72,7 @@
     int32_t split, item_cap;
     int32_t lpt; uint32_t lpt_n;
     int32_t graph_eligible;
+    int32_t lone, copy_class;
 };
 
 static inline int plan_shared_walk_need(const StackFigures & s) {
@@ -100,6 +119,7 @@
     RenderPlan p; memset(&p, 0, sizeof(p));
     const Knobs & K = in.knobs;
     p.flags = in.flags; p.views = in.views;
+    p.lone = K.lone_entry && in.lone; p.copy_class = p.lone && in.copy_class;
     const bool count_work = (in.flags & RTX_RENDER_COUNT_WORK) != 0;
     const bool simple = (in.flags & RTX_RENDER_SIMPLE_TRACE) != 0;
     p.cull = (in.flags & RTX_RENDER_CULL_DEAD_SHADOW_RAYS) != 0 && !simple && !count_work;
```
